# perdoch/hesaff

Hardware: AMD Instinct MI355X
Metric: keypoints/sec (descriptors written), 4K grayscale batch (higher is better)
Workload: dtype f32

## Files before the change

hesaff_amd/csrc/capi_impl.h:

```cpp
#pragma once

namespace {

int fail(hesaff_ctx *c, const HsError &e)
{
   if (c) c->err = e.msg; else g_create_error = e.msg;
   return e.code;
}

#define HS_API_BEGIN try {
#define HS_API_END(ctx)                                              \
   }                                                                 \
   catch (const HsError &e) { return fail(ctx, e); }                 \
   catch (const std::exception &e) { return fail(ctx, HsError(HESAFF_ERR_NOMEM, e.what())); } \
   return HESAFF_OK;

void bind_device(hesaff_ctx *c) { HIP_TRY(hipSetDevice(c->device)); }

void finish_stream(hesaff_ctx *c)
{
   HIP_TRY(hipStreamSynchronize(c->stream));
   HIP_TRY(hipGetLastError());
}

bool finite_f(float v) { return v == v && v - v == 0.0f; }

void validate_params(const hesaff_params &p)
{
   if (!finite_f(p.threshold) || !finite_f(p.edgeEigenValueRatio) || !finite_f(p.initialSigma) || !finite_f(p.convergenceThreshold) ||
       !finite_f(p.mrSize) || !finite_f(p.maxBinValue))
      throw HsError(HESAFF_ERR_ARG, "non-finite parameter");
   if (!(p.initialSigma > 0.0f)) throw HsError(HESAFF_ERR_ARG, "initialSigma must be positive");
   if (!(p.mrSize > 0.0f)) throw HsError(HESAFF_ERR_ARG, "mrSize must be positive");
   if (!(p.edgeEigenValueRatio > 0.0f)) throw HsError(HESAFF_ERR_ARG, "edgeEigenValueRatio must be positive");
   if (p.maxIterations < 1 || p.maxIterations > 1000) throw HsError(HESAFF_ERR_ARG, "maxIterations out of range (1..1000)");
   if (p.fast == 1)
      throw HsError(HESAFF_ERR_ARG, "hesaff_params.fast = 1 was withdrawn in ABI version 4 (it bought 1.02x); use 0 (parity mode) or 2");
   if (p.fast != 0 && p.fast != 2) throw HsError(HESAFF_ERR_ARG, "fast must be 0 (parity mode) or 2");
}

void begin_device_batch(hesaff_ctx *c, int n)
{
   bind_device(c);
   if (n > c->par.max_batch) throw HsError(HESAFF_ERR_ARG, "n exceeds hesaff_params.max_batch for the device-resident entry point");
}

template <class CHECK>
void detect_device(hesaff_ctx *c, int n, const SrcImages &src, int height, int width, int32_t *count_hessian, int32_t *count_desc,
                   const void **d_keys_out, int64_t *total_out, CHECK check_source)
{
   plan(c, c->par.max_batch, height, width);
   check_source();
   run_batch(c, src, n, height, width);
   const int32_t *hs = c->h_starts, *ds = c->h_starts + (n + 1);
   for (int b = 0; b < n; b++) {
      if (count_hessian) count_hessian[b] = hs[b + 1] - hs[b];
      if (count_desc) count_desc[b] = ds[b + 1] - ds[b];
   }
   if (d_keys_out) *d_keys_out = c->geo.b_out.p;
   if (total_out) *total_out = ds[n];
}

}

extern "C" {

const char *hesaff_version(void)
{
#ifdef HESAFF_TUNING
   return "hesaff_amd 0.3 (gfx950, tuning build)";
#else
   return "hesaff_amd 0.3 (gfx950)";
#endif
}

int hesaff_abi_version(void) { return HESAFF_ABI_VERSION; }
size_t hesaff_sizeof_params(void) { return sizeof(hesaff_params); }
size_t hesaff_sizeof_timings(void) { return sizeof(hesaff_timings); }
size_t hesaff_sizeof_region(void) { return sizeof(hesaff_region); }

int hesaff_device_count(void)
{
   int n = 0;
   if (hipGetDeviceCount(&n) != hipSuccess) { (void)hipGetLastError(); return 0; }
   return n;
}

int hesaff_shard_range(int n, int rank, int world, int *lo, int *hi)
{
   if (n < 0 || world < 1 || rank < 0 || rank >= world || !lo || !hi) return HESAFF_ERR_ARG;
   *lo = (int)(((long long)n * rank + world - 1) / world);
   *hi = (int)(((long long)n * (rank + 1) + world - 1) / world);
   return HESAFF_OK;
}

int hesaff_default_params(hesaff_params *p)
{
   if (!p) return HESAFF_ERR_ARG;
   p->threshold = 16.0f / 3.0f;
   p->edgeEigenValueRatio = 10.0f;
   p->initialSigma = 1.6f;
   p->maxIterations = 16;
   p->convergenceThreshold = 0.05f;
   p->mrSize = 3.0f * sqrtf(3.0f);
   p->maxBinValue = 0.2f;
   p->upscaleInputImage = 0;
   p->max_batch = 64;
   p->max_kpts_per_mpx = 40000;
   p->fast = 0;
   return HESAFF_OK;
}

int hesaff_create(hesaff_ctx **out, const hesaff_params *p, int device)
{
   if (!out) return HESAFF_ERR_ARG;
   *out = nullptr;
   hesaff_ctx *c = nullptr;
   try {
      int ndev = 0;
      if (hipGetDeviceCount(&ndev) != hipSuccess || ndev <= 0)
         throw HsError(HESAFF_ERR_DEVICE, "no HIP device visible: libhesaff_amd has no CPU fallback");
      if (device < 0 || device >= ndev) throw HsError(HESAFF_ERR_ARG, "device ordinal out of range");
      c = new hesaff_ctx();
      if (p) c->par = *p; else hesaff_default_params(&c->par);
      if (c->par.max_batch < 1) c->par.max_batch = 1;
      if (c->par.max_kpts_per_mpx < 1000) c->par.max_kpts_per_mpx = 1000;
      validate_params(c->par);
      c->device = device;
      c->fast_pyramid = c->par.fast == 2;
#ifdef HESAFF_TUNING
      if (const char *fm = getenv("HESAFF_FAST")) c->fast_pyramid = atoi(fm) == 2;
#endif
      bind_device(c);
      hipDeviceProp_t prop;
      HIP_TRY(hipGetDeviceProperties(&prop, device));
      if (strncmp(prop.gcnArchName, "gfx950", 6) != 0) {
         std::string m = std::string("device is ") + prop.gcnArchName + ", this library is built for gfx950 only";
         throw HsError(HESAFF_ERR_DEVICE, m);
      }
      {
         hipStream_t *slots[7] = {&c->stream, &c->side_streams[0], &c->side_streams[1], &c->side_streams[2], &c->side_streams[3], &c->sift_stream,
                                  &c->aff_stream};
         const int group[7] = {0, 1, 1, 2, 0, 3, 2};
         hipStream_t made[4] = {nullptr, nullptr, nullptr, nullptr};
         if (take_stream_set(device, c->sset))
            for (int g = 0; g < 4; g++) made[g] = c->sset.comp[g];
         for (int i = 0; i < 7; i++) {
            if (!made[group[i]]) HIP_TRY(hipStreamCreateWithFlags(&made[group[i]], hipStreamNonBlocking));
            *slots[i] = made[group[i]];
         }
         for (int g = 0; g < 4; g++) c->sset.comp[g] = made[g];
      }
      for (int i = 0; i < HS_NSIDE; i++) c->ev_join[i] = DevEvent(hipEventDisableTiming);
      c->ev_fork = DevEvent(hipEventDisableTiming);
      c->ev_detect_done = DevEvent(hipEventDisableTiming | hipEventBlockingSync);
      c->ev_batch_done = DevEvent(hipEventDisableTiming | hipEventBlockingSync);
      for (int i = 0; i < HS_NSLOT; i++) {
         c->ev_extract_done[i] = DevEvent(hipEventDisableTiming);
         c->ev_sift_done[i] = DevEvent(hipEventDisableTiming);
      }
      set_kernel_attrs(c);
      build_tables(c);
      refresh_tables_struct(c);
      memset(&c->tm, 0, sizeof c->tm);
#ifdef HESAFF_TUNING
      if (const char *ov = getenv("HESAFF_OVERLAP")) c->no_overlap = atoi(ov) == 0;
      c->debug = getenv("HESAFF_DEBUG") != nullptr;
#endif
   } catch (const HsError &e) {
      hesaff_destroy(c);
      return fail(nullptr, e);
   } catch (const std::exception &e) {
      hesaff_destroy(c);
      return fail(nullptr, HsError(HESAFF_ERR_NOMEM, e.what()));
   }
   *out = c;
   return HESAFF_OK;
}

void hesaff_destroy(hesaff_ctx *c)
{
   if (!c) return;
   const int device = c->device;
   (void)hipSetDevice(device);
   StreamSet set = c->sset;
   set.h2d = c->h2d_stream; set.d2h = c->d2h_stream;
   for (hipStream_t st : {c->stream, set.comp[0], set.comp[1], set.comp[2], set.comp[3], set.h2d, set.d2h})
      if (st) (void)hipStreamSynchronize(st);
   delete c;
   if (set.comp[0]) give_stream_set(device, set);
}

const char *hesaff_last_error(const hesaff_ctx *c) { return c ? c->err.c_str() : g_create_error.c_str(); }

int hesaff_set_profiling(hesaff_ctx *c, int level)
{
   if (!c) return HESAFF_ERR_ARG;
   c->profiling = level;
   return HESAFF_OK;
}

int hesaff_get_timings(const hesaff_ctx *c, hesaff_timings *t)
{
   if (!c || !t) return HESAFF_ERR_ARG;
   *t = c->tm;
   return HESAFF_OK;
}

int hesaff_detect_batch_device(hesaff_ctx *c, int n, const void *d_gray, int width, int height, int32_t *count_hessian,
                               int32_t *count_desc, const void **d_keys_out, int64_t *total_out)
{
   if (!c || n < 1 || !d_gray) return HESAFF_ERR_ARG;
   HS_API_BEGIN
   begin_device_batch(c, n);
   detect_device(c, n, SrcImages::u8(d_gray, 1, (long long)width * height, width), height, width, count_hessian, count_desc, d_keys_out, total_out, [] {});
   HS_API_END(c)
}

}

namespace {
using namespace hesaff_engine;

[[noreturn]] void throw_bad_f32(int index, const uint8_t *img, int H, int W, size_t stride)
{
   int row = 0, col = 0;
   float v = 0.0f;
   char msg[256];
   if (first_bad_f32(img, H, W, stride, &row, &col, &v))
      snprintf(msg, sizeof msg, "image %d: pixel (row %d, column %d) is %.9g; float input must be finite with |v| <= 2^20", index, row, col, (double)v);
   else
      snprintf(msg, sizeof msg, "image %d: a pixel is not finite or exceeds 2^20 in magnitude", index);
   throw HsError(HESAFF_ERR_ARG, msg);
}

const char *describe_bad_record(const hesaff_region &r, int from, int n_oct)
{
   const float lim = 1048576.0f;
   if (r.type < 0 || r.type > 2) return "type is not 0, 1 or 2";
   if (!finite_f(r.x) || !finite_f(r.y) || !finite_f(r.s) || !finite_f(r.response)) return "x, y, s or response is not finite";
   if (fabsf(r.x) > lim || fabsf(r.y) > lim) return "|x| or |y| exceeds 2^20";
   if (!(r.s > 0.0f && r.s <= lim)) return "s is not in (0, 2^20]";
   if (from == HESAFF_FROM_POINTS) {
      if (r.octave < 0 || r.octave >= n_oct) return "octave is outside this image's pyramid";
      if (r.level < 0 || r.level >= HS_NSCALES) return "level is not one the detector finds keypoints on (0..2)";
      return nullptr;
   }
   const float a[4] = {r.a11, r.a12, r.a21, r.a22};
   for (float v : a) {
      if (!finite_f(v)) return "a11..a22 is not finite";
      if (fabsf(v) > lim) return "|a_ij| exceeds 2^20";
   }
   if ((double)r.a11 * (double)r.a22 - (double)r.a12 * (double)r.a21 == 0.0) return "a11 * a22 - a12 * a21 is zero";
   if ((double)r.a11 * (double)r.a11 + (double)r.a12 * (double)r.a12 == 0.0) return "a11^2 + a12^2 is zero";
   return nullptr;
}

int pyramid_octaves(int H, int W, int up)
{
   int n = 0;
   for (int r = H << up, cc = W << up; r > 2 * HS_BORDER + 2 && cc > 2 * HS_BORDER + 2 && n < HS_MAX_OCTAVES; r /= 2, cc /= 2) n++;
   return n;
}

void ensure_copy_streams(hesaff_ctx *c)
{
   if (c->h2d_stream) return;
   int prio_least = 0, prio_greatest = 0;
   HIP_TRY(hipDeviceGetStreamPriorityRange(&prio_least, &prio_greatest));
   if (c->sset.h2d && c->sset.d2h) {
      c->h2d_stream = c->sset.h2d; c->d2h_stream = c->sset.d2h;
   } else {
      HIP_TRY(hipStreamCreateWithPriority(&c->h2d_stream, hipStreamNonBlocking, prio_greatest));
      HIP_TRY(hipStreamCreateWithPriority(&c->d2h_stream, hipStreamNonBlocking, prio_greatest));
   }
   for (int i = 0; i < 2; i++) {
      c->ev_h2d[i] = DevEvent(hipEventDisableTiming);
      c->ev_h2d_blk[i] = DevEvent(hipEventDisableTiming | hipEventBlockingSync);
      c->ev_in_free[i] = DevEvent(hipEventDisableTiming | hipEventBlockingSync);
      c->ev_out_ready[i] = DevEvent(hipEventDisableTiming);
      c->ev_d2h[i] = DevEvent(hipEventDisableTiming | hipEventBlockingSync);
      for (int q = 0; q < 4; q++) c->ev_exp[i][q] = DevEvent(hipEventDefault);
   }
}

void run_chunks(hesaff_ctx *c, ChunkIO &io, int ring)
{
   bind_device(c);
   ensure_copy_streams(c);
   struct State {
      HostChunk q;
      std::vector<int32_t> nh, nd;
      std::vector<size_t> off;
      std::vector<unsigned long long> toff;
      size_t text_at = 0, bin_at = 0;
      size_t regions_at = 0;
      int total = 0, block = -1, no = 0, largest = 0;
      uint32_t n_rec = 0;
      bool copied = false;
   };
   const int wants = io.wants();
   c->ring.reset(ring);
   if (ring > 0 && (int)c->pin_out.size() < ring) c->pin_out.resize((size_t)ring);
   std::vector<std::future<void>> presize((size_t)std::max(ring, 0));
   bool presized = false;
   struct JoinPresize {
      std::vector<std::future<void>> &f;
      ~JoinPresize() { for (auto &x : f) if (x.valid()) x.wait(); }
   } join_presize{presize};

   auto stage = [&](int k) -> std::unique_ptr<State> {
      (void)pthread_setname_np(pthread_self(), "hs-stage");
      HIP_TRY(hipSetDevice(c->device));
      std::unique_ptr<State> s(new State());
      if (!io.next(s->q)) return nullptr;
      const HostChunk &q = s->q;
      const int slot = k & 1;
      const size_t row_bytes = (size_t)q.W * q.bpp(), img_bytes = row_bytes * q.H;
      const size_t unit = q.blob_bytes ? q.blob_bytes : img_bytes, total = unit * q.data.size();
      hs_wait_event(c->ev_in_free[slot]);
      s->largest = std::max<int>((int)q.data.size(), std::min(io.largest_chunk((int)q.data.size()), c->par.max_batch));
      c->b_in2[slot].ensure(img_bytes * (size_t)s->largest);
      if (q.blob_bytes) c->b_jcoef[slot].ensure(unit * (size_t)s->largest);
      if (q.pinned) {
         uint8_t *dst = (uint8_t *)(q.blob_bytes ? c->b_jcoef[slot].p : c->b_in2[slot].p);
         for (size_t b = 0; b < q.data.size(); b++)
            HIP_TRY(hipMemcpyAsync(dst + unit * b, q.data[b], unit, hipMemcpyHostToDevice, c->h2d_stream));
         HIP_TRY(hipEventRecord(c->ev_h2d[slot], c->h2d_stream));
         HIP_TRY(hipEventRecord(c->ev_h2d_blk[slot], c->h2d_stream));
         hs_wait_event(c->ev_h2d_blk[slot]);
         io.staged(q);
         return s;
      }
      c->pin_in[slot].ensure(unit * (size_t)s->largest);
      const size_t nimg = q.data.size();
      std::vector<size_t> bad_img(nimg + 1, nimg);
      auto copy_images = [&](size_t b0, size_t b1) {
         for (size_t b = b0; b < b1; b++) {
            uint8_t *dst = (uint8_t *)c->pin_in[slot].p + unit * b;
            if (q.blob_bytes) { memcpy(dst, q.data[b], unit); continue; }
            const size_t stride = q.stride[b];
            if (q.f32) {
               for (int y = 0; y < q.H; y++)
                  if (!copy_row_f32(dst + row_bytes * y, q.data[b] + stride * y, q.W)) { bad_img[b0] = b; return; }
               continue;
            }
            if (stride == row_bytes) memcpy(dst, q.data[b], img_bytes);
            else for (int y = 0; y < q.H; y++) memcpy(dst + row_bytes * y, q.data[b] + stride * y, row_bytes);
         }
      };
      const size_t nthr = (total >= ((size_t)32 << 20) && nimg >= 4) ? (size_t)std::max(1, std::min(4, c->stage_threads)) : 1;
      {
         std::vector<std::thread> th;
         size_t t = 1;
         try {
            for (; t < nthr; t++) th.emplace_back(copy_images, nimg * t / nthr, nimg * (t + 1) / nthr);
         } catch (...) {
         }
         copy_images(0, nimg / nthr);
         if (t < nthr) copy_images(nimg * t / nthr, nimg);
         for (auto &x : th) x.join();
      }
      if (q.f32) {
         const size_t b = *std::min_element(bad_img.begin(), bad_img.end());
         if (b < nimg) throw_bad_f32(q.index[b], q.data[b], q.H, q.W, q.stride[b]);
      }
      if (q.from) {
         const int n_oct = pyramid_octaves(q.H, q.W, c->up);
         unsigned long long n_rec = 0;
         for (int cnt : q.region_count) n_rec += (unsigned long long)cnt;
         if (n_rec > 0x7fffffffull) throw HsError(HESAFF_ERR_CAPACITY, "more records in a chunk than 32-bit indices hold");
         const size_t rec_at = describe_records_offset((int)nimg), bytes = rec_at + (size_t)n_rec * sizeof(hesaff_region);
         c->pin_reg[slot].ensure_grow(bytes);
         c->b_reg[slot].ensure_grow(bytes);
         int32_t *starts = (int32_t *)c->pin_reg[slot].p;
         hesaff_region *dst = (hesaff_region *)((char *)c->pin_reg[slot].p + rec_at);
         size_t at = 0;
         for (size_t b = 0; b < nimg; b++) {
            starts[b] = (int32_t)at;
            const hesaff_region *src = q.regions[b];
            for (int i = 0; i < q.region_count[b]; i++) {
               if (const char *why = describe_bad_record(src[i], q.from, n_oct)) {
                  char msg[256];
                  snprintf(msg, sizeof msg, "image %d: record %d: %s", q.index[b], i, why);
                  throw HsError(HESAFF_ERR_ARG, msg);
               }
               dst[at + (size_t)i] = src[i];
            }
            at += (size_t)q.region_count[b];
         }
         starts[nimg] = (int32_t)at;
         s->n_rec = (uint32_t)at;
         HIP_TRY(hipMemcpyAsync(c->b_reg[slot].p, c->pin_reg[slot].p, bytes, hipMemcpyHostToDevice, c->h2d_stream));
      }
      HIP_TRY(hipMemcpyAsync(q.blob_bytes ? c->b_jcoef[slot].p : c->b_in2[slot].p, c->pin_in[slot].p, total, hipMemcpyHostToDevice, c->h2d_stream));
      HIP_TRY(hipEventRecord(c->ev_h2d[slot], c->h2d_stream));
      io.staged(q);
      return s;
   };
   auto deliver = [&](State &s) {
      if (s.copied) hs_wait_event(c->ev_d2h[s.no & 1]);
      if (s.total > 0 && c->profiling && (wants & (WANT_TEXT | WANT_BIN))) {
         float ms = 0.0f;
         float ms2 = 0.0f;
         if (hipEventElapsedTime(&ms, c->ev_exp[s.no & 1][0], c->ev_exp[s.no & 1][1]) == hipSuccess && hipEventElapsedTime(&ms2, c->ev_exp[s.no & 1][2], c->ev_exp[s.no & 1][3]) == hipSuccess) {
            ms += ms2; c->export_ms = ms; c->export_rows = s.total; c->tm.export_ms = ms; c->tm.export_rows = s.total; }
         else (void)hipGetLastError();
      }
      ChunkDone d;
      const char *blk = (const char *)c->pin_out[(size_t)s.block].p;
      d.chunk = &s.q; d.count_hessian = s.nh.data(); d.count_desc = s.nd.data(); d.key_off = s.off.data();
      d.keys = (wants & WANT_KEYS) ? (const hesaff_keypoint *)blk : nullptr; d.block = s.block;
      if (wants & WANT_TEXT) { d.text = blk + s.text_at; d.text_off = s.toff.data(); }
      if (wants & WANT_BIN) d.bin = blk + s.bin_at;
      if (wants & WANT_REGIONS) d.regions = (const hesaff_region *)(blk + s.regions_at);
      io.done(d);
   };

   std::future<std::unique_ptr<State>> staged = std::async(std::launch::async, stage, 0);
   std::unique_ptr<State> prev;
   try {
      for (int k = 0;; k++) {
         const auto dbg_t0 = std::chrono::steady_clock::now();
         const double dbg_c0 = c->debug ? thread_cpu_ms() : 0.0;
         std::unique_ptr<State> cur = staged.get();
         if (!cur) break;
         const auto dbg_t1 = std::chrono::steady_clock::now();
         const double dbg_c1 = c->debug ? thread_cpu_ms() : 0.0;
         cur->no = k;
         staged = std::async(std::launch::async, stage, k + 1);
         const HostChunk &q = cur->q;
         const int slot = k & 1, B = (int)q.data.size();
         const size_t row_bytes = (size_t)q.W * q.bpp(), img_bytes = row_bytes * q.H;
         HIP_TRY(hipStreamWaitEvent(c->stream, c->ev_h2d[slot], 0));
         try {
            plan(c, std::max(std::min<int>(c->par.max_batch, B), cur->largest), q.H, q.W);
            if (q.blob_bytes) jpeg_pixels(c, c->b_jcoef[slot].as<uint8_t>(), make_jpeg_geom(q.jpeg), B, (uint8_t *)c->b_in2[slot].p, img_bytes, c->stream);
            const SrcImages src = q.f32 ? SrcImages::f32(c->b_in2[slot].p, (long long)img_bytes, (int)row_bytes)
                                        : SrcImages::u8(c->b_in2[slot].p, q.ch, (long long)img_bytes, (int)row_bytes);
            if (q.from) run_describe(c, src, B, q.H, q.W, (const uint8_t *)c->b_reg[slot].p, cur->n_rec, q.from);
            else run_batch(c, src, B, q.H, q.W);
         } catch (const HsError &e) {
            if (e.code != HESAFF_ERR_ARG && e.code != HESAFF_ERR_CAPACITY) throw;
            HIP_TRY(hipEventRecord(c->ev_in_free[slot], c->stream));
            if (!io.failed(q, e.code)) throw;
            continue;
         }
         HIP_TRY(hipEventRecord(c->ev_in_free[slot], c->stream));
         const auto dbg_t2 = std::chrono::steady_clock::now();
         const double dbg_c2 = c->debug ? thread_cpu_ms() : 0.0;
         const int32_t *hs = c->h_starts, *ds = c->h_starts + (B + 1);
         cur->total = ds[B];
         cur->nh.resize((size_t)B); cur->nd.resize((size_t)B); cur->off.resize((size_t)B);
         for (int b = 0; b < B; b++) {
            cur->nh[(size_t)b] = hs[b + 1] - hs[b];
            cur->nd[(size_t)b] = ds[b + 1] - ds[b];
            cur->off[(size_t)b] = (size_t)ds[b];
         }
         const size_t n_rows = (size_t)cur->total, n_hess = (size_t)hs[B];
         const KeyRec *d_keys = c->geo.b_out.as<KeyRec>();
         size_t at = 0;
         auto place = [&at](size_t bytes) { const size_t o = at; at = (at + bytes + 255) & ~(size_t)255; return o; };
// ... 209 lines not shown
int hesaff_describe_regions(hesaff_ctx *c, int n, const uint8_t *const *images, const int *widths, const int *heights, const int *strides,
                            const int *channels, const hesaff_region *const *regions, const int *counts, int from, hesaff_region_result *results)
{
   if (!c || n < 0 || (n > 0 && (!images || !widths || !heights || !regions || !counts || !results))) return HESAFF_ERR_ARG;
   HS_API_BEGIN
   const DescribeInput di = describe_input(n, regions, counts, from);
   detect_images(c, n, images, false, widths, heights, strides, channels, 0, [&](ArrayIO &io) { io.region_results = results; }, di);
   HS_API_END(c)
}

int hesaff_describe_regions_f32(hesaff_ctx *c, int n, const float *const *images, const int *widths, const int *heights, const int *strides,
                                const hesaff_region *const *regions, const int *counts, int from, hesaff_region_result *results)
{
   if (!c || n < 0 || (n > 0 && (!images || !widths || !heights || !regions || !counts || !results))) return HESAFF_ERR_ARG;
   HS_API_BEGIN
   const DescribeInput di = describe_input(n, regions, counts, from);
   detect_images(c, n, images, true, widths, heights, strides, nullptr, 0, [&](ArrayIO &io) { io.region_results = results; }, di);
   HS_API_END(c)
}

int hesaff_detect_batch_device_f32(hesaff_ctx *c, int n, const void *d_planes, int width, int height, int row_stride, int64_t img_stride,
                                   int32_t *count_hessian, int32_t *count_desc, const void **d_keys_out, int64_t *total_out)
{
   if (!c || n < 1 || !d_planes || width < 1 || height < 1 || row_stride < 0 || img_stride < 0) return HESAFF_ERR_ARG;
   HS_API_BEGIN
   begin_device_batch(c, n);
   const long long rs = row_stride ? row_stride : 4LL * width;
   const long long is = img_stride ? (long long)img_stride : rs * height;
   if ((uintptr_t)d_planes % 4 != 0) throw HsError(HESAFF_ERR_ARG, "float planes not 4-byte aligned");
   if (rs < 4LL * width || rs % 4 != 0 || rs > 0x7fffffffLL)
      throw HsError(HESAFF_ERR_ARG, "row stride of a float plane must be at least 4 * width bytes and a multiple of 4");
   if (is % 4 != 0 || (n > 1 && is < rs * (height - 1) + 4LL * width))
      throw HsError(HESAFF_ERR_ARG, "image stride of the float planes must be a multiple of 4 and keep the images apart");
   detect_device(c, n, SrcImages::f32(d_planes, is, (int)rs), height, width, count_hessian, count_desc, d_keys_out, total_out,
                 [&] { check_device_f32(c, n, (const uint8_t *)d_planes, is, (int)rs, height, width); });
   HS_API_END(c)
}

int hesaff_set_output_format(hesaff_ctx *c, int format)
{
   if (!c || (format & ~(HESAFF_OUT_TEXT | HESAFF_OUT_BIN)) != 0 || format == 0) return HESAFF_ERR_ARG;
   c->out_format = format;
   return HESAFF_OK;
}

int hesaff_set_resume(hesaff_ctx *c, int on)
{
   if (!c || on < 0 || on > 2) return HESAFF_ERR_ARG;
   c->resume = on;
   return HESAFF_OK;
}

int hesaff_set_pinned_read_budget(hesaff_ctx *c, size_t max_bytes, size_t keep_bytes)
{
   if (!c) return HESAFF_ERR_ARG;
   {
      std::lock_guard<std::mutex> lk(c->pin_read.mu);
      c->pin_read.max_bytes = max_bytes;
      c->pin_read.keep_bytes = std::min(keep_bytes, max_bytes);
   }
   c->pin_read.trim(c->pin_read.keep_bytes);
   return HESAFF_OK;
}

int hesaff_set_pool_priority(hesaff_ctx *c, int mode)
{
   if (!c || mode < -1 || mode > 1) return HESAFF_ERR_ARG;
   c->pool_priority = mode;
   return HESAFF_OK;
}

int hesaff_process_files(hesaff_ctx *c, int n, const char *const *paths, const char *const *out_paths, int decode_threads,
                         int write_threads, hesaff_file_status *status)
{
   if (!c || n < 0 || (n > 0 && (!paths || !status))) return HESAFF_ERR_ARG;
   HS_API_BEGIN
   for (int i = 0; i < n; i++) { status[i].rc = HESAFF_ERR_IO; status[i].stage = HESAFF_FILE_PENDING; status[i].count_hessian = 0; status[i].count_desc = 0; }
   hesaff_host_plan hp;
   (void)hesaff_host_plan_for(1, &hp);
   const int dt = std::max(1, std::min(decode_threads > 0 ? decode_threads : hp.decode_threads, 64));
   const int wt = std::max(1, std::min(write_threads > 0 ? write_threads : hp.write_threads, 256));
   const bool device_jpeg = true;
   PinHooks pin;
   c->pin_read.device = c->device;
   pin.alloc = [](size_t bytes, void *user) -> void * { return ((hesaff_ctx *)user)->pin_read.take(bytes); };
   pin.release = [](void *p, size_t bytes, void *user) { ((hesaff_ctx *)user)->pin_read.give(p, bytes); };
   pin.user = c;
   const bool nice_pool = c->pool_priority == 1 || (c->pool_priority < 0 && hesaff_host_threads() <= dt + wt + 1);
   FileIO io(&c->ring, c->par.max_batch, c->par.mrSize, c->out_format, n, paths, out_paths, status, dt, wt, true, c->resume, device_jpeg, pin, nice_pool);
   c->stage_threads = hesaff_stage_threads_for_pool(dt + wt);
   try {
      run_chunks(c, io, 3);
      io.wait_writers();
   } catch (...) {
      io.shutdown();
      c->pin_read.trim(c->pin_read.keep_bytes);
      throw;
   }
   io.shutdown();
   c->pin_read.trim(c->pin_read.keep_bytes);
   HS_API_END(c)
}


int hesaff_stage_gaussian_blur(hesaff_ctx *c, const float *in, int rows, int cols, float sigma, float *out)
{
   if (!c || !in || !out || rows < 1 || cols < 1 || !(sigma > 0.0f)) return HESAFF_ERR_ARG;
   HS_API_BEGIN
   bind_device(c);
   const int K = hesaff::gauss_ksize(sigma);
   const int pitch = round_up(cols, 64);
   const size_t n = (size_t)rows * pitch;
   c->b_stage.ensure(n * 4 * 3 + (size_t)(K + 16) * 4);
   float *d_in = c->b_stage.as<float>(), *d_tmp = d_in + n, *d_out = d_tmp + n, *d_taps = d_out + n;
   std::vector<float> taps(K, 1.0f);
   if (K > 1) hesaff::gauss_taps(K, sigma, taps.data());
   HIP_TRY(hipMemcpy2DAsync(d_in, (size_t)pitch * 4, in, (size_t)cols * 4, (size_t)cols * 4, rows, hipMemcpyHostToDevice, c->stream));
   HIP_TRY(hipMemcpyAsync(d_taps, taps.data(), (size_t)K * 4, hipMemcpyHostToDevice, c->stream));
   DPlane pi = make_plane(d_in, rows, cols, pitch), pt = make_plane(d_tmp, rows, cols, pitch), po = make_plane(d_out, rows, cols, pitch);
   const DPlane none = make_plane(nullptr, 0, 0, 0);
   if (K == 1) {
      HIP_TRY(hipMemcpyAsync(d_out, d_in, n * 4, hipMemcpyDeviceToDevice, c->stream));
   } else if (K == 9 || K == 11 || K == 13 || K == 15) {
      launch_blur_hess<true, false, false>(c, pi, po, none, none, d_taps, K, 0.0f, 1);
   } else {
      const dim3 grid((cols + 255) / 256, rows, 1);
      hipLaunchKernelGGL(k_blur_rows_generic, grid, dim3(256), 0, c->stream, pi, pt, (const float *)d_taps, K);
      hipLaunchKernelGGL(k_blur_cols_generic, grid, dim3(256), 0, c->stream, pt, po, (const float *)d_taps, K);
   }
   HIP_TRY(hipMemcpy2DAsync(out, (size_t)cols * 4, d_out, (size_t)pitch * 4, (size_t)cols * 4, rows, hipMemcpyDeviceToHost, c->stream));
   finish_stream(c);
   HS_API_END(c)
}

int hesaff_stage_hessian_response(hesaff_ctx *c, const float *in, int rows, int cols, float norm, float *out)
{
   if (!c || !in || !out || rows < 1 || cols < 1) return HESAFF_ERR_ARG;
   HS_API_BEGIN
   bind_device(c);
   const int pitch = round_up(cols, 64);
   const size_t n = (size_t)rows * pitch;
   c->b_stage.ensure(n * 4 * 4 + 64);
   float *d_in = c->b_stage.as<float>(), *d_out = d_in + n, *d_l = d_out + n, *d_r = d_l + n, *d_taps = d_r + n;
   HIP_TRY(hipMemcpy2DAsync(d_in, (size_t)pitch * 4, in, (size_t)cols * 4, (size_t)cols * 4, rows, hipMemcpyHostToDevice, c->stream));
   DPlane pi = make_plane(d_in, rows, cols, pitch), po = make_plane(d_out, rows, cols, pitch);
   std::vector<float> taps(9);
   hesaff::gauss_taps(9, 1.2262737f, taps.data());
   HIP_TRY(hipMemcpyAsync(d_taps, taps.data(), 9 * 4, hipMemcpyHostToDevice, c->stream));
   launch_march<9, true, true, false, true>(c, pi, make_plane(d_l, rows, cols, pitch), make_plane(d_r, rows, cols, pitch), make_plane(nullptr, 0, 0, 0),
                                            d_taps, 1.0f, 1, po, norm * norm);
   HIP_TRY(hipMemcpy2DAsync(out, (size_t)cols * 4, d_out, (size_t)pitch * 4, (size_t)cols * 4, rows, hipMemcpyDeviceToHost, c->stream));
   finish_stream(c);
   HS_API_END(c)
}

int hesaff_stage_half_image(hesaff_ctx *c, const float *in, int rows, int cols, float *out)
{
   if (!c || !in || !out || rows < 2 || cols < 2) return HESAFF_ERR_ARG;
   HS_API_BEGIN
   bind_device(c);
   const size_t n = (size_t)rows * cols;
   const int r2 = rows / 2, c2 = cols / 2;
   c->b_stage.ensure(n * 4 * 2);
   float *d_in = c->b_stage.as<float>(), *d_out = d_in + n;
   HIP_TRY(hipMemcpyAsync(d_in, in, n * 4, hipMemcpyHostToDevice, c->stream));
   DPlane pi = make_plane(d_in, rows, cols, cols), po = make_plane(d_out, r2, c2, c2);
   hipLaunchKernelGGL(k_half, dim3((c2 + 255) / 256, r2, 1), dim3(256), 0, c->stream, pi, po);
   HIP_TRY(hipMemcpyAsync(out, d_out, (size_t)r2 * c2 * 4, hipMemcpyDeviceToHost, c->stream));
   finish_stream(c);
   HS_API_END(c)
}

static int stage_pyramid(hesaff_ctx *c, const void *image, bool f32, int rows, int cols, float *planes, int *n_octaves, size_t *n_floats)
{
   if (!c || rows < 1 || cols < 1) return HESAFF_ERR_ARG;
   HS_API_BEGIN
   bind_device(c);
   plan(c, 1, rows, cols);
   size_t nf = 0;
   for (const OctGeom &g : c->oct) nf += (size_t)10 * g.rows * g.cols;
   if (n_octaves) *n_octaves = (int)c->oct.size();
   if (n_floats) *n_floats = nf;
   if (planes) {
      if (!image) throw HsError(HESAFF_ERR_ARG, f32 ? "plane is NULL" : "gray is NULL");
      const size_t row_bytes = (size_t)cols * (f32 ? 4 : 1), bytes = row_bytes * rows;
      if (f32) {
         if ((uintptr_t)image % 4 != 0) throw HsError(HESAFF_ERR_ARG, "float plane not 4-byte aligned");
         int r = 0, col = 0;
         float v = 0.0f;
         if (first_bad_f32((const uint8_t *)image, rows, cols, row_bytes, &r, &col, &v))
            throw_bad_f32(0, (const uint8_t *)image, rows, cols, row_bytes);
      }
      c->b_input.ensure(bytes);
      c->b_stage.ensure((size_t)rows * round_up(cols, 64) * 4);
      HIP_TRY(hipMemcpyAsync(c->b_input.p, image, bytes, hipMemcpyHostToDevice, c->stream));
      c->ev_used = 0;
      StageTimer tm(c);
      Lists s = make_lists(c);
      const SrcImages src = f32 ? SrcImages::f32(c->b_input.p, (long long)bytes, (int)row_bytes) : SrcImages::u8(c->b_input.p, 1, (long long)bytes, (int)row_bytes);
      run_detection(c, src, 1, s, tm, true, planes);
      finish_stream(c);
   }
   HS_API_END(c)
}

int hesaff_stage_pyramid(hesaff_ctx *c, const uint8_t *gray, int rows, int cols, float *planes, int *n_octaves, size_t *n_floats)
{
   return stage_pyramid(c, gray, false, rows, cols, planes, n_octaves, n_floats);
}

int hesaff_stage_pyramid_f32(hesaff_ctx *c, const float *plane, int rows, int cols, float *planes, int *n_octaves, size_t *n_floats)
{
   return stage_pyramid(c, plane, true, rows, cols, planes, n_octaves, n_floats);
}

int hesaff_stage_hessian_keypoints(hesaff_ctx *c, const uint8_t *gray, int rows, int cols, int cap, float *f, int32_t *iv, int *count)
{
   if (!c || !gray || rows < 1 || cols < 1 || !count) return HESAFF_ERR_ARG;
   HS_API_BEGIN
   bind_device(c);
   plan(c, 1, rows, cols);
   c->b_input.ensure((size_t)rows * cols);
   HIP_TRY(hipMemcpyAsync(c->b_input.p, gray, (size_t)rows * cols, hipMemcpyHostToDevice, c->stream));
   c->ev_used = 0;
   StageTimer tm(c);
   Lists s = make_lists(c);
   run_detection(c, SrcImages::u8(c->b_input.p, 1, (long long)rows * cols, cols), 1, s, tm, false, nullptr);
   uint32_t cn[8];
   HIP_TRY(hipMemcpyAsync(cn, s.counters, sizeof cn, hipMemcpyDeviceToHost, c->stream));
   finish_stream(c);
   if (cn[2] != 0 || cn[1] > c->cap) throw HsError(HESAFF_ERR_CAPACITY, "keypoint capacity exceeded");
   const int n = (int)cn[3];
   *count = n;
   const int m = std::min(n, cap);
   if (m > 0 && f && iv) {
      std::vector<float> x(m), y(m), sc(m), resp(m);
      std::vector<int32_t> meta(m), key(m);
      HIP_TRY(hipMemcpy(x.data(), s.hl.x, (size_t)m * 4, hipMemcpyDeviceToHost));
      HIP_TRY(hipMemcpy(y.data(), s.hl.y, (size_t)m * 4, hipMemcpyDeviceToHost));
      HIP_TRY(hipMemcpy(sc.data(), s.hl.s, (size_t)m * 4, hipMemcpyDeviceToHost));
      HIP_TRY(hipMemcpy(resp.data(), s.hl.response, (size_t)m * 4, hipMemcpyDeviceToHost));
      HIP_TRY(hipMemcpy(meta.data(), s.hl.meta, (size_t)m * 4, hipMemcpyDeviceToHost));
      HIP_TRY(hipMemcpy(key.data(), s.hl.r0c0, (size_t)m * 4, hipMemcpyDeviceToHost));
      for (int i = 0; i < m; i++) {
         const int octave = (meta[i] >> 4) & 15, level = (meta[i] >> 2) & 3, type = meta[i] & 3;
         const OctGeom &g = c->oct[octave];
         const uint32_t pix = (uint32_t)key[i] % (uint32_t)(g.rows * g.cols);
         f[5 * i] = x[i]; f[5 * i + 1] = y[i]; f[5 * i + 2] = sc[i]; f[5 * i + 3] = c->consts.pd0 * (float)(1 << octave); f[5 * i + 4] = resp[i];
         iv[5 * i] = type; iv[5 * i + 1] = octave; iv[5 * i + 2] = level; iv[5 * i + 3] = (int32_t)(pix / g.cols); iv[5 * i + 4] = (int32_t)(pix % g.cols);
      }
   }
   HS_API_END(c)
}

int hesaff_stage_find_affine_shape(hesaff_ctx *c, const float *blur, int rows, int cols, int n, const float *kp, int32_t *converged,
                                   float *U, int32_t *iters)
{
   if (!c || !blur || !kp || rows < 2 || cols < 2 || n < 0) return HESAFF_ERR_ARG;
   HS_API_BEGIN
   bind_device(c);
   if (n == 0) return HESAFF_OK;
   const size_t np = (size_t)rows * cols;
   c->b_stage.ensure(np * 4 + (size_t)n * (4 + 6) * 4 + 64);
   float *d_plane = c->b_stage.as<float>();
   float *d_kp = d_plane + np;
   int32_t *d_conv = (int32_t *)(d_kp + (size_t)4 * n), *d_iters = d_conv + n;
   float *d_U = (float *)(d_iters + n);
   HIP_TRY(hipMemcpyAsync(d_plane, blur, np * 4, hipMemcpyHostToDevice, c->stream));
   HIP_TRY(hipMemcpyAsync(d_kp, kp, (size_t)n * 16, hipMemcpyHostToDevice, c->stream));
   AffineOut ao; ao.converged = d_conv; ao.iters = d_iters; ao.U = d_U;
   DPlane P = make_plane(d_plane, rows, cols, cols);
   hipLaunchKernelGGL(k_affine_stage, dim3(std::min((n + HS_AFFP_G - 1) / HS_AFFP_G, 256 * 6)), dim3(64), 0, c->stream, P, (const float *)d_kp, n, c->tables, c->consts, ao);
   if (converged) HIP_TRY(hipMemcpyAsync(converged, d_conv, (size_t)n * 4, hipMemcpyDeviceToHost, c->stream));
   if (iters) HIP_TRY(hipMemcpyAsync(iters, d_iters, (size_t)n * 4, hipMemcpyDeviceToHost, c->stream));
   if (U) HIP_TRY(hipMemcpyAsync(U, d_U, (size_t)n * 16, hipMemcpyDeviceToHost, c->stream));
   finish_stream(c);
   HS_API_END(c)
}

int hesaff_stage_rectify(hesaff_ctx *c, int n, float *A)
{
   if (!c || !A || n < 0) return HESAFF_ERR_ARG;
   HS_API_BEGIN
   bind_device(c);
   if (n == 0) return HESAFF_OK;
   c->b_stage.ensure((size_t)n * 16);
   HIP_TRY(hipMemcpyAsync(c->b_stage.p, A, (size_t)n * 16, hipMemcpyHostToDevice, c->stream));
   hipLaunchKernelGGL(k_rectify_stage, dim3((n + 255) / 256), dim3(256), 0, c->stream, n, c->b_stage.as<float>());
   HIP_TRY(hipMemcpyAsync(A, c->b_stage.p, (size_t)n * 16, hipMemcpyDeviceToHost, c->stream));
   finish_stream(c);
   HS_API_END(c)
}

int hesaff_stage_normalize_affine(hesaff_ctx *c, const float *img, int rows, int cols, int n, const float *kp, const float *A,
                                  int32_t *rejected, float *patches)
{
   if (!c || !img || !kp || !A || rows < 2 || cols < 2 || n < 0) return HESAFF_ERR_ARG;
   HS_API_BEGIN
   bind_device(c);
   if (n == 0) return HESAFF_OK;
   plan(c, 1, rows, cols);
   if ((uint32_t)n > c->cap) throw HsError(HESAFF_ERR_CAPACITY, "too many keypoints for this image size");
   Lists s = make_lists(c);
   hipStream_t st = c->stream;
   HIP_TRY(hipMemcpy2DAsync(c->gray.p, (size_t)c->gray.pitch * 4, img, (size_t)cols * 4, (size_t)cols * 4, rows, hipMemcpyHostToDevice, st));
   std::vector<float> x(n), y(n), sc(n);
   std::vector<int32_t> meta(n, 0), P0(n), alive(n);
   for (int i = 0; i < n; i++) { x[i] = kp[3 * i]; y[i] = kp[3 * i + 1]; sc[i] = kp[3 * i + 2]; }
   HIP_TRY(hipMemcpyAsync(s.hl.x, x.data(), (size_t)n * 4, hipMemcpyHostToDevice, st));
   HIP_TRY(hipMemcpyAsync(s.hl.y, y.data(), (size_t)n * 4, hipMemcpyHostToDevice, st));
   HIP_TRY(hipMemcpyAsync(s.hl.s, sc.data(), (size_t)n * 4, hipMemcpyHostToDevice, st));
   HIP_TRY(hipMemcpyAsync(s.hl.meta, meta.data(), (size_t)n * 4, hipMemcpyHostToDevice, st));
   HIP_TRY(hipMemcpyAsync(s.pw.A, A, (size_t)n * 16, hipMemcpyHostToDevice, st));
   HIP_TRY(hipMemsetAsync(s.counters, 0, 64 * 4, st));
   uint32_t nn = (uint32_t)n;
   HIP_TRY(hipMemcpyAsync(s.counters + 3, &nn, 4, hipMemcpyHostToDevice, st));
   hipLaunchKernelGGL(k_prepare_patch_given_A, dim3((n + 255) / 256), dim3(256), 0, st, s.hl, (const uint32_t *)(s.counters + 3), rows, cols,
                      c->consts, c->tables, s.pw);
   c->b_patches.ensure((size_t)n * HS_PATCH_PIX * 4);
   HIP_TRY(hipMemsetAsync(c->b_patches.p, 0, (size_t)n * HS_PATCH_PIX * 4, st));
   unsigned long long large_rows = 0;
   c->batch_max_p = 0;
   for (int i = 0; i < n; i++) {
      const float mrScale = ceilf(sc[i] * c->consts.mrSize);
      const long long P = (mrScale < 1.0e6f) ? 2 * (long long)mrScale + 3 : 0;
      if (P > HS_BIN3_PMAX && P <= c->max_p0 + 2) { large_rows += (unsigned long long)P; c->batch_max_p = std::max(c->batch_max_p, (int)P); }
   }
   if (large_rows > 0xffffffffull) throw HsError(HESAFF_ERR_NOMEM, "too many huge windows in one call");
   run_patch_stage(c, s, c->gray, c->b_patches.as<float>(), 0, (uint32_t)large_rows);
   uint32_t ovf = 0;
   HIP_TRY(hipMemcpyAsync(&ovf, s.counters + 6, 4, hipMemcpyDeviceToHost, st));
   HIP_TRY(hipMemcpyAsync(alive.data(), s.pw.alive, (size_t)n * 4, hipMemcpyDeviceToHost, st));
   if (patches) HIP_TRY(hipMemcpyAsync(patches, c->b_patches.p, (size_t)n * HS_PATCH_PIX * 4, hipMemcpyDeviceToHost, st));
   finish_stream(c);
   if (ovf) throw HsError(HESAFF_ERR_NOMEM, "large-window row buffer exceeded (internal bound violated)");
   if (rejected) for (int i = 0; i < n; i++) rejected[i] = alive[i] ? 0 : 1;
   HS_API_END(c)
}

int hesaff_stage_sift(hesaff_ctx *c, int n, const float *patches, uint8_t *desc)
{
   if (!c || !patches || !desc || n < 0) return HESAFF_ERR_ARG;
   HS_API_BEGIN
   bind_device(c);
   if (n == 0) return HESAFF_OK;
   const size_t N = (size_t)n;
   const size_t off_alive = N * HS_PATCH_PIX * 4, off_mv = off_alive + N * 4, off_vec = off_mv + N * 8, off_desc = off_vec + N * 128 * 4;
   const size_t off_vo = (off_desc + N * 128 + 63) & ~(size_t)63, total = off_vo + N * HS_VO_PITCH * 8 + 64;
   c->b_stage.ensure(total);
   char *base = (char *)c->b_stage.p;
   std::vector<int32_t> ones(N, 1);
   HIP_TRY(hipMemcpyAsync(base, patches, N * HS_PATCH_PIX * 4, hipMemcpyHostToDevice, c->stream));
   HIP_TRY(hipMemcpyAsync(base + off_alive, ones.data(), N * 4, hipMemcpyHostToDevice, c->stream));
   HIP_TRY(hipMemsetAsync(base + off_vo, 0, N * HS_VO_PITCH * 8 + 64, c->stream));
   SiftIO so;
   so.patches = (const float *)base; so.alive = (const int32_t *)(base + off_alive); so.meanvar = (float *)(base + off_mv);
   so.vec = (float *)(base + off_vec); so.desc = (uint8_t *)(base + off_desc); so.h_lo = 0; so.h_hi = (uint32_t)n;
   launch_sift(c, c->stream, so, (uint32_t)n, (float2 *)(base + off_vo));
   HIP_TRY(hipMemcpyAsync(desc, base + off_desc, N * 128, hipMemcpyDeviceToHost, c->stream));
   finish_stream(c);
   HS_API_END(c)
}

int hesaff_stage_export(hesaff_ctx *c, const hesaff_keypoint *keys, int n, float mrSize, int format, char **out, size_t *len)
{
   if (!c || n < 0 || (n > 0 && !keys) || !out || !len || (format != HESAFF_OUT_TEXT && format != HESAFF_OUT_BIN)) return HESAFF_ERR_ARG;
   HS_API_BEGIN
   bind_device(c);
   const float saved = c->par.mrSize;
   c->par.mrSize = mrSize;
   char *buf = nullptr;
   try {
      const size_t N = (size_t)n;
      c->b_stage.ensure(std::max<size_t>(N * sizeof(KeyRec), 16));
      if (n > 0) HIP_TRY(hipMemcpyAsync(c->b_stage.p, keys, N * sizeof(KeyRec), hipMemcpyHostToDevice, c->stream));
      const KeyRec *d_keys = c->b_stage.as<KeyRec>();
      char head[64];
      size_t hl, body;
      if (format == HESAFF_OUT_TEXT) {
         const int32_t starts[2] = {0, n};
         c->b_ex_starts.ensure(16);
         HIP_TRY(hipMemcpyAsync(c->b_ex_starts.p, starts, sizeof starts, hipMemcpyHostToDevice, c->stream));
         std::vector<unsigned long long> off;
         body = (size_t)export_text_prepare(c, d_keys, (uint32_t)n, c->b_ex_starts.as<int32_t>(), 1, off);
         hl = (size_t)snprintf(head, sizeof head, "%d\n%d\n", 128, n);
      } else {
         body = N * EX_BIN_ROW;
         memcpy(head, "HESAFFB1", 8);
         const uint32_t dim = 128, cnt = (uint32_t)n;
         memcpy(head + 8, &dim, 4); memcpy(head + 12, &cnt, 4);
         hl = 16;
      }
      buf = (char *)malloc(hl + body + 1);
      if (!buf) throw HsError(HESAFF_ERR_NOMEM, "malloc failed");
      memcpy(buf, head, hl);
      if (body > 0) {
         c->b_generic.ensure(body + 16);
         if (format == HESAFF_OUT_TEXT) export_text_write(c, d_keys, (uint32_t)n, (char *)c->b_generic.p);
         else export_bin_rows(c, d_keys, (uint32_t)n, (char *)c->b_generic.p);
         HIP_TRY(hipMemcpyAsync(buf + hl, c->b_generic.p, body, hipMemcpyDeviceToHost, c->stream));
      }
      finish_stream(c);
      *out = buf;
      *len = hl + body;
   } catch (...) {
      c->par.mrSize = saved;
      free(buf);
      throw;
   }
   c->par.mrSize = saved;
   HS_API_END(c)
}

int hesaff_stage_fmt_g(hesaff_ctx *c, int n, const float *v, char *text, int32_t *lens)
{
   if (!c || n < 0 || (n > 0 && (!v || !text || !lens))) return HESAFF_ERR_ARG;
   HS_API_BEGIN
   bind_device(c);
   if (n == 0) return HESAFF_OK;
   const size_t N = (size_t)n;
   c->b_stage.ensure(N * (4 + 16 + 4));
   float *d_v = c->b_stage.as<float>();
   int32_t *d_len = (int32_t *)(d_v + N);
   char *d_text = (char *)(d_len + N);
   HIP_TRY(hipMemcpyAsync(d_v, v, N * 4, hipMemcpyHostToDevice, c->stream));
   HIP_TRY(hipMemsetAsync(d_text, 0, N * 16, c->stream));
   hipLaunchKernelGGL(k_fmt_g_test, dim3((n + 255) / 256), dim3(256), 0, c->stream, n, (const float *)d_v, d_text, d_len);
   HIP_TRY(hipMemcpyAsync(text, d_text, N * 16, hipMemcpyDeviceToHost, c->stream));
   HIP_TRY(hipMemcpyAsync(lens, d_len, N * 4, hipMemcpyDeviceToHost, c->stream));
   finish_stream(c);
   HS_API_END(c)
}

int hesaff_stage_jpeg_pixels(hesaff_ctx *c, const hesaff_jpeg_layout *layout, int n, const uint8_t *blobs, size_t blob_bytes, uint8_t *pixels)
{
   if (!c || !layout || n < 0 || (n > 0 && (!blobs || !pixels))) return HESAFF_ERR_ARG;
   HS_API_BEGIN
   bind_device(c);
   if (n == 0) return HESAFF_OK;
   const JpegGeom g = make_jpeg_geom(*layout);
   if ((size_t)g.blob_bytes != blob_bytes) throw HsError(HESAFF_ERR_ARG, "blob size does not match the layout");
   const size_t img = (size_t)g.W * g.H * g.nc;
   c->b_jcoef[0].ensure(blob_bytes * (size_t)n);
   c->b_stage.ensure(img * (size_t)n);
   HIP_TRY(hipMemcpyAsync(c->b_jcoef[0].p, blobs, blob_bytes * (size_t)n, hipMemcpyHostToDevice, c->stream));
   jpeg_pixels(c, c->b_jcoef[0].as<uint8_t>(), g, n, c->b_stage.as<uint8_t>(), img, c->stream);
   HIP_TRY(hipMemcpyAsync(pixels, c->b_stage.p, img * (size_t)n, hipMemcpyDeviceToHost, c->stream));
   finish_stream(c);
   HS_API_END(c)
}

int hesaff_stage_math(hesaff_ctx *c, int n, const float *a, const float *b, float *atan2_out, float *pow2_out)
{
   if (!c || !a || !b || n < 0) return HESAFF_ERR_ARG;
   HS_API_BEGIN
   bind_device(c);
   if (n == 0) return HESAFF_OK;
   c->b_stage.ensure((size_t)n * 16);
   float *d_a = c->b_stage.as<float>(), *d_b = d_a + n, *d_at = d_b + n, *d_pw = d_at + n;
   HIP_TRY(hipMemcpyAsync(d_a, a, (size_t)n * 4, hipMemcpyHostToDevice, c->stream));
   HIP_TRY(hipMemcpyAsync(d_b, b, (size_t)n * 4, hipMemcpyHostToDevice, c->stream));
   hipLaunchKernelGGL(k_math, dim3((n + 255) / 256), dim3(256), 0, c->stream, n, (const float *)d_a, (const float *)d_b, d_at, d_pw);
   if (atan2_out) HIP_TRY(hipMemcpyAsync(atan2_out, d_at, (size_t)n * 4, hipMemcpyDeviceToHost, c->stream));
   if (pow2_out) HIP_TRY(hipMemcpyAsync(pow2_out, d_pw, (size_t)n * 4, hipMemcpyDeviceToHost, c->stream));
   finish_stream(c);
   HS_API_END(c)
}

int hesaff_stage_math_sift(hesaff_ctx *c, int n, const float *gy, const float *gx, float *ori_general, float *ori_nd, float *grad_general,
                           float *grad_nd)
{
   if (!c || !gy || !gx || !ori_general || !ori_nd || !grad_general || !grad_nd || n < 0) return HESAFF_ERR_ARG;
   HS_API_BEGIN
   bind_device(c);
   if (n == 0) return HESAFF_OK;
   c->b_stage.ensure((size_t)n * 24);
   float *d = c->b_stage.as<float>();
   HIP_TRY(hipMemcpyAsync(d, gy, (size_t)n * 4, hipMemcpyHostToDevice, c->stream));
   HIP_TRY(hipMemcpyAsync(d + n, gx, (size_t)n * 4, hipMemcpyHostToDevice, c->stream));
   hipLaunchKernelGGL(k_math_sift, dim3(std::min(4096, (n + 255) / 256)), dim3(256), 0, c->stream, n, (const float *)d, (const float *)(d + n),
                      d + 2 * (size_t)n, d + 3 * (size_t)n, d + 4 * (size_t)n, d + 5 * (size_t)n);
   float *outs[4] = {ori_general, ori_nd, grad_general, grad_nd};
   for (int q = 0; q < 4; q++) HIP_TRY(hipMemcpyAsync(outs[q], d + (2 + q) * (size_t)n, (size_t)n * 4, hipMemcpyDeviceToHost, c->stream));
   finish_stream(c);
   HS_API_END(c)
}


int hesaff_table_gauss_mask(int size, float *mask)
{
   if (size < 1 || !(size & 1) || !mask) return HESAFF_ERR_ARG;
   hesaff::gauss_mask(size, mask);
   return HESAFF_OK;
}
int hesaff_table_circ_gauss_mask(int size, float *mask)
{
   if (size < 1 || !(size & 1) || !mask) return HESAFF_ERR_ARG;
   hesaff::circ_gauss_mask(size, mask);
   return HESAFF_OK;
}
int hesaff_table_sift_bins(int32_t *bin0, int32_t *bin1, float *w0, float *w1)
{
   if (!bin0 || !bin1 || !w0 || !w1) return HESAFF_ERR_ARG;
   hesaff::sift_bins(bin0, bin1, w0, w1);
   return HESAFF_OK;
}
int hesaff_table_gauss_kernel(float sigma, int cap, float *taps, int *ksize)
{
   if (!ksize) return HESAFF_ERR_ARG;
   const int K = hesaff::gauss_ksize(sigma);
   *ksize = K;
   if (taps) {
      if (cap < K) return HESAFF_ERR_ARG;
      if (K == 1) taps[0] = 1.0f; else hesaff::gauss_taps(K, sigma, taps);
   }
   return HESAFF_OK;
}

}
```

hesaff_amd/csrc/hmath.h:

```cpp
#pragma once
#include <stdint.h>

#if defined(__HIPCC__)
#define HM_HD __host__ __device__ __forceinline__
#else
#define HM_HD inline
#endif

HM_HD uint32_t hm_f2u(float f) { union { float f; uint32_t u; } v; v.f = f; return v.u; }
HM_HD float    hm_u2f(uint32_t u) { union { float f; uint32_t u; } v; v.u = u; return v.f; }
HM_HD uint64_t hm_d2u(double f) { union { double f; uint64_t u; } v; v.f = f; return v.u; }
HM_HD double   hm_u2d(uint64_t u) { union { double f; uint64_t u; } v; v.u = u; return v.f; }

HM_HD float hm_fabsf(float x) { return hm_u2f(hm_f2u(x) & 0x7fffffffu); }

HM_HD float hm_atanf(float x)
{
   const float atanhi0 = hm_u2f(0x3eed6338u), atanhi1 = hm_u2f(0x3f490fdau),
               atanhi2 = hm_u2f(0x3f7b985eu), atanhi3 = hm_u2f(0x3fc90fdau);
   const float atanlo0 = hm_u2f(0x31ac3769u), atanlo1 = hm_u2f(0x33222168u),
               atanlo2 = hm_u2f(0x33140fb4u), atanlo3 = hm_u2f(0x33a22168u);
   const float aT0 = hm_u2f(0x3eaaaaabu), aT1 = hm_u2f(0xbe4ccccdu), aT2 = hm_u2f(0x3e124925u),
               aT3 = hm_u2f(0xbde38e38u), aT4 = hm_u2f(0x3dba2e6eu), aT5 = hm_u2f(0xbd9d8795u),
               aT6 = hm_u2f(0x3d886b35u), aT7 = hm_u2f(0xbd6ef16bu), aT8 = hm_u2f(0x3d4bda59u),
               aT9 = hm_u2f(0xbd15a221u), aT10 = hm_u2f(0x3c8569d7u);
   const int32_t hx = (int32_t)hm_f2u(x);
   const int32_t ix = hx & 0x7fffffff;
   int id;
   float hi = 0.0f, lo = 0.0f;
   if (ix >= 0x4c000000) {
      if (ix > 0x7f800000) return x + x;
      return (hx > 0) ? (atanhi3 + atanlo3) : (-atanhi3 - atanlo3);
   }
   if (ix < 0x3ee00000) {
      if (ix < 0x31000000) return x;
      id = -1;
   } else {
      x = hm_fabsf(x);
      float num, den;
      if (ix < 0x3f980000) {
         if (ix < 0x3f300000) { id = 0; hi = atanhi0; lo = atanlo0; num = 2.0f * x - 1.0f; den = 2.0f + x; }
         else                 { id = 1; hi = atanhi1; lo = atanlo1; num = x - 1.0f; den = x + 1.0f; }
      } else {
         if (ix < 0x401c0000) { id = 2; hi = atanhi2; lo = atanlo2; num = x - 1.5f; den = 1.0f + 1.5f * x; }
         else                 { id = 3; hi = atanhi3; lo = atanlo3; num = -1.0f; den = x; }
      }
      x = num / den;
   }
   const float z = x * x;
   const float w = z * z;
   const float s1 = z * (aT0 + w * (aT2 + w * (aT4 + w * (aT6 + w * (aT8 + w * aT10)))));
   const float s2 = w * (aT1 + w * (aT3 + w * (aT5 + w * (aT7 + w * aT9))));
   if (id < 0) return x - x * (s1 + s2);
   const float r = hi - ((x * (s1 + s2) - lo) - x);
   return (hx < 0) ? -r : r;
}

HM_HD float hm_atan2f(float y, float x)
{
   const float tiny = 1.0e-30f;
   const float pi_o_4 = hm_u2f(0x3f490fdbu), pi_o_2 = hm_u2f(0x3fc90fdbu),
               pi = hm_u2f(0x40490fdbu), pi_lo = hm_u2f(0xb3bbbd2eu);
   const int32_t hx = (int32_t)hm_f2u(x), hy = (int32_t)hm_f2u(y);
   const int32_t ix = hx & 0x7fffffff, iy = hy & 0x7fffffff;
   if (ix > 0x7f800000 || iy > 0x7f800000) return x + y;
   if (hx == 0x3f800000) return hm_atanf(y);
   const int m = (int)(((uint32_t)hy >> 31) & 1u) | (int)(((uint32_t)hx >> 30) & 2u);
   if (iy == 0) {
      switch (m) {
         case 0: case 1: return y;
         case 2: return pi + tiny;
         default: return -pi - tiny;
      }
   }
   if (ix == 0) return (hy < 0) ? (-pi_o_2 - tiny) : (pi_o_2 + tiny);
   if (ix == 0x7f800000) {
      if (iy == 0x7f800000) {
         switch (m) {
            case 0: return pi_o_4 + tiny;
            case 1: return -pi_o_4 - tiny;
            case 2: return 3.0f * pi_o_4 + tiny;
            default: return -3.0f * pi_o_4 - tiny;
         }
      } else {
         switch (m) {
            case 0: return 0.0f;
            case 1: return -0.0f;
            case 2: return pi + tiny;
            default: return -pi - tiny;
         }
      }
   }
   if (iy == 0x7f800000) return (hy < 0) ? (-pi_o_2 - tiny) : (pi_o_2 + tiny);
   const int32_t k = (iy - ix) >> 23;
   float z;
   if (k > 60) z = pi_o_2 + 0.5f * pi_lo;
   else if (hx < 0 && k < -60) z = 0.0f;
   else z = hm_atanf(hm_fabsf(y / x));
   switch (m) {
      case 0: return z;
      case 1: return hm_u2f(hm_f2u(z) ^ 0x80000000u);
      case 2: return pi - (z - pi_lo);
      default: return (z - pi_lo) - pi;
   }
}

HM_HD float hm_atan2f_sel(float y, float x)
{
   const float pi_o_2 = hm_u2f(0x3fc90fdbu), pi = hm_u2f(0x40490fdbu), pi_lo = hm_u2f(0xb3bbbd2eu);
   const int32_t hx = (int32_t)hm_f2u(x), hy = (int32_t)hm_f2u(y);
   const int32_t ix = hx & 0x7fffffff, iy = hy & 0x7fffffff;
   const int32_t k = (iy - ix) >> 23;
   if ((ix >= 0x7f800000) | (iy >= 0x7f800000) | ((iy != 0) & (ix != 0) & ((k > 60) | (k < -60)))) return hm_atan2f(y, x);
   const float q = hm_fabsf(y / x);
   const int32_t iq = (int32_t)hm_f2u(q);
   const bool i0 = iq < 0x3f300000, i1 = iq < 0x3f980000, i2 = iq < 0x401c0000, im = iq < 0x3ee00000;
   float num = i1 ? (i0 ? 2.0f * q - 1.0f : q - 1.0f) : (i2 ? q - 1.5f : -1.0f);
   float den = i1 ? (i0 ? 2.0f + q : q + 1.0f) : (i2 ? 1.0f + 1.5f * q : q);
   float hi = i1 ? (i0 ? hm_u2f(0x3eed6338u) : hm_u2f(0x3f490fdau)) : (i2 ? hm_u2f(0x3f7b985eu) : hm_u2f(0x3fc90fdau));
   float lo = i1 ? (i0 ? hm_u2f(0x31ac3769u) : hm_u2f(0x33222168u)) : (i2 ? hm_u2f(0x33140fb4u) : hm_u2f(0x33a22168u));
   num = im ? q : num;
   den = im ? 1.0f : den;
   hi = im ? 0.0f : hi;
   lo = im ? 0.0f : lo;
   const float xr = num / den;
   const float z = xr * xr;
   const float w = z * z;
   const float aT0 = hm_u2f(0x3eaaaaabu), aT1 = hm_u2f(0xbe4ccccdu), aT2 = hm_u2f(0x3e124925u),
               aT3 = hm_u2f(0xbde38e38u), aT4 = hm_u2f(0x3dba2e6eu), aT5 = hm_u2f(0xbd9d8795u),
               aT6 = hm_u2f(0x3d886b35u), aT7 = hm_u2f(0xbd6ef16bu), aT8 = hm_u2f(0x3d4bda59u),
               aT9 = hm_u2f(0xbd15a221u), aT10 = hm_u2f(0x3c8569d7u);
   const float s1 = z * (aT0 + w * (aT2 + w * (aT4 + w * (aT6 + w * (aT8 + w * aT10)))));
   const float s2 = w * (aT1 + w * (aT3 + w * (aT5 + w * (aT7 + w * aT9))));
   float za = hi - ((xr * (s1 + s2) - lo) - xr);
   za = (iq >= 0x4c000000) ? hm_u2f(0x3fc90fdau) + hm_u2f(0x33a22168u) : za;
   float r = (hx < 0) ? pi - (za - pi_lo) : za;
   r = (ix == 0) ? ((iy == 0) ? ((hx < 0) ? pi : 0.0f) : pi_o_2) : r;
   return hm_u2f(hm_f2u(r) ^ ((uint32_t)hy & 0x80000000u));
}


#define HM_ATAN_TAB_FLOATS 40
#define HM_ATAN_TAB_INIT                                                                                           \
   {1.0f, 0.0f, 0.0f, 1.0f, 0.0f, 0.0f, 0.0f, 0.0f,                                                               \
    2.0f, 1.0f, -1.0f, 2.0f, 0x1.dac67p-2f , 0x1.586ed2p-28f , 0.0f, 0.0f,                  \
    1.0f, 1.0f, -1.0f, 1.0f, 0x1.921fb4p-1f , 0x1.4442dp-25f , 0.0f, 0.0f,                  \
    1.0f, 1.5f, -1.5f, 1.0f, 0x1.f730bcp-1f , 0x1.281f68p-25f , 0.0f, 0.0f,                 \
    0.0f, 1.0f, -1.0f, 0.0f, 0x1.921fb4p+0f , 0x1.4442dp-24f , 0.0f, 0.0f}

#if defined(__HIPCC__)
__host__ __device__ __attribute__((noinline)) inline float hm_atan2f_rare(float y, float x) { return hm_atan2f(y, x); }
#else
inline float hm_atan2f_rare(float y, float x) { return hm_atan2f(y, x); }
#endif

HM_HD float hm_div_normal(float a, float b)
{
#if defined(__HIP_DEVICE_COMPILE__)
   const float r0 = __builtin_amdgcn_rcpf(b);
   const float e0 = __builtin_fmaf(-b, r0, 1.0f);
   const float r1 = __builtin_fmaf(e0, r0, r0);
   const float q0 = a * r1;
   const float e1 = __builtin_fmaf(-b, q0, a);
   const float q1 = __builtin_fmaf(e1, r1, q0);
   const float e2 = __builtin_fmaf(-b, q1, a);
   return __builtin_fmaf(e2, r1, q1);
#else
   return a / b;
#endif
}
HM_HD float hm_sqrt_normal(float x)
{
#if defined(__HIP_DEVICE_COMPILE__)
   float s = __builtin_amdgcn_sqrtf(x);
   const float sd = hm_u2f(hm_f2u(s) - 1u), su = hm_u2f(hm_f2u(s) + 1u);
   const float vp = __builtin_fmaf(-sd, s, x), vs = __builtin_fmaf(-su, s, x);
   s = (vp <= 0.0f) ? sd : s;
   s = (vs > 0.0f) ? su : s;
   return s;
#else
   return __builtin_sqrtf(x);
#endif
}

template <bool ND>
HM_HD float hm_atan2f_tab_t(float y, float x, const float *tab)
{
   const float pi_o_2 = hm_u2f(0x3fc90fdbu), pi = hm_u2f(0x40490fdbu), pi_lo = hm_u2f(0xb3bbbd2eu);
   const int32_t hx = (int32_t)hm_f2u(x), hy = (int32_t)hm_f2u(y);
   const int32_t ix = hx & 0x7fffffff, iy = hy & 0x7fffffff;
   const int32_t k = (iy - ix) >> 23;
   if ((ix >= 0x7f800000) | (iy >= 0x7f800000) | ((iy != 0) & (ix != 0) & ((k > 60) | (k < -60)))) return hm_atan2f_rare(y, x);
   const float q = hm_fabsf(ND ? hm_div_normal(y, x) : y / x);
   const int32_t iq = (int32_t)hm_f2u(q);
   const int id = (int)(iq >= 0x3ee00000) + (int)(iq >= 0x3f300000) + (int)(iq >= 0x3f980000) + (int)(iq >= 0x401c0000);
   const float *row = tab + 8 * id;
   const float num = row[0] * q + row[2];
   const float den = row[1] * q + row[3];
   const float hi = row[4], lo = row[5];
   const float xr = ND ? hm_div_normal(num, den) : num / den;
   const float z = xr * xr;
   const float w = z * z;
   const float aT0 = hm_u2f(0x3eaaaaabu), aT1 = hm_u2f(0xbe4ccccdu), aT2 = hm_u2f(0x3e124925u),
               aT3 = hm_u2f(0xbde38e38u), aT4 = hm_u2f(0x3dba2e6eu), aT5 = hm_u2f(0xbd9d8795u),
               aT6 = hm_u2f(0x3d886b35u), aT7 = hm_u2f(0xbd6ef16bu), aT8 = hm_u2f(0x3d4bda59u),
               aT9 = hm_u2f(0xbd15a221u), aT10 = hm_u2f(0x3c8569d7u);
   const float s1 = z * (aT0 + w * (aT2 + w * (aT4 + w * (aT6 + w * (aT8 + w * aT10)))));
   const float s2 = w * (aT1 + w * (aT3 + w * (aT5 + w * (aT7 + w * aT9))));
   float za = hi - ((xr * (s1 + s2) - lo) - xr);
   za = (iq >= 0x4c000000) ? hm_u2f(0x3fc90fdau) + hm_u2f(0x33a22168u) : za;
   float r = (hx < 0) ? pi - (za - pi_lo) : za;
   r = (ix == 0) ? ((iy == 0) ? ((hx < 0) ? pi : 0.0f) : pi_o_2) : r;
   return hm_u2f(hm_f2u(r) ^ ((uint32_t)hy & 0x80000000u));
}
HM_HD float hm_atan2f_tab(float y, float x, const float *tab) { return hm_atan2f_tab_t<false>(y, x, tab); }
HM_HD float hm_atan2f_tab_nd(float y, float x, const float *tab) { return hm_atan2f_tab_t<true>(y, x, tab); }

HM_HD float hm_pow2f(float y)
{
   const uint64_t T[32] = {
      0x3ff0000000000000ull, 0x3fefd9b0d3158574ull, 0x3fefb5586cf9890full, 0x3fef9301d0125b51ull,
      0x3fef72b83c7d517bull, 0x3fef54873168b9aaull, 0x3fef387a6e756238ull, 0x3fef1e9df51fdee1ull,
      0x3fef06fe0a31b715ull, 0x3feef1a7373aa9cbull, 0x3feedea64c123422ull, 0x3feece086061892dull,
      0x3feebfdad5362a27ull, 0x3feeb42b569d4f82ull, 0x3feeab07dd485429ull, 0x3feea47eb03a5585ull,
      0x3feea09e667f3bcdull, 0x3fee9f75e8ec5f74ull, 0x3feea11473eb0187ull, 0x3feea589994cce13ull,
      0x3feeace5422aa0dbull, 0x3feeb737b0cdc5e5ull, 0x3feec49182a3f090ull, 0x3feed503b23e255dull,
      0x3feee89f995ad3adull, 0x3feeff76f2fb5e47ull, 0x3fef199bdd85529cull, 0x3fef3720dcef9069ull,
      0x3fef5818dcfba487ull, 0x3fef7c97337b9b5full, 0x3fefa4afa2a490daull, 0x3fefd0765b6e4540ull };
   const double C0 = hm_u2d(0x3fac6af84b912394ull);
   const double C1 = hm_u2d(0x3fcebfce50fac4f3ull);
   const double C2 = hm_u2d(0x3fe62e42ff0c52d6ull);
   const double SHIFT = hm_u2d(0x42e8000000000000ull);
   const double xd = (double)y;
   double kd = xd + SHIFT;
   const uint64_t ki = hm_d2u(kd);
   kd -= SHIFT;
   const double r = xd - kd;
   uint64_t t = T[ki & 31];
   t += ki << (52 - 5);
   const double s = hm_u2d(t);
#ifdef HM_POW2F_FMA
   const double z = __builtin_fma(C0, r, C1);
   const double r2 = r * r;
   double p = __builtin_fma(C2, r, 1.0);
   p = __builtin_fma(z, r2, p);
#else
   const double z = C0 * r + C1;
   const double r2 = r * r;
   double p = C2 * r + 1.0;
   p = z * r2 + p;
#endif
   p = p * s;
   return (float)p;
}

HM_HD float hm_sift_orient_coord(float ori)
{
   const double twopi = hm_u2d(0x401921fb54442d18ull);
   const double inv_twopi = hm_u2d(0x3fc45f306dc9c883ull);
   const double a = 8.0 * ((double)ori + twopi);
   const double q = a * inv_twopi;
   const double r = __builtin_fma(-q, twopi, a);
   const double q2 = __builtin_fma(r, inv_twopi, q);
   return (float)q2;
}
```

hesaff_amd/csrc/kernels_keypoint.h:

```cpp
#pragma once
#include <type_traits>
#include "device_common.h"
#include "kernels_pyramid.h"

struct PlaneTab {
   DPlane L[HS_MAX_OCTAVES][HS_NSCALES];
};

struct KpTables {
   const float *smm_mask;
   const float *sift_mask;
   const int32_t *mask_idx;
   int n_masked;
   const int4 *sgrad_nb;
   const int2 *sgrad_om;
   const int4 *vo_rows;
   const uint16_t *vo_src;
   const int32_t *bin0, *bin1;
   const float *w0, *w1;
   const float *patch_taps;
   const int32_t *patch_tap_off;
   const int32_t *patch_tap_k;
   int max_p0;
};

struct AffineOut {
   int32_t *converged;
   float *U;
   int32_t *iters;
};

#define HS_AFF_G 4
__device__ inline bool hs_window_outside(int imRows, int imCols, float ofsx, float ofsy, float a11, float a12, float a21, float a22, int half)
{
   const float width = (float)(imCols - 1), height = (float)(imRows - 1);
   bool outside = false;
#pragma unroll
   for (int q = 0; q < 4; q++) {
      const int j = (q & 1) ? half : -half, i = (q & 2) ? half : -half;
      const float rx = ofsx + (float)j * a12, ry = ofsy + (float)j * a22;
      const float fx = floorf(rx + (float)i * a11), fy = floorf(ry + (float)i * a21);
      outside = outside || !(fx >= 0.0f && fy >= 0.0f && fx < width && fy < height);
   }
   return outside;
}

#define HS_AFF_NT 23
#define HS_AFFP_G 4
#define HS_AFFP_L (64 / HS_AFFP_G)
#define HS_AFFP_SH 4
#define HS_AFFP_NT ((HS_SMM_PIX + HS_AFFP_L - 1) / HS_AFFP_L)
#define HS_AFF_BATCHES 2
#define HS_AFF_ARR 364

struct AffKp { const float *blur; int rows, cols, pitch; float x, y, s, pd; };

template <class Fetch>
__device__ __forceinline__ void hs_affine_groups(uint32_t first, uint32_t n, const float *__restrict__ mask_g, const DConsts &k, AffineOut out,
                                                 Fetch fetch)
{
   __shared__ __attribute__((aligned(16))) float s_arr[HS_AFFP_G][3][HS_AFF_ARR];
   __shared__ float s_mask[HS_AFF_ARR];
   __shared__ float s_bc[HS_AFFP_G][8];
   const int lane = threadIdx.x, grp = lane >> HS_AFFP_SH, li = lane & (HS_AFFP_L - 1);
   for (int i = lane; i < HS_SMM_PIX; i += 64) s_mask[i] = mask_g[i];
   float *s_img = s_arr[grp][0], *s_pa = s_arr[grp][0], *s_pb = s_arr[grp][1], *s_pc = s_arr[grp][2];
   uint32_t hstep = gridDim.x * HS_AFFP_G, h_end = n;
   uint32_t h = first + blockIdx.x * HS_AFFP_G + grp;
   if ((gridDim.x & 7u) == 0u && n > first) {
      const uint32_t n_items = (n - first + HS_AFFP_G - 1) / HS_AFFP_G;
      const uint32_t xcd = blockIdx.x & 7u, rank = blockIdx.x >> 3, per_xcd = gridDim.x >> 3;
      const uint32_t it_lo = (uint32_t)(((unsigned long long)n_items * xcd) >> 3), it_hi = (uint32_t)(((unsigned long long)n_items * (xcd + 1)) >> 3);
      hstep = per_xcd * HS_AFFP_G;
      h_end = min(first + it_hi * HS_AFFP_G, n);
      h = first + (it_lo + rank) * HS_AFFP_G + grp;
   }
#define HS_AFF_END h_end
   if (k.maxIterations <= 0) {
      for (; h < HS_AFF_END; h += hstep)
         if (li == 0) {
            out.converged[h] = 0; out.iters[h] = 0;
            out.U[4 * h + 0] = 1.0f; out.U[4 * h + 1] = 0.0f; out.U[4 * h + 2] = 0.0f; out.U[4 * h + 3] = 1.0f;
         }
      return;
   }
   const float *blur = nullptr;
   int pitch = 0, width = 0, height = 0, l = 0;
   float lx = 0, ly = 0, ratio = 0, u11 = 1.0f, u12 = 0.0f, u21 = 0.0f, u22 = 1.0f;
   float eigen_ratio_act = 0.0f, eigen_ratio_bef = 0.0f;
   bool active = h < HS_AFF_END;
   auto load_kp = [&]() {
      if (active) {
         const AffKp q = fetch(h);
         blur = q.blur; pitch = q.pitch; width = q.cols - 1; height = q.rows - 1;
         lx = q.x / q.pd; ly = q.y / q.pd;
         ratio = q.s / (k.affInitialSigma * q.pd);
         u11 = 1.0f; u12 = 0.0f; u21 = 0.0f; u22 = 1.0f;
         eigen_ratio_act = 0.0f; eigen_ratio_bef = 0.0f;
         l = 0;
      }
   };
   load_kp();
   HS_WAVE_LDS_SYNC();
   while (__ballot(active) != 0ull) {
      bool win_in = true;
      if (active) {
         const float a11 = u11 * ratio, a12 = u12 * ratio, a21 = u21 * ratio, a22 = u22 * ratio;
         win_in = !hs_window_outside(height + 1, width + 1, lx, ly, a11, a12, a21, a22, HS_SMM >> 1);
      }
      const bool all_in = __ballot(active && !win_in) == 0ull;
      auto sample = [&](auto inside_c) {
         constexpr bool INSIDE = decltype(inside_c)::value;
         const float a11 = u11 * ratio, a12 = u12 * ratio, a21 = u21 * ratio, a22 = u22 * ratio;
#pragma unroll
         for (int half = 0; half < HS_AFF_BATCHES; half++) {
            constexpr int NB = (HS_AFFP_NT + HS_AFF_BATCHES - 1) / HS_AFF_BATCHES;
            float sv[NB];
#pragma unroll
            for (int t = 0; t < NB; t++) {
               const int idx = min(li + HS_AFFP_L * (half * NB + t), HS_SMM_PIX - 1);
               const int jj = idx / HS_SMM, ii = idx - jj * HS_SMM;
               const int j = jj - (HS_SMM >> 1), i = ii - (HS_SMM >> 1);
               const float rx = lx + (float)j * a12;
               const float ry = ly + (float)j * a22;
               const float wx = rx + (float)i * a11;
               const float wy = ry + (float)i * a21;
               if (INSIDE) {
                  sv[t] = hs_tap_inside_ptr(blur, pitch, wx, wy);
               } else {
                  bool outside = false;
                  sv[t] = hs_bilinear(blur, pitch, width, height, wx, wy, outside);
               }
            }
#pragma unroll
            for (int t = 0; t < NB; t++) HS_KEEP(sv[t]);
#pragma unroll
            for (int t = 0; t < NB; t++) {
               const int idx = li + HS_AFFP_L * (half * NB + t);
               if (idx < HS_SMM_PIX) s_img[idx] = sv[t];
            }
         }
      };
      if (active) {
         if (all_in) sample(std::true_type{});
         else sample(std::false_type{});
      }
      HS_WAVE_LDS_SYNC();
      if (active) {
         float pa[HS_AFFP_NT];
#pragma unroll
         for (int t = 0; t < HS_AFFP_NT; t++) {
            const int idx = min(li + HS_AFFP_L * t, HS_SMM_PIX - 1);
            const int r = idx / HS_SMM, c = idx - r * HS_SMM;
            const float gxx = s_img[idx + (c < HS_SMM - 1 ? 1 : 0)] - s_img[idx - (c > 0 ? 1 : 0)];
            const float gyy = s_img[idx + (r < HS_SMM - 1 ? HS_SMM : 0)] - s_img[idx - (r > 0 ? HS_SMM : 0)];
            const float v = s_mask[idx];
            const float gxy = gxx * gyy;
            pa[t] = gxx * gxx * v;
            if (li + HS_AFFP_L * t < HS_SMM_PIX) {
               s_pb[idx] = gxy * v;
               s_pc[idx] = gyy * gyy * v;
            }
         }
         HS_WAVE_LDS_SYNC();
#pragma unroll
         for (int t = 0; t < HS_AFFP_NT; t++) {
            const int idx = li + HS_AFFP_L * t;
            if (idx < HS_SMM_PIX) s_pa[idx] = pa[t];
         }
      }
      HS_WAVE_LDS_SYNC();
      if (active && li < 3) {
         const float *pp = s_arr[grp][li];
         const float4 *p4 = reinterpret_cast<const float4 *>(pp);
         float acc = 0.0f;
         for (int i0 = 0; i0 < HS_SMM_PIX / 4; i0 += 10) {
            float4 q[10];
#pragma unroll
            for (int u = 0; u < 10; u++) q[u] = p4[i0 + u];
#pragma unroll
            for (int u = 0; u < 10; u++) { acc += q[u].x; acc += q[u].y; acc += q[u].z; acc += q[u].w; }
         }
         acc += pp[HS_SMM_PIX - 1];
         s_bc[grp][li] = acc / (float)HS_SMM_PIX;
      }
      HS_WAVE_LDS_SYNC();
      if (active && li == 0) {
         float a = s_bc[grp][0], b = s_bc[grp][1], c = s_bc[grp][2];
         float l1, l2;
         hs_inv_sqrt(a, b, c, l1, l2);
         eigen_ratio_bef = eigen_ratio_act;
         eigen_ratio_act = 1 - l2 / l1;
         const float u11t = u11, u12t = u12;
         const float n11 = a * u11t + b * u21, n12 = a * u12t + b * u22;
         const float n21 = b * u11t + c * u21, n22 = b * u12t + c * u22;
         int state = 0;
         if (!hs_eigenvalues(n11, n12, n21, n22, l1, l2)) state = 1;
         else if ((l1 / l2 > 6) || (l2 / l1 > 6)) state = 1;
         else if (eigen_ratio_act < k.convergenceThreshold && eigen_ratio_bef < k.convergenceThreshold) state = 2;
         s_bc[grp][3] = n11; s_bc[grp][4] = n12; s_bc[grp][5] = n21; s_bc[grp][6] = n22;
         s_bc[grp][7] = __int_as_float(state);
      }
      HS_WAVE_LDS_SYNC();
      if (active) {
         u11 = s_bc[grp][3]; u12 = s_bc[grp][4]; u21 = s_bc[grp][5]; u22 = s_bc[grp][6];
         const int state = __float_as_int(s_bc[grp][7]);
         if (state != 0 || l + 1 >= k.maxIterations) {
            if (li == 0) {
               out.converged[h] = (state == 2) ? 1 : 0;
               out.iters[h] = (state == 2) ? l : 0;
               out.U[4 * h + 0] = u11; out.U[4 * h + 1] = u12; out.U[4 * h + 2] = u21; out.U[4 * h + 3] = u22;
            }
            h += hstep;
            active = h < HS_AFF_END;
            load_kp();
         } else {
            l++;
         }
      }
      HS_WAVE_LDS_SYNC();
   }
}


__global__ __launch_bounds__(64) void k_affine(PlaneTab pt, HessList hl, uint32_t h_lo, uint32_t h_hi, const uint32_t *__restrict__ n_ptr,
                                               KpTables tb, DConsts k, AffineOut out)
{
   const uint32_t n = min(min(*n_ptr, hl.cap), h_hi);
   hs_affine_groups(
      h_lo, n, tb.smm_mask, k, out, [&](uint32_t h) {
      const int meta = hl.meta[h];
      const int b = meta >> 8, octave = (meta >> 4) & 15, level = (meta >> 2) & 3;
      const DPlane &P = pt.L[octave][level];
      AffKp q;
      q.blur = P.img(b); q.rows = P.rows; q.cols = P.cols; q.pitch = P.pitch;
      q.x = hl.x[h]; q.y = hl.y[h]; q.s = hl.s[h]; q.pd = k.pd0 * (float)(1 << octave);
      return q;
   });
}

__global__ __launch_bounds__(64) void k_affine_stage(DPlane P, const float *__restrict__ kp , int n, KpTables tb, DConsts k,
                                                     AffineOut out)
{
   hs_affine_groups(0u, (uint32_t)n, tb.smm_mask, k, out, [&](uint32_t h) {
      AffKp q;
      q.blur = P.img(0); q.rows = P.rows; q.cols = P.cols; q.pitch = P.pitch;
      q.x = kp[4 * h]; q.y = kp[4 * h + 1]; q.s = kp[4 * h + 2]; q.pd = kp[4 * h + 3];
      return q;
   });
}

#define HS_NBINS 5
#define HS_BIN3_PMAX 512
__host__ __device__ inline int hs_patch_bin(int P) { return P <= 41 ? 0 : (P <= 64 ? 1 : (P <= 128 ? 2 : (P <= HS_BIN3_PMAX ? 3 : 4))); }

struct PatchWork {
   float *A;
   int32_t *P0;
   int32_t *alive;
   uint32_t *bin_count;
   uint32_t *bin_work;
   uint32_t *bin_items;
   uint32_t cap;
};

__device__ __forceinline__ int hs_window_p0(float s, float mrSize)
{
   const float mrScale = ceilf(s * mrSize);
   const int m = (mrScale < 1.0e6f) ? (int)mrScale : 1000000;
   return 2 * m + 1;
}

__global__ __launch_bounds__(256) void k_image_large_rows(HessList hl, const uint32_t *__restrict__ n_ptr, float mrSize, uint32_t *__restrict__ rows, int nimg,
                                                          int max_p0);

template <bool RECTIFY>
__device__ __forceinline__ void hs_prepare_patch_body(const HessList &hl, uint32_t h_lo, uint32_t n, const AffineOut &aff, int imRows, int imCols,
                                                      const DConsts &k, const KpTables &tb, const PatchWork &pw)
{
   for (uint32_t h0 = h_lo + blockIdx.x * blockDim.x; h0 < n; h0 += gridDim.x * blockDim.x) {
      const uint32_t h = h0 + threadIdx.x;
      const bool valid = h < n;
      int alive = 0, P0 = 0;
      if (valid && (!RECTIFY || aff.converged[h])) {
         float a11, a12, a21, a22;
         if (RECTIFY) {
            a11 = aff.U[4 * h]; a12 = aff.U[4 * h + 1]; a21 = aff.U[4 * h + 2]; a22 = aff.U[4 * h + 3];
            hs_rectify(a11, a12, a21, a22);
            pw.A[4 * h] = a11; pw.A[4 * h + 1] = a12; pw.A[4 * h + 2] = a21; pw.A[4 * h + 3] = a22;
         } else {
            a11 = pw.A[4 * h]; a12 = pw.A[4 * h + 1]; a21 = pw.A[4 * h + 2]; a22 = pw.A[4 * h + 3];
         }
         P0 = hs_window_p0(hl.s[h], k.mrSize);
         const float scale = (float)P0 / (float)HS_PATCH;
         bool rej = hs_check_borders(imRows, imCols, hl.x[h], hl.y[h], a11 * scale, a12 * scale, a21 * scale, a22 * scale);
         if (!rej && (double)scale > 0.4) rej = hs_window_outside(imRows, imCols, hl.x[h], hl.y[h], a11, a12, a21, a22, (P0 + 2) >> 1);
         alive = (!rej && P0 <= tb.max_p0) ? 1 : 0;
      }
      if (valid) {
         pw.alive[h] = alive;
         pw.P0[h] = alive ? P0 : 0;
      }
      int bin = -1;
      if (alive) {
         const float scale = (float)P0 / (float)HS_PATCH;
         const int P = ((double)scale > 0.4) ? P0 + 2 : 0;
         bin = hs_patch_bin(P);
      }
      const int lane = threadIdx.x & 63;
#pragma unroll
      for (int bq = 0; bq < HS_NBINS; bq++) {
         const unsigned long long m = __ballot(bin == bq);
         if (m == 0ull) continue;
         const int leader = __ffsll((long long)m) - 1;
         uint32_t base = 0;
         if (lane == leader) base = atomicAdd(pw.bin_count + bq, (uint32_t)__popcll(m));
         base = __shfl(base, leader, 64);
         if (bin == bq) pw.bin_items[(size_t)bq * pw.cap + base + (uint32_t)__popcll(m & ((1ull << lane) - 1ull))] = h;
      }
   }
}

__global__ __launch_bounds__(256) void k_image_large_rows(HessList hl, const uint32_t *__restrict__ n_ptr, float mrSize, uint32_t *__restrict__ rows, int nimg,
                                                          int max_p0)
{
   const uint32_t n = min(*n_ptr, hl.cap);
   for (uint32_t h = blockIdx.x * blockDim.x + threadIdx.x; h < n; h += gridDim.x * blockDim.x) {
      const int P0 = hs_window_p0(hl.s[h], mrSize);
      const float scale = (float)P0 / (float)HS_PATCH;
      const int P = ((double)scale > 0.4) ? P0 + 2 : 0;
      if (hs_patch_bin(P) == HS_NBINS - 1 && P0 < (1 << 20) && P0 <= max_p0) {
         atomicAdd(rows + (hl.meta[h] >> 8), (uint32_t)P);
         atomicMax(rows + nimg + 1, (uint32_t)P);
      }
   }
}

__global__ __launch_bounds__(256) void k_prepare_patch(HessList hl, uint32_t h_lo, uint32_t h_hi, const uint32_t *__restrict__ n_ptr, AffineOut aff,
                                                       int imRows, int imCols, DConsts k, KpTables tb, PatchWork pw)
{
   hs_prepare_patch_body<true>(hl, h_lo, min(min(*n_ptr, hl.cap), h_hi), aff, imRows, imCols, k, tb, pw);
}

__global__ __launch_bounds__(256) void k_prepare_patch_given_A(HessList hl, const uint32_t *__restrict__ n_ptr, int imRows, int imCols,
                                                               DConsts k, KpTables tb, PatchWork pw)
{
   AffineOut none;
   none.converged = nullptr; none.U = nullptr; none.iters = nullptr;
   hs_prepare_patch_body<false>(hl, 0u, min(*n_ptr, hl.cap), none, imRows, imCols, k, tb, pw);
}

struct KeyRec {
   float x, y, s, a11, a12, a21, a22, response;
   int32_t type;
   uint8_t desc[128];
};

#define HS_PACK_KP 64
#define HS_PACK_DW 41
__global__ __launch_bounds__(256) void k_pack(HessList hl, const uint32_t *__restrict__ n_ptr, PatchWork pw,
                                              const uint32_t *__restrict__ rank, const uint8_t *__restrict__ desc, KeyRec *__restrict__ out)
{
   static_assert(sizeof(KeyRec) == 4 * HS_PACK_DW, "record layout");
   __shared__ uint32_t s_rec[HS_PACK_KP * HS_PACK_DW];
   __shared__ int s_lr[HS_PACK_KP];
   const uint32_t n = min(*n_ptr, hl.cap);
   const int tid = threadIdx.x;
   const uint32_t *desc32 = reinterpret_cast<const uint32_t *>(desc);
   uint32_t *out32 = reinterpret_cast<uint32_t *>(out);
   for (uint32_t h0 = blockIdx.x * HS_PACK_KP; h0 < n; h0 += gridDim.x * HS_PACK_KP) {
      const uint32_t base = rank[h0];
      if (tid < HS_PACK_KP) {
         const uint32_t h = h0 + tid;
         const bool live = h < n && pw.alive[h];
         const int lr = live ? (int)(rank[h] - base) : -1;
         s_lr[tid] = lr;
         if (live) {
            uint32_t *r = s_rec + lr * HS_PACK_DW;
            const float4 A = *reinterpret_cast<const float4 *>(pw.A + 4 * (size_t)h);
            r[0] = __float_as_uint(hl.x[h]); r[1] = __float_as_uint(hl.y[h]); r[2] = __float_as_uint(hl.s[h]);
            r[3] = __float_as_uint(A.x); r[4] = __float_as_uint(A.y); r[5] = __float_as_uint(A.z); r[6] = __float_as_uint(A.w);
            r[7] = __float_as_uint(hl.response[h]);
            r[8] = (uint32_t)(hl.meta[h] & 3);
         }
      }
      __syncthreads();
      int n_live = 0;
#pragma unroll
      for (int q = 0; q < HS_PACK_KP * 32 / 256; q++) {
         const int idx = tid + 256 * q, j = idx >> 5, d = idx & 31;
         const int lr = s_lr[j];
         if (lr >= 0) s_rec[lr * HS_PACK_DW + 9 + d] = desc32[(size_t)(h0 + j) * 32 + d];
      }
      for (int j = HS_PACK_KP - 1; j >= 0; j--)
         if (s_lr[j] >= 0) { n_live = s_lr[j] + 1; break; }
      __syncthreads();
      const uint32_t total = (uint32_t)n_live * HS_PACK_DW;
      uint32_t *o = out32 + (size_t)base * HS_PACK_DW;
      for (uint32_t i = tid; i < total; i += 256) o[i] = s_rec[i];
      __syncthreads();
   }
}

struct RegionTab { float pd[HS_MAX_OCTAVES]; };
#define HS_REGION_DW 16
__global__ __launch_bounds__(256) void k_pack_regions(HessList hl, uint32_t n, AffineOut aff, PatchWork pw, const uint32_t *__restrict__ rank,
                                                      const int32_t *__restrict__ desc_starts, RegionTab tab, uint4 *__restrict__ out)
{
   for (uint32_t h = blockIdx.x * blockDim.x + threadIdx.x; h < n; h += gridDim.x * blockDim.x) {
      const int meta = hl.meta[h];
      const int b = meta >> 8, octave = (meta >> 4) & 15, level = (meta >> 2) & 3, type = meta & 3;
      const bool converged = aff.converged[h] != 0;
      const bool described = converged && pw.alive[h] != 0;
      uint4 U = make_uint4(0u, 0u, 0u, 0u);
      uint32_t iters = 0u;
      if (converged) {
         U = *reinterpret_cast<const uint4 *>(aff.U + 4 * (size_t)h);
         iters = (uint32_t)aff.iters[h];
      }
      const uint32_t outcome = converged ? (described ? 2u : 1u) : 0u;
      const uint32_t key = described ? rank[h] - (uint32_t)desc_starts[b] : 0xffffffffu;
      uint4 *o = out + 4 * (size_t)h;
      o[0] = make_uint4(__float_as_uint(hl.x[h]), __float_as_uint(hl.y[h]), __float_as_uint(hl.s[h]), __float_as_uint(tab.pd[octave]));
      o[1] = make_uint4(__float_as_uint(hl.response[h]), (uint32_t)type, (uint32_t)octave, (uint32_t)level);
      o[2] = U;
      o[3] = make_uint4(iters, outcome, key, 0u);
   }
}

__global__ __launch_bounds__(256) void k_ingest_regions(const uint4 *__restrict__ recs, uint32_t n, const int32_t *__restrict__ starts, int nimg,
                                                        int shapes, HessList hl, AffineOut aff, uint32_t *__restrict__ n_hess,
                                                        int32_t *__restrict__ hess_starts)
{
   const uint32_t t0 = blockIdx.x * blockDim.x + threadIdx.x;
   if (t0 <= (uint32_t)nimg) hess_starts[t0] = starts[t0];
   if (t0 == 0) *n_hess = n;
   for (uint32_t h = t0; h < n; h += gridDim.x * blockDim.x) {
      const uint4 *r = recs + 4 * (size_t)h;
      const uint4 q0 = r[0], q1 = r[1];
      int lo = 0, hi = nimg;
      while (hi - lo > 1) {
         const int mid = (lo + hi) >> 1;
         if ((uint32_t)starts[mid] <= h) lo = mid; else hi = mid;
      }
      const uint32_t octave = q1.z < (uint32_t)HS_MAX_OCTAVES ? q1.z : 0u, level = q1.w < 4u ? q1.w : 0u, type = q1.y & 3u;
      hl.x[h] = __uint_as_float(q0.x); hl.y[h] = __uint_as_float(q0.y); hl.s[h] = __uint_as_float(q0.z);
      hl.response[h] = __uint_as_float(q1.x);
      hl.meta[h] = (int32_t)(((uint32_t)lo << 8) | (octave << 4) | (level << 2) | type);
      hl.r0c0[h] = 0;
      if (shapes) {
         const uint4 q2 = r[2], q3 = r[3];
         *reinterpret_cast<uint4 *>(aff.U + 4 * (size_t)h) = q2;
         aff.converged[h] = 1;
         aff.iters[h] = (int32_t)q3.x;
      }
   }
}

__global__ void k_math(int n, const float *__restrict__ a, const float *__restrict__ b, float *__restrict__ at, float *__restrict__ pw)
{
   const int i = blockIdx.x * blockDim.x + threadIdx.x;
   if (i >= n) return;
   at[i] = hm_atan2f(a[i], b[i]);
   pw[i] = hm_pow2f(a[i]);
}

__global__ void k_rectify_stage(int n, float *A)
{
   const int i = blockIdx.x * blockDim.x + threadIdx.x;
   if (i >= n) return;
   hs_rectify(A[4 * i], A[4 * i + 1], A[4 * i + 2], A[4 * i + 3]);
}
```

hesaff_amd/csrc/kernels_sift.h:

```cpp
#pragma once
#include "kernels_patch.h"

struct SiftIO {
   const float *patches;
   const int32_t *alive;
   float *meanvar;
   float *vec;
   uint8_t *desc;
   uint32_t h_lo, h_hi;
};

#define HS_VO_DIM 40
#define HS_VO_TILE (HS_VO_DIM * HS_VO_DIM)
#define HS_VO_ITEMS 648
#define HS_VO_ZERO 642
#define HS_VO_PITCH (2 * HS_VO_ITEMS)
#define HS_SIFT_MSK_IT 5
#define SM_TILE 64

#define SM_KP 16
#define SM_PX (64 * 64 / SM_KP)
#define SM_UNROLL 8
#define SM_ROW (SM_PX + 1)
__global__ __launch_bounds__(64) void k_sift_meanvar(SiftIO io, KpTables tb)
{
   __shared__ float s_tile[SM_KP * SM_ROW];
   const int lane = threadIdx.x;
   const uint32_t n = io.h_hi - io.h_lo;
   const uint32_t k0 = blockIdx.x * SM_KP;
   const int nm = tb.n_masked;
   const float gsum = (float)nm;
   const uint32_t kmine = min(k0 + (uint32_t)min(lane, SM_KP - 1), n - 1);
   float sum = 0.0f, mean = 0.0f;
   for (int pass = 0; pass < 2; pass++) {
      float acc = 0.0f;
      for (int c0 = 0; c0 < nm; c0 += SM_PX) {
         const int cnt = min(SM_PX, nm - c0);
         int pix[SM_PX / 64];
#pragma unroll
         for (int u = 0; u < SM_PX / 64; u++) pix[u] = (lane + 64 * u < cnt) ? tb.mask_idx[c0 + lane + 64 * u] : 0;
#pragma unroll SM_UNROLL
         for (int k = 0; k < SM_KP; k++) {
            const uint32_t kp = min(k0 + k, n - 1);
            const float *pp = io.patches + (size_t)kp * HS_PATCH_PIX;
#pragma unroll
            for (int u = 0; u < SM_PX / 64; u++) {
               const float *q = pp + pix[u];
               s_tile[k * SM_ROW + lane + 64 * u] = *q;
            }
         }
         __syncthreads();
         if (lane < SM_KP) {
            const float *row = s_tile + lane * SM_ROW;
            if (pass == 0) {
               for (int l = 0; l < cnt; l++) acc += row[l];
            } else {
               for (int l = 0; l < cnt; l++) { const float d = mean - row[l]; acc += d * d; }
            }
         }
         __syncthreads();
      }
      if (pass == 0) { sum = acc; mean = sum / gsum; }
      else {
         const float var = sqrtf(acc / gsum);
         if (lane < SM_KP && k0 + lane < n) { io.meanvar[2 * (size_t)kmine] = mean; io.meanvar[2 * (size_t)kmine + 1] = var; }
      }
   }
}

__global__ __launch_bounds__(256) void k_sift_grad(SiftIO io, KpTables tb, float2 *__restrict__ vo)
{
   __shared__ float s_p[HS_PATCH_PIX];
   __shared__ float s_at[HM_ATAN_TAB_FLOATS];
   __shared__ __attribute__((aligned(16))) float2 s_vo[HS_VO_TILE];
   const int tid = threadIdx.x;
   const uint32_t n = io.h_hi - io.h_lo;
   for (int i = tid; i < HS_VO_TILE; i += 256) s_vo[i] = make_float2(0.0f, 0.0f);
   constexpr int VO_NI = (HS_VO_ITEMS + 255) / 256;
   int vsrc[VO_NI];
#pragma unroll
   for (int i = 0; i < VO_NI; i++) vsrc[i] = tb.vo_src[min(tid + 256 * i, HS_VO_ITEMS - 1)];
   {
      const float at_init[HM_ATAN_TAB_FLOATS] = HM_ATAN_TAB_INIT;
      if (tid < HM_ATAN_TAB_FLOATS) s_at[tid] = at_init[tid];
   }
   int4 nbq[HS_SIFT_MSK_IT];
   int2 omq[HS_SIFT_MSK_IT];
#pragma unroll
   for (int q = 0; q < HS_SIFT_MSK_IT; q++) { nbq[q] = tb.sgrad_nb[tid + 256 * q]; omq[q] = tb.sgrad_om[tid + 256 * q]; }
   uint32_t k = blockIdx.x;
   if (k >= n) return;
   float pv[HS_PATCH_PIX_IT];
   int alive = io.alive[io.h_lo + k];
   float mean = io.meanvar[2 * (size_t)k], var = io.meanvar[2 * (size_t)k + 1];
   {
      const float *gp = io.patches + (size_t)k * HS_PATCH_PIX;
#pragma unroll
      for (int q = 0; q < HS_PATCH_PIX_IT; q++) pv[q] = gp[min(tid + 256 * q, HS_PATCH_PIX - 1)];
   }
   for (; k < n; k += gridDim.x) {
      const bool cur_alive = alive != 0;
      const bool cur_norm = !((double)var < 0.0001);
      if (cur_alive) {
         const bool norm = cur_norm;
         const float fac = 50.0f / var;
#pragma unroll
         for (int q = 0; q < HS_PATCH_PIX_IT; q++) {
            const int i = tid + 256 * q;
            if (i < HS_PATCH_PIX) {
               float v = pv[q];
               if (norm) { v = 128 + fac * (v - mean); v = v > 255 ? 255.0f : v; v = v < 0 ? 0.0f : v; }
               s_p[i] = v;
            }
         }
      }
      const uint32_t kn = k + gridDim.x;
      if (kn < n) {
         alive = io.alive[io.h_lo + kn];
         mean = io.meanvar[2 * (size_t)kn]; var = io.meanvar[2 * (size_t)kn + 1];
         const float *gp = io.patches + (size_t)kn * HS_PATCH_PIX;
#pragma unroll
         for (int q = 0; q < HS_PATCH_PIX_IT; q++) pv[q] = gp[min(tid + 256 * q, HS_PATCH_PIX - 1)];
      }
      __syncthreads();
      if (cur_alive) {
         auto pixels = [&](auto nd_c) {
            constexpr bool ND = decltype(nd_c)::value;
#pragma unroll
            for (int q = 0; q < HS_SIFT_MSK_IT; q++) {
               if (omq[q].x >= 0) {
                  const char *sp = reinterpret_cast<const char *>(s_p);
                  const float gx = *reinterpret_cast<const float *>(sp + nbq[q].y) - *reinterpret_cast<const float *>(sp + nbq[q].x);
                  const float gy = *reinterpret_cast<const float *>(sp + nbq[q].w) - *reinterpret_cast<const float *>(sp + nbq[q].z);
                  const float grad = ND ? hm_sqrt_normal(gx * gx + gy * gy) : sqrtf(gx * gx + gy * gy);
                  const float ori = ND ? hm_atan2f_tab_nd(gy, gx, s_at) : hm_atan2f_tab(gy, gx, s_at);
                  const float o = hm_sift_orient_coord(ori);
                  s_vo[omq[q].x] = make_float2(__int_as_float(omq[q].y) * grad, o);
               }
               __builtin_amdgcn_sched_barrier(0);
            }
         };
         if (cur_norm) pixels(std::true_type{});
         else pixels(std::false_type{});
      }
      __syncthreads();
      if (cur_alive) {
         float4 *o4 = reinterpret_cast<float4 *>(vo + (size_t)k * HS_VO_PITCH);
         const float4 *t4 = reinterpret_cast<const float4 *>(s_vo);
#pragma unroll
         for (int i = 0; i < VO_NI; i++) {
            const int e = tid + 256 * i;
            if (e < HS_VO_ITEMS) {
               const float4 v = t4[vsrc[i]];
               hs_store_nt4(reinterpret_cast<float *>(o4 + e), v.x, v.y, v.z, v.w);
            }
         }
      }
      __syncthreads();
   }
}


__global__ void k_math_sift(int n, const float *__restrict__ gy, const float *__restrict__ gx, float *__restrict__ ori_g,
                            float *__restrict__ ori_nd, float *__restrict__ grad_g, float *__restrict__ grad_nd)
{
   __shared__ float s_at[HM_ATAN_TAB_FLOATS];
   {
      const float at_init[HM_ATAN_TAB_FLOATS] = HM_ATAN_TAB_INIT;
      if (threadIdx.x < HM_ATAN_TAB_FLOATS) s_at[threadIdx.x] = at_init[threadIdx.x];
   }
   __syncthreads();
   for (int i = blockIdx.x * blockDim.x + threadIdx.x; i < n; i += gridDim.x * blockDim.x) {
      const float y = gy[i], x = gx[i];
      ori_g[i] = hm_atan2f(y, x);
      ori_nd[i] = hm_atan2f_tab_nd(y, x, s_at);
      grad_g[i] = sqrtf(x * x + y * y);
      grad_nd[i] = hm_sqrt_normal(x * x + y * y);
   }
}

#define HS_HIST_AHEAD 1
__global__ __launch_bounds__(64) void k_sift_hist(SiftIO io, KpTables tb, const float2 *__restrict__ vo)
{
   __shared__ __attribute__((aligned(2048))) float s_acc[8 * 64];
   __shared__ float s_cw[64];
   const int tid = threadIdx.x;
   const int kq = tid >> 4, cell = tid & 15, cb_r = cell >> 2, cb_c = cell & 3;
   {
      const int b = tid >> 4, i = tid & 15, r = 8 * b + i;
      float w = 0.0f;
      if (r < HS_PATCH) {
         if (tb.bin0[r] == 8 * b && tb.w0[r] != 0.0f) w = tb.w0[r];
         else if (tb.bin1[r] == 8 * b) w = tb.w1[r];
      }
      s_cw[tid] = w;
      __syncthreads();
   }
   float cwc[16];
#pragma unroll
   for (int j = 0; j < 16; j++) cwc[j] = s_cw[cb_c * 16 + j];
   const uint32_t n = io.h_hi - io.h_lo;
   float *acc = s_acc + tid;
   typedef __attribute__((address_space(3))) float lds_float;
   const uint32_t acc_base = (uint32_t)(uintptr_t)(lds_float *)acc;
   __shared__ __attribute__((aligned(16))) float4 s_rows[16 * (HS_VO_DIM / 2)];
   __shared__ uint16_t s_vtab[HS_VO_DIM * (HS_VO_DIM / 2)];
   for (int q = tid; q < HS_VO_DIM * (HS_VO_DIM / 2); q += 64) {
      const int r = q / (HS_VO_DIM / 2), f = q - r * (HS_VO_DIM / 2);
      const int4 rw = tb.vo_rows[r];
      s_vtab[q] = (uint16_t)((f >= rw.y && f <= rw.z) ? rw.x + f : HS_VO_ZERO);
   }
   __syncthreads();
   int st_kq[5];
   const uint16_t *st_tab[5];
#pragma unroll
   for (int u = 0; u < 5; u++) {
      const int e = tid + 64 * u, row16 = e / (HS_VO_DIM / 2);
      st_kq[u] = row16 >> 2;
      st_tab[u] = s_vtab + 8 * (row16 & 3) * (HS_VO_DIM / 2) + (e - row16 * (HS_VO_DIM / 2));
   }
   const float4 *my_rows = s_rows + (4 * kq + cb_r) * (HS_VO_DIM / 2) + 4 * cb_c;
   for (uint32_t g = blockIdx.x; 4 * g < n; g += gridDim.x) {
      const uint32_t k = 4 * g + kq;
      const bool valid = k < n && io.alive[io.h_lo + min(k, n - 1)];
#pragma unroll
      for (int b = 0; b < 8; b++) acc[64 * b] = 0.0f;
      const float4 *g4 = reinterpret_cast<const float4 *>(vo + (size_t)(4 * g) * HS_VO_PITCH);
      const int kmax = (int)min(3u, n - 1 - 4 * g);
      int st_src[5];
#pragma unroll
      for (int u = 0; u < 5; u++) st_src[u] = min(st_kq[u], kmax) * HS_VO_ITEMS;
      auto item_at = [&](int u, int i) { return st_src[u] + (int)st_tab[u][i * (HS_VO_DIM / 2)]; };
      float4 st0 = g4[item_at(0, 0)], st1 = g4[item_at(1, 0)], st2 = g4[item_at(2, 0)], st3 = g4[item_at(3, 0)],
             st4 = g4[item_at(4, 0)];
      auto step = [&](int i, float4 &a0, float4 &a1, float4 &a2, float4 &a3, float4 &a4) {
         HS_WAVE_LDS_SYNC();
         s_rows[tid] = a0; s_rows[tid + 64] = a1; s_rows[tid + 128] = a2; s_rows[tid + 192] = a3; s_rows[tid + 256] = a4;
         HS_WAVE_LDS_SYNC();
         {
            const int in = min(i + HS_HIST_AHEAD, 15);
            a0 = g4[item_at(0, in)]; a1 = g4[item_at(1, in)]; a2 = g4[item_at(2, in)]; a3 = g4[item_at(3, in)];
            a4 = g4[item_at(4, in)];
         }
         if (valid) {
            float4 cur[8];
#pragma unroll
            for (int m = 0; m < 8; m++) cur[m] = my_rows[m];
            const float wr = s_cw[cb_r * 16 + i];
#pragma unroll
            for (int j = 0; j < 16; j++) {
               const float qx = (j & 1) ? cur[j >> 1].z : cur[j >> 1].x;
               const float qy = (j & 1) ? cur[j >> 1].w : cur[j >> 1].y;
               const float wc = cwc[j] * qx;
               const float v = wr * wc;
               const float wo1 = __builtin_amdgcn_fractf(qy);
               const float wo0 = 1.0f - wo1;
               const uint32_t x8 = (uint32_t)(int)qy << 8;
               lds_float *p0 = (lds_float *)(uintptr_t)((x8 & 0x700u) | acc_base);
               lds_float *p1 = (lds_float *)(uintptr_t)(((x8 + 0x100u) & 0x700u) | acc_base);
               const float t0 = v * wo0, t1 = v * wo1;
               const float a0 = *p0, a1 = *p1;
               *p0 = a0 + t0;
               *p1 = a1 + t1;
            }
         }
      };
#pragma unroll 1
      for (int i = 0; i < 16; i++) step(i, st0, st1, st2, st3, st4);
      if (k < n) {
         float4 *dst = reinterpret_cast<float4 *>(io.vec + (size_t)k * 128 + cell * 8);
         dst[0] = make_float4(acc[0], acc[64], acc[128], acc[192]);
         dst[1] = make_float4(acc[256], acc[320], acc[384], acc[448]);
      }
   }
}

__global__ __launch_bounds__(64) void k_sift_quantize(SiftIO io, DConsts kc)
{
   __shared__ float s_t[SM_TILE * 129];
   const int lane = threadIdx.x;
   const uint32_t n = io.h_hi - io.h_lo;
   const uint32_t k0 = blockIdx.x * SM_TILE;
   for (int k = 0; k < SM_TILE; k++) {
      const uint32_t kp = min(k0 + k, n - 1);
      s_t[k * 129 + lane] = io.vec[(size_t)kp * 128 + lane];
      s_t[k * 129 + 64 + lane] = io.vec[(size_t)kp * 128 + 64 + lane];
   }
   __syncthreads();
   float *v = s_t + lane * 129;
   {
      float vectlen = 0.0f;
      for (int i = 0; i < 128; i++) { const float x = v[i]; vectlen += x * x; }
      vectlen = sqrtf(vectlen);
      const float fac = 1.0f / vectlen;
      bool changed = false;
      for (int i = 0; i < 128; i++) {
         float x = v[i] * fac;
         if (x > kc.maxBinValue) { x = kc.maxBinValue; changed = true; }
         v[i] = x;
      }
      if (changed) {
         float l2 = 0.0f;
         for (int i = 0; i < 128; i++) { const float x = v[i]; l2 += x * x; }
         l2 = sqrtf(l2);
         const float f2 = 1.0f / l2;
         for (int i = 0; i < 128; i++) v[i] *= f2;
      }
      for (int i = 0; i < 128; i++) {
         const float q = 512.0f * v[i];
         int bq = (q == q) ? (int)q : 0;
         v[i] = (float)min(bq, 255);
      }
   }
   __syncthreads();
   for (int k = 0; k < SM_TILE; k++) {
      const uint32_t kp = k0 + k;
      if (kp >= n) break;
      const uint32_t h = io.h_lo + kp;
      if (!io.alive[h]) continue;
      if (lane < 32) {
         const float *r = s_t + k * 129 + 4 * lane;
         const uint32_t w = (uint32_t)r[0] | ((uint32_t)r[1] << 8) | ((uint32_t)r[2] << 16) | ((uint32_t)r[3] << 24);
         *reinterpret_cast<uint32_t *>(io.desc + (size_t)h * 128 + 4 * lane) = w;
      }
   }
}
```

hesaff_amd/csrc/pipeline.hip:

```cpp
#include <hip/hip_runtime.h>
#include <algorithm>
#include <atomic>
#include <chrono>
#include <cmath>
#include <cstdio>
#include <cstdlib>
#include <cstring>
#include <string>
#include <vector>
#include <condition_variable>
#include <deque>
#include <future>
#include <map>
#include <memory>
#include <mutex>
#include <thread>

#include "../../include/hesaff_amd.h"
#include "host_tables.h"
#include "kernels_keypoint.h"
#include "kernels_patch.h"
#include "kernels_sift.h"
#include "kernels_pyramid.h"
#include "kernels_export.h"
// ... 44 lines not shown
   HsError(int c, const std::string &m) : code(c), msg(m) {}
};

static void hs_wait_event(hipEvent_t ev)
{
   timespec t0;
   clock_gettime(CLOCK_MONOTONIC, &t0);
   for (int tries = 0;; tries++) {
      const hipError_t e = hipEventQuery(ev);
      if (e == hipSuccess) return;
      if (e != hipErrorNotReady) throw HsError(HESAFF_ERR_DEVICE, std::string("hipEventQuery: ") + hipGetErrorString(e));
      (void)hipGetLastError();
      if (tries < 16) continue;
      timespec now;
      clock_gettime(CLOCK_MONOTONIC, &now);
      const long long waited = (long long)(now.tv_sec - t0.tv_sec) * 1000000000ll + (now.tv_nsec - t0.tv_nsec);
      const timespec nap = {0, (long)std::min<long long>(std::max<long long>(waited / 8, 20000), 200000)};
      nanosleep(&nap, nullptr);
   }
}

static double thread_cpu_ms()
{
   timespec ts;
   clock_gettime(CLOCK_THREAD_CPUTIME_ID, &ts);
   return (double)ts.tv_sec * 1e3 + (double)ts.tv_nsec * 1e-6;
}

struct DevBuf {
   void *p = nullptr;
   size_t bytes = 0;
   DevBuf() = default;
   DevBuf(const DevBuf &) = delete;
   DevBuf &operator=(const DevBuf &) = delete;
   DevBuf(DevBuf &&o) noexcept : p(o.p), bytes(o.bytes) { o.p = nullptr; o.bytes = 0; }
   DevBuf &operator=(DevBuf &&o) noexcept
   {
      if (this != &o) { release(); p = o.p; bytes = o.bytes; o.p = nullptr; o.bytes = 0; }
      return *this;
   }
   ~DevBuf() { release(); }
   void ensure(size_t need)
   {
      if (need <= bytes) return;
      void *q = nullptr;
      hipError_t e = hipMalloc(&q, need);
      if (e != hipSuccess && p) {
         (void)hipGetLastError();
         (void)hipFree(p);
         p = nullptr; bytes = 0;
         e = hipMalloc(&q, need);
      }
      if (e != hipSuccess) {
         (void)hipGetLastError();
         if (p) (void)hipFree(p);
         p = nullptr; bytes = 0;
         char buf[256];
         snprintf(buf, sizeof buf, "hipMalloc(%zu bytes) failed: %s", need, hipGetErrorString(e));
         throw HsError(HESAFF_ERR_NOMEM, buf);
      }
      if (p) (void)hipFree(p);
      p = q;
      bytes = need;
   }
   void ensure_grow(size_t need)
   {
      if (need <= bytes) return;
      try { ensure(need + need / 8); }
      catch (const HsError &) { ensure(need); }
   }
   void release()
   {
      if (p) (void)hipFree(p);
      p = nullptr;
      bytes = 0;
   }
   template <class T> T *as() const { return (T *)p; }
};

struct PinBuf {
   void *p = nullptr;
   size_t bytes = 0;
   PinBuf() = default;
   PinBuf(const PinBuf &) = delete;
   PinBuf &operator=(const PinBuf &) = delete;
   PinBuf(PinBuf &&o) noexcept : p(o.p), bytes(o.bytes) { o.p = nullptr; o.bytes = 0; }
   PinBuf &operator=(PinBuf &&o) noexcept
   {
      if (this != &o) { release(); p = o.p; bytes = o.bytes; o.p = nullptr; o.bytes = 0; }
      return *this;
   }
   ~PinBuf() { release(); }
   void release() { if (p) (void)hipHostFree(p); p = nullptr; bytes = 0; }
   hipError_t replace(size_t cap)
   {
      release();
      const hipError_t e = hipHostMalloc(&p, cap, hipHostMallocDefault);
      if (e != hipSuccess) p = nullptr; else bytes = cap;
      return e;
   }
   void ensure(size_t need)
   {
      if (need <= bytes) return;
      const hipError_t e = replace(need);
      if (e != hipSuccess) throw HsError(HESAFF_ERR_NOMEM, std::string("hipHostMalloc failed: ") + hipGetErrorString(e));
   }
   void ensure_grow(size_t need)
   {
      if (need <= bytes) return;
      ensure((need + need / 4 + ((size_t)2 << 20) - 1) & ~(((size_t)2 << 20) - 1));
   }
   void *ensure_small(size_t need)
   {
      if (need > bytes && replace(std::max<size_t>(need * 2, 4096)) != hipSuccess)
         throw HsError(HESAFF_ERR_NOMEM, "hipHostMalloc failed (small result block)");
      return p;
   }
};

struct DevEvent {
   hipEvent_t e = nullptr;
   DevEvent() = default;
   explicit DevEvent(unsigned flags) { HIP_TRY(hipEventCreateWithFlags(&e, flags)); }
   DevEvent(const DevEvent &) = delete;
   DevEvent &operator=(const DevEvent &) = delete;
   DevEvent(DevEvent &&o) noexcept : e(o.e) { o.e = nullptr; }
   DevEvent &operator=(DevEvent &&o) noexcept
   {
      if (this != &o) { reset(); e = o.e; o.e = nullptr; }
      return *this;
   }
   ~DevEvent() { reset(); }
   void reset() { if (e) (void)hipEventDestroy(e); e = nullptr; }
   operator hipEvent_t() const { return e; }
};

struct OctGeom {
   int rows, cols, pitch;
   long long word_base;
   int words_per_row;
};

static inline int round_up(int v, int m) { return (v + m - 1) / m * m; }

#define HS_NSIDE 4
#define HS_LARGE_NW 2
#define HS_LARGE_SPLIT 1280
#define HS_AFF_BLOCKS_PER_CU 8
#define HS_GRID_LOC 1024
#define HS_GRID_DED 512
#define HS_GRID_SCAT 1024
#define HS_GRID_PACK 3584
#define HS_MID_CAP 6
#define HS_BIG_CAP 4
#define HS_OVERSUB 128u
#define HS_NSLOT 3
struct StreamSet { hipStream_t comp[4] = {nullptr, nullptr, nullptr, nullptr}; hipStream_t h2d = nullptr, d2h = nullptr; };
static std::mutex g_sets_mu;
static std::map<int, std::vector<StreamSet>> g_idle_sets;
static bool take_stream_set(int device, StreamSet &out)
{
   std::lock_guard<std::mutex> lk(g_sets_mu);
   std::vector<StreamSet> &v = g_idle_sets[device];
   if (v.empty()) return false;
   out = v.back();
   v.pop_back();
   return true;
}
static void give_stream_set(int device, const StreamSet &s)
{
   std::lock_guard<std::mutex> lk(g_sets_mu);
   g_idle_sets[device].push_back(s);
}

struct hesaff_ctx {
   hesaff_params par;
   int device = 0;
   StreamSet sset;
   hipStream_t stream = nullptr;
   std::string err;
   hesaff::OctaveSchedule sched;
   DConsts consts;

   DevBuf t_smm, t_sift, t_bin0, t_bin1, t_w0, t_w1, t_pyr_taps, t_patch_taps, t_patch_off, t_patch_k;
   int pyr_K[5];
   int pyr_tap_off[5];
   bool pyr_march = false;
   int max_p0 = 0;
   int batch_max_p = 0;
   int n_masked = 0;
   KpTables tables;

   int up = 0;
   int B = 0, H = 0, W = 0;
   std::vector<OctGeom> oct;
   long long words_per_image = 0;
   uint32_t cap = 0;
   uint32_t cand_cap = 0;
   bool map_clean = false;
   int map_kbits = 32;
   uint32_t map_epoch = 0;

   struct GeomBufs {
      DevBuf b_gray, b_up, b_L, b_L3, b_R, b_map, b_bitmask, b_prefix, b_blocksums;
      DevBuf b_cand, b_rec_f, b_rec_i, b_rec_w, b_hess_f, b_hess_i, b_aff, b_pw, b_bins, b_rank, b_desc, b_out, b_starts;
   } geo;
   DevBuf b_generic;
   std::vector<DPlane> L;
   DPlane gray, upimg, L3, R[5];
   DevBuf b_counters;
   DevBuf b_patches, b_stage;
   DevBuf b_input;
   DevBuf b_in2[2], b_outstage[2];
   PinBuf pin_in[2];
   PinBuf pin_reg[2];
   DevBuf b_reg[2];
   struct PinReadCache {
      static constexpr size_t kLargest = (size_t)64 << 20;
      size_t max_bytes = (size_t)4 << 30;
      size_t keep_bytes = (size_t)1 << 30;
      std::mutex mu;
      std::vector<std::pair<void *, size_t>> parked;
      size_t bytes_total = 0;
      int device = 0;
      void *take(size_t bytes)
      {
         if (bytes == 0 || bytes > kLargest) return nullptr;
         std::vector<std::pair<void *, size_t>> evicted;
         bool room = false;
         {
            std::lock_guard<std::mutex> lk(mu);
            for (size_t k = 0; k < parked.size(); k++)
               if (parked[k].second == bytes) { void *q = parked[k].first; parked[k] = parked.back(); parked.pop_back(); return q; }
            while (bytes_total + bytes > max_bytes && !parked.empty()) {
               evicted.push_back(parked.back());
               bytes_total -= parked.back().second;
               parked.pop_back();
            }
            room = bytes_total + bytes <= max_bytes;
            if (room) bytes_total += bytes;
         }
         for (auto &b : evicted) (void)hipHostFree(b.first);
         if (!room) return nullptr;
         void *q = nullptr;
         if (hipSetDevice(device) != hipSuccess || hipHostMalloc(&q, bytes, hipHostMallocDefault) != hipSuccess) {
            (void)hipGetLastError();
            std::lock_guard<std::mutex> lk(mu);
            bytes_total -= bytes;
            return nullptr;
         }
         return q;
      }
      void give(void *q, size_t bytes)
      {
         std::lock_guard<std::mutex> lk(mu);
         parked.emplace_back(q, bytes);
      }
      void trim(size_t keep)
      {
         std::vector<std::pair<void *, size_t>> out;
         {
            std::lock_guard<std::mutex> lk(mu);
            size_t held = 0;
            for (auto &b : parked) held += b.second;
            while (held > keep && !parked.empty()) {
               out.push_back(parked.back());
               held -= parked.back().second; bytes_total -= parked.back().second;
               parked.pop_back();
            }
         }
         for (auto &b : out) (void)hipHostFree(b.first);
      }
      ~PinReadCache() { trim(0); }
   } pin_read;
   DevEvent ev_h2d_blk[2];
   std::vector<PinBuf> pin_out;
   hesaff_engine::BlockRing ring;
   hipStream_t h2d_stream = nullptr, d2h_stream = nullptr;
   DevEvent ev_exp[2][4];
   float export_ms = 0.0f; int32_t export_rows = 0;
   DevEvent ev_h2d[2], ev_in_free[2], ev_out_ready[2], ev_d2h[2];
   PinBuf h_small_end, h_small_mid, h_small_exp;
   int32_t *h_starts = nullptr;
   DevBuf t_mask_idx, t_sgrad_nb, t_sgrad_om, t_vo_rows, t_vo_src, b_rowprefix, b_trows, b_trows2, b_trows3;
   DevBuf b_jcoef[2], b_jplane;
   DevBuf b_ex_len, b_ex_sums, b_ex_off, b_ex_imgoff, b_ex_starts;
   size_t rows_lds_set = 0;
   int n_cu = 256;
   uint32_t g_small0 = 256 * 6, g_small1 = 256 * 4, g_mid = HS_MID_BLOCKS, g_big = HS_BIG_BLOCKS, g_lfin = 256 * 4, g_shist = 256 * 32;
   uint32_t sgrad_grid = 256 * 32;
   uint32_t trows_rows = 4u << 20;

   hesaff_timings tm;
   int profiling = 0;
   int out_format = HESAFF_OUT_TEXT;
   int resume = 0;
   int pool_priority = -1;
   int stage_threads = 4;
   hipStream_t side_streams[HS_NSIDE] = {nullptr, nullptr, nullptr, nullptr};
   hipStream_t sift_stream = nullptr;
   hipStream_t aff_stream = nullptr;
   DevEvent ev_detect_done, ev_batch_done;
   std::vector<DevEvent> ev_aff;
   DevEvent ev_extract_done[HS_NSLOT], ev_sift_done[HS_NSLOT];
   DevBuf b_patches2[HS_NSLOT];
   DevBuf b_siftvec2, b_meanvar2, b_siftvo2;
   DevEvent ev_fork, ev_join[HS_NSIDE];
   bool fast_pyramid = false;
   bool no_overlap = false;
   bool debug = false;

   std::vector<DevEvent> ev_pool;
   size_t ev_used = 0;
};

namespace {

struct EvPair { hipEvent_t a, b; int kind; double bytes; };

hipEvent_t get_event(hesaff_ctx *c)
{
   if (c->ev_used == c->ev_pool.size()) c->ev_pool.emplace_back(hipEventDefault);
   return c->ev_pool[c->ev_used++];
}

template <class T> void upload(DevBuf &b, const std::vector<T> &v)
{
   b.ensure(std::max<size_t>(v.size() * sizeof(T), 16));
   HIP_TRY(hipMemcpy(b.p, v.data(), v.size() * sizeof(T), hipMemcpyHostToDevice));
}

void build_tables(hesaff_ctx *c)
{
   std::vector<float> smm(HS_SMM_PIX), sm(HS_PATCH_PIX), w0(HS_PATCH), w1(HS_PATCH);
   std::vector<int32_t> b0(HS_PATCH), b1(HS_PATCH);
   hesaff::gauss_mask(HS_SMM, smm.data());
   hesaff::circ_gauss_mask(HS_PATCH, sm.data());
   hesaff::sift_bins(b0.data(), b1.data(), w0.data(), w1.data());
   {
      std::vector<int32_t> midx;
      for (int i = 0; i < HS_PATCH_PIX; i++)
         if (sm[i] > 0) midx.push_back(i);
      c->n_masked = (int)midx.size();
      upload(c->t_mask_idx, midx);
      std::vector<int32_t> nb(4 * 1280, 0), om(2 * 1280, 0);
      for (size_t s = 0; s < 1280; s++) {
         const bool used = s < midx.size();
         const int i = used ? midx[s] : 0, r = i / HS_PATCH, cc = i - r * HS_PATCH;
         const bool valid = used && r < HS_PATCH - 1 && cc < HS_PATCH - 1;
         if (valid) {
            nb[4 * s + 0] = 4 * (cc == 0 ? i : i - 1);
            nb[4 * s + 1] = 4 * (i + 1);
            nb[4 * s + 2] = 4 * (r == 0 ? i : i - HS_PATCH);
            nb[4 * s + 3] = 4 * (i + HS_PATCH);
         }
         om[2 * s + 0] = valid ? r * (HS_PATCH - 1) + cc : -1;
         memcpy(&om[2 * s + 1], &sm[i], 4);
      }
      upload(c->t_sgrad_nb, nb); upload(c->t_sgrad_om, om);
      std::vector<int32_t> vrow(4 * HS_VO_DIM, 0);
      std::vector<uint16_t> vsrc(HS_VO_ITEMS, 0);
      int at = 0;
      for (int r = 0; r < HS_VO_DIM; r++) {
         int flo = 1, fhi = 0;
         for (int cc = 0; cc < HS_VO_DIM; cc++)
            if (sm[r * HS_PATCH + cc] > 0) { if (fhi < flo) flo = cc / 2; fhi = cc / 2; }
         vrow[4 * r + 0] = at - flo; vrow[4 * r + 1] = flo; vrow[4 * r + 2] = fhi;
         for (int f = flo; f <= fhi; f++, at++)
            if (at < HS_VO_ITEMS) vsrc[(size_t)at] = (uint16_t)(r * (HS_VO_DIM / 2) + f);
      }
      if (at != HS_VO_ZERO || sm[0] > 0) throw HsError(HESAFF_ERR_ARG, "internal: gradient-pair layout does not match the circular mask");
      upload(c->t_vo_rows, vrow); upload(c->t_vo_src, vsrc);
   }
   upload(c->t_smm, smm); upload(c->t_sift, sm); upload(c->t_bin0, b0); upload(c->t_bin1, b1); upload(c->t_w0, w0); upload(c->t_w1, w1);
   c->up = c->par.upscaleInputImage > 0 ? 1 : 0;
   c->sched = hesaff::make_schedule(c->par.initialSigma, c->up != 0);
   std::vector<float> taps;
   for (int i = 0; i < 5; i++) {
      const float sigma = i == 0 ? c->sched.init_sigma : c->sched.blur_sigma[i];
      c->pyr_tap_off[i] = (int)taps.size();
      taps.resize(taps.size() + 256, 0.0f);
      if (i == 0 && !(c->sched.init_sigma > 0.0f)) { c->pyr_K[0] = 0; continue; }
      const int K = hesaff::gauss_ksize(sigma);
      if (K > 255) throw HsError(HESAFF_ERR_ARG, "initialSigma too large (a pyramid blur would need more than 255 taps)");
      c->pyr_K[i] = K;
      if (K == 1) taps[c->pyr_tap_off[i]] = 1.0f;
      else hesaff::gauss_taps(K, sigma, taps.data() + c->pyr_tap_off[i]);
   }
   c->pyr_march = c->pyr_K[1] == 9 && c->pyr_K[2] == 11 && c->pyr_K[3] == 13 && c->pyr_K[4] == 15;
   upload(c->t_pyr_taps, taps);
   const hesaff_params &p = c->par;
   DConsts &k = c->consts;
   k.edgeScoreThreshold = (p.edgeEigenValueRatio + 1.0f) * (p.edgeEigenValueRatio + 1.0f) / p.edgeEigenValueRatio;
   k.finalThreshold = p.threshold * p.threshold;
   k.positiveThreshold = (float)(0.8 * k.finalThreshold);
   k.negativeThreshold = -k.positiveThreshold;
   k.convergenceThreshold = p.convergenceThreshold;
   k.affInitialSigma = 1.6f;
   k.mrSize = p.mrSize;
   k.maxBinValue = p.maxBinValue;
   k.maxIterations = p.maxIterations;
   k.pd0 = c->up ? 0.5f : 1.0f;
}

void ensure_patch_taps(hesaff_ctx *c, int max_p0)
{
   if (max_p0 <= c->max_p0) return;
   if ((max_p0 & 1) == 0) max_p0++;
   std::vector<float> taps;
   std::vector<int32_t> off((max_p0 + 1) / 2), kk((max_p0 + 1) / 2);
   for (int P0 = 1; P0 <= max_p0; P0 += 2) {
      const float scale = (float)P0 / (float)HS_PATCH;
      const float sigma = 1.5f * scale;
      const int K = hesaff::gauss_ksize(sigma);
      off[(P0 - 1) / 2] = (int32_t)taps.size();
      kk[(P0 - 1) / 2] = K;
      taps.resize(taps.size() + K);
      if (K == 1) taps[taps.size() - 1] = 1.0f;
      else hesaff::gauss_taps(K, sigma, taps.data() + off[(P0 - 1) / 2]);
   }
   upload(c->t_patch_taps, taps); upload(c->t_patch_off, off); upload(c->t_patch_k, kk);
   c->max_p0 = max_p0;
}

void refresh_tables_struct(hesaff_ctx *c)
{
   KpTables &t = c->tables;
   t.smm_mask = c->t_smm.as<float>(); t.sift_mask = c->t_sift.as<float>();
   t.bin0 = c->t_bin0.as<int32_t>(); t.bin1 = c->t_bin1.as<int32_t>();
   t.w0 = c->t_w0.as<float>(); t.w1 = c->t_w1.as<float>();
   t.patch_taps = c->t_patch_taps.as<float>(); t.patch_tap_off = c->t_patch_off.as<int32_t>(); t.patch_tap_k = c->t_patch_k.as<int32_t>();
   t.max_p0 = c->max_p0;
   t.mask_idx = c->t_mask_idx.as<int32_t>();
   t.sgrad_nb = c->t_sgrad_nb.as<int4>(); t.sgrad_om = c->t_sgrad_om.as<int2>();
   t.vo_rows = c->t_vo_rows.as<int4>(); t.vo_src = c->t_vo_src.as<uint16_t>();
   t.n_masked = c->n_masked;
}

DPlane make_plane(float *p, int rows, int cols, int pitch)
{
   DPlane d;
   d.p = p; d.rows = rows; d.cols = cols; d.pitch = pitch; d.img_stride = (long long)rows * pitch;
   return d;
}

template <class KERNEL> void set_dyn_lds(KERNEL kern, size_t lds)
{
   HIP_TRY(hipFuncSetAttribute((const void *)kern, hipFuncAttributeMaxDynamicSharedMemorySize, (int)lds));
}

size_t small_extract_lds_bytes(int bin) { return (size_t)(bin == 0 ? SmallGeom<0>::FLOATS : SmallGeom<1>::FLOATS) * 4; }
size_t mid_lds_bytes() { return (size_t)MidGeom<HS_MID_PMAX>::FLOATS * 4; }
size_t big_lds_bytes() { return (size_t)MidGeom<HS_BIN3_PMAX>::FLOATS * 4; }

constexpr size_t HS_LDS_PER_CU = 160 * 1024;
struct LargeGeom { int srow_stride, tap_stride; size_t lds; };
LargeGeom large_geom(int pmax)
{
   LargeGeom g;
   g.srow_stride = round_up((int)(pmax * 1.23) + 16, 64);
   g.tap_stride = round_up((int)(pmax * 0.22) + 8, 64);
   g.lds = (size_t)4 * (g.srow_stride + g.tap_stride) * 4;
   return g;
}

template <class KERNEL> uint32_t resident_grid(hesaff_ctx *c, KERNEL kern, int threads, size_t dyn_lds, uint32_t fallback_per_cu)
{
   int nb = 0;
   if (hipOccupancyMaxActiveBlocksPerMultiprocessor(&nb, (const void *)kern, threads, dyn_lds) != hipSuccess || nb < 1) {
      (void)hipGetLastError();
      nb = (int)fallback_per_cu;
   }
   return (uint32_t)c->n_cu * (uint32_t)nb;
}

void set_kernel_attrs(hesaff_ctx *c)
{
   set_dyn_lds(k_patch_extract_small<0>, small_extract_lds_bytes(0));
   set_dyn_lds(k_patch_extract_small<1>, small_extract_lds_bytes(1));
   set_dyn_lds(k_patch_mid<HS_MID_PMAX>, mid_lds_bytes());
   set_dyn_lds(k_patch_mid<HS_BIN3_PMAX>, big_lds_bytes());
   hipDeviceProp_t prop;
   HIP_TRY(hipGetDeviceProperties(&prop, c->device));
   c->n_cu = std::max(1, prop.multiProcessorCount);
   c->g_small0 = resident_grid(c, k_patch_extract_small<0>, 256, small_extract_lds_bytes(0), 6);
   c->g_small1 = resident_grid(c, k_patch_extract_small<1>, 256, small_extract_lds_bytes(1), 4);
   c->g_mid = std::min<uint32_t>(resident_grid(c, k_patch_mid<HS_MID_PMAX>, 256, mid_lds_bytes(), HS_MID_CAP), HS_MID_BLOCKS);
   c->g_big = std::min<uint32_t>(resident_grid(c, k_patch_mid<HS_BIN3_PMAX>, 256, big_lds_bytes(), HS_BIG_CAP), HS_BIG_BLOCKS);
   c->g_lfin = resident_grid(c, k_patch_large_finish, 256, 0, 4);
   c->g_shist = resident_grid(c, k_sift_hist, 64, 0, 32);
   c->sgrad_grid = (uint32_t)c->n_cu * 32u;
   c->g_small0 *= HS_OVERSUB; c->g_small1 *= HS_OVERSUB; c->g_shist *= HS_OVERSUB;
}

void plan_buffers(hesaff_ctx *c, int B, int H, int W);
void plan(hesaff_ctx *c, int B, int H, int W)
{
   try {
      plan_buffers(c, B, H, W);
   } catch (const HsError &e) {
      if (e.code == HESAFF_ERR_NOMEM) {
         (void)hipStreamSynchronize(c->stream);
         c->geo = hesaff_ctx::GeomBufs();
         c->map_clean = false;
      }
      throw;
   }
}

void plan_buffers(hesaff_ctx *c, int B, int H, int W)
{
   if (B <= c->B && H == c->H && W == c->W) return;
   if (H < 1 || W < 1 || (H << c->up) > 65535 || (W << c->up) > 65535) throw HsError(HESAFF_ERR_ARG, "image size out of range (1..65535 at the first pyramid level)");
   const int PH = H << c->up, PW = W << c->up;
   c->B = c->H = c->W = 0;
   c->oct.clear();
   c->L.clear();
   long long words = 0;
   size_t L_floats = 0;
   {
      int r = PH, cc = PW;
      const int minSize = 2 * HS_BORDER + 2;
      while (r > minSize && cc > minSize) {
         OctGeom g;
         g.rows = r; g.cols = cc; g.pitch = round_up(cc, 64);
         g.words_per_row = (cc + 63) / 64;
         g.word_base = words;
         words += (long long)HS_NSCALES * r * g.words_per_row;
         L_floats += (size_t)3 * B * r * g.pitch;
         c->oct.push_back(g);
         r /= 2; cc /= 2;
         if ((int)c->oct.size() >= HS_MAX_OCTAVES) break;
      }
   }
   c->words_per_image = words;
   const int pitch0 = round_up(W, 64);
   const size_t plane0 = (size_t)B * H * pitch0;
   c->geo.b_gray.ensure(plane0 * 4);
   c->gray = make_plane(c->geo.b_gray.as<float>(), H, W, pitch0);
   c->geo.b_L.ensure(std::max<size_t>(L_floats * 4, 16));
   {
      float *p = c->geo.b_L.as<float>();
      for (const OctGeom &g : c->oct)
         for (int l = 0; l < 3; l++) {
            c->L.push_back(make_plane(p, g.rows, g.cols, g.pitch));
            p += (size_t)B * g.rows * g.pitch;
         }
   }
   const int ppitch0 = round_up(PW, 64);
   const size_t pplane0 = (size_t)B * PH * ppitch0;
   if (c->up) {
      c->geo.b_up.ensure(pplane0 * 4);
      c->upimg = make_plane(c->geo.b_up.as<float>(), PH, PW, ppitch0);
   }
   c->geo.b_L3.ensure(pplane0 * 4);
   c->geo.b_R.ensure(pplane0 * 4 * 5);
   {
      const void *before = c->geo.b_map.p;
      const size_t before_bytes = c->geo.b_map.bytes;
      c->geo.b_map.ensure(std::max<size_t>((size_t)B * PH * PW * 4, 16));
      if (c->geo.b_map.p != before || c->geo.b_map.bytes != before_bytes) c->map_clean = false;
      int kb = 1;
      while (kb < 32 && (3ull * (unsigned long long)PH * PW) > (1ull << kb)) kb++;
      if (kb != c->map_kbits) { c->map_kbits = kb; c->map_clean = false; }
   }
   const long long total_words = (long long)B * words;
   c->geo.b_bitmask.ensure(std::max<size_t>((size_t)total_words * 8, 16));
   c->geo.b_prefix.ensure(std::max<size_t>((size_t)(total_words + 1) * 4, 16));
   double mpx = (double)B * PH * PW / 1.0e6;
   double capd = mpx * (double)c->par.max_kpts_per_mpx;
   if (capd < 4096) capd = 4096;
   if (capd > 2.0e9) throw HsError(HESAFF_ERR_ARG, "batch too large for 32-bit keypoint indices");
   c->cap = ((uint32_t)capd + 63u) & ~63u;
   const size_t cap = c->cap;
   const long long scan_items = std::max<long long>(total_words, (long long)cap);
   c->geo.b_blocksums.ensure((size_t)((scan_items + SCAN_BLOCK - 1) / SCAN_BLOCK + 1) * 4);
   c->b_counters.ensure(64 * 4);
   {
      const unsigned long long waves0 = (unsigned long long)((PW + EXM_STRIP - 1) / EXM_STRIP) * (unsigned long long)(PH / 32 + 1) * (unsigned long long)B;
      const unsigned long long cc = (unsigned long long)cap + (unsigned long long)cap / 8 + HS_CAND_BLOCK * waves0;
      if (cc > 0xfffffff0ull) throw HsError(HESAFF_ERR_ARG, "batch too large for 32-bit candidate indices");
      c->cand_cap = (uint32_t)cc;
      c->geo.b_cand.ensure((size_t)cc * sizeof(CandRec));
   }
   c->geo.b_rec_f.ensure(cap * 4 * 4);
   c->geo.b_rec_i.ensure(cap * 4 * 4);
   c->geo.b_rec_w.ensure(cap * 8);
   c->geo.b_hess_f.ensure(cap * 4 * 4);
   c->geo.b_hess_i.ensure(cap * 2 * 4);
   c->geo.b_aff.ensure(cap * 6 * 4);
   c->geo.b_pw.ensure(cap * 6 * 4);
   c->geo.b_bins.ensure(cap * HS_NBINS * 4);
   c->geo.b_rank.ensure((cap + 1) * 4);
   c->geo.b_desc.ensure(cap * 128);
   c->geo.b_out.ensure(cap * sizeof(KeyRec));
   c->geo.b_starts.ensure(((size_t)(B + 1) * 3 + 2) * 4);
   const int max_p0 = (int)std::floor(std::sqrt((double)W * (double)H)) + 3;
   ensure_patch_taps(c, max_p0);
   refresh_tables_struct(c);
   c->b_trows2.ensure((size_t)HS_MID_BLOCKS * (HS_MID_PMAX + 2 * HS_MID_RPAD) * HS_NEED * 4);
   c->b_trows3.ensure((size_t)HS_BIG_BLOCKS * (HS_BIN3_PMAX + 2 * HS_BIG_RPAD) * HS_NEED * 4);
   {
      const LargeGeom lg = large_geom(c->max_p0 + 2);
      if (lg.lds / 4 > HS_LDS_PER_CU) throw HsError(HESAFF_ERR_ARG, "image too large for the large-window row kernel (sqrt(width x height) above about 27900)");
      const size_t want = std::min<size_t>(lg.lds + (size_t)8 * lg.srow_stride * 4, HS_LDS_PER_CU);
      if (want > c->rows_lds_set) {
         set_dyn_lds(k_patch_large_rows, want);
         c->rows_lds_set = want;
      }
   }
   c->B = B; c->H = H; c->W = W;
}

template <class LOAD> void exclusive_scan(hesaff_ctx *c, LOAD load, long long n, uint32_t *out, uint32_t *total)
{
   if (n <= 0) { HIP_TRY(hipMemsetAsync(total, 0, 4, c->stream)); return; }
   const int nb = (int)((n + SCAN_BLOCK - 1) / SCAN_BLOCK);
   uint32_t *bs = c->geo.b_blocksums.as<uint32_t>();
   hipLaunchKernelGGL(k_scan_reduce<LOAD>, dim3(nb), dim3(256), 0, c->stream, load, n, bs);
   hipLaunchKernelGGL(k_scan_sums, dim3(1), dim3(256), 0, c->stream, bs, nb, total);
   hipLaunchKernelGGL(k_scan_down<LOAD>, dim3(nb), dim3(256), 0, c->stream, load, n, bs, out);
}

struct StageTimer {
   hesaff_ctx *c;
   std::vector<EvPair> pairs;
   std::vector<hipStream_t> streams;
   explicit StageTimer(hesaff_ctx *ctx) : c(ctx) {}
   int begin(int kind, double bytes = 0, hipStream_t st = nullptr)
   {
      if (!c->profiling) return -1;
      if (kind >= 100 && c->profiling < 2) return -1;
      if (!st) st = c->stream;
      EvPair p; p.a = get_event(c); p.b = get_event(c); p.kind = kind; p.bytes = bytes;
      (void)hipEventRecord(p.a, st);
      pairs.push_back(p);
      streams.push_back(st);
      return (int)pairs.size() - 1;
   }
   void end(int id) { if (id >= 0) (void)hipEventRecord(pairs[id].b, streams[id]); }
};

enum { T_PYR = 0, T_DET = 1, T_AFF = 2, T_PATCH = 3, T_SIFT = 4, T_TOTAL = 5, T_PACK = 6, T_BLURHESS = 100, T_EXTREMA = 101 };

template <int K, bool WL, bool WR, bool WH, bool WR0 = false, int SRC = SRC_PLANE>
void launch_march(hesaff_ctx *c, const DPlane &in, const DPlane &outL, const DPlane &outR, const DPlane &outHalf, const float *taps,
                  float norm2, int B, const DPlane &outR0 = DPlane(), float norm2_in = 0.0f, const GraySrc &gs = GraySrc(), const DPlane &outGray = DPlane())
{
   const int strips = (in.cols + BM_STRIP - 1) / BM_STRIP;
   const long long blocks_per_band = (long long)((strips + 3) / 4) * B;
   int best_nb = 16 * (int)std::max<long long>(1, std::min<long long>(4, 64 / std::max<long long>(1, blocks_per_band)));
   best_nb = std::max(1, std::min(best_nb, std::max(1, in.rows / 8)));
   const int band = (in.rows + best_nb - 1) / best_nb;
   if (c->debug) fprintf(stderr, "[hesaff] march K=%d %dx%d B=%d bands=%d band=%d blocks=%lld\n", K, in.cols, in.rows, B, best_nb, band, blocks_per_band * best_nb);
   const dim3 grid((strips + 3) / 4, (in.rows + band - 1) / band, B);
   hipLaunchKernelGGL((k_blur_hess_march<K, WL, WR, WH, WR0, SRC>), grid, dim3(256), 0, c->stream, in, outL, outR, outHalf, taps, norm2, band, outR0, norm2_in, gs, outGray);
}

template <bool WL, bool WR, bool WH>
void launch_blur_hess(hesaff_ctx *c, const DPlane &in, const DPlane &outL, const DPlane &outR, const DPlane &outHalf, const float *taps, int K,
                      float norm2, int B)
{
   switch (K) {
      case 9: launch_march<9, WL, WR, WH>(c, in, outL, outR, outHalf, taps, norm2, B); return;
      case 11: launch_march<11, WL, WR, WH>(c, in, outL, outR, outHalf, taps, norm2, B); return;
      case 13: launch_march<13, WL, WR, WH>(c, in, outL, outR, outHalf, taps, norm2, B); return;
      case 15: launch_march<15, WL, WR, WH>(c, in, outL, outR, outHalf, taps, norm2, B); return;
      default: break;
   }
   if (K <= 2 * BH_RMAX + 1) {
      const dim3 grid((in.cols + BH_TW - 1) / BH_TW, (in.rows + BH_TH - 1) / BH_TH, B);
      hipLaunchKernelGGL((k_blur_hess_tile<WL, WR, WH>), grid, dim3(256), 0, c->stream, in, outL, outR, outHalf, taps, K, norm2);
      return;
   }
   const size_t planeF = (size_t)B * in.rows * in.pitch;
   c->b_generic.ensure(planeF * 4 * 2);
   const DPlane tmp = make_plane(c->b_generic.as<float>(), in.rows, in.cols, in.pitch);
   const DPlane blurred = WL ? outL : make_plane(c->b_generic.as<float>() + planeF, in.rows, in.cols, in.pitch);
   const dim3 grid((in.cols + 255) / 256, in.rows, B);
   hipLaunchKernelGGL(k_blur_rows_generic, grid, dim3(256), 0, c->stream, in, tmp, taps, K);
   hipLaunchKernelGGL(k_blur_cols_generic, grid, dim3(256), 0, c->stream, tmp, blurred, taps, K);
   if (WR) hipLaunchKernelGGL(k_hess, grid, dim3(256), 0, c->stream, blurred, outR, norm2);
   if (WH) hipLaunchKernelGGL(k_half, dim3((outHalf.cols + 255) / 256, outHalf.rows, B), dim3(256), 0, c->stream, blurred, outHalf);
}

enum SrcFormat { HS_SRC_U8C1 = 0, HS_SRC_U8C3 = 1, HS_SRC_F32 = 2 };
struct SrcImages {
   const uint8_t *p;
   int format;
   long long img_stride;
   int row_stride;
   int channels() const { return format == HS_SRC_U8C3 ? 3 : 1; }
   static SrcImages u8(const void *p, int channels, long long img_stride, int row_stride)
   {
      return SrcImages{(const uint8_t *)p, channels == 3 ? HS_SRC_U8C3 : HS_SRC_U8C1, img_stride, row_stride};
   }
   static SrcImages f32(const void *p, long long img_stride, int row_stride) { return SrcImages{(const uint8_t *)p, HS_SRC_F32, img_stride, row_stride}; }
};

struct Lists {
   CandList cl;
   RecList rl;
   HessList hl;
   AffineOut ao;
   PatchWork pw;
   uint32_t *counters;
};

Lists make_lists(hesaff_ctx *c)
{
   Lists s;
   uint32_t *cnt = c->b_counters.as<uint32_t>();
   const size_t cap = c->cap;
   s.counters = cnt;
   s.cl.count = cnt + 0; s.cl.items = c->geo.b_cand.as<CandRec>(); s.cl.cap = c->cand_cap; s.cl.overflow = cnt + 2;
   s.rl.count = cnt + 1; s.rl.cap = c->cap;
   float *rf = c->geo.b_rec_f.as<float>();
   s.rl.x = rf; s.rl.y = rf + cap; s.rl.s = rf + 2 * cap; s.rl.response = rf + 3 * cap;
   uint32_t *ri = c->geo.b_rec_i.as<uint32_t>();
   s.rl.meta = (int32_t *)ri; s.rl.cell = ri + cap; s.rl.key = ri + 2 * cap; s.rl.bit = ri + 3 * cap;
   s.rl.word = c->geo.b_rec_w.as<long long>();
   float *hf = c->geo.b_hess_f.as<float>();
   s.hl.x = hf; s.hl.y = hf + cap; s.hl.s = hf + 2 * cap; s.hl.response = hf + 3 * cap;
   int32_t *hi = c->geo.b_hess_i.as<int32_t>();
   s.hl.meta = hi; s.hl.r0c0 = hi + cap; s.hl.cap = c->cap;
   int32_t *ai = c->geo.b_aff.as<int32_t>();
   s.ao.converged = ai; s.ao.iters = ai + cap; s.ao.U = (float *)(ai + 2 * cap);
   int32_t *pi = c->geo.b_pw.as<int32_t>();
   s.pw.P0 = pi; s.pw.alive = pi + cap; s.pw.A = (float *)(pi + 2 * cap);
   s.pw.bin_count = cnt + 8; s.pw.bin_work = cnt + 24; s.pw.bin_items = c->geo.b_bins.as<uint32_t>(); s.pw.cap = c->cap;
   return s;
}

void run_patch_stage(hesaff_ctx *c, const Lists &s, const DPlane &image, float *patches_out, uint32_t h_base, uint32_t large_rows_bound,
                     const PlaneTab *pt = nullptr)
{
   hipStream_t st = c->stream;
   PatchIO io;
   memset(&io, 0, sizeof io);
   io.image = image;
   io.patches = patches_out;
   io.h_base = h_base;
   if (c->fast_pyramid && pt) {
      hipStream_t s0 = st;
      const bool forked = c->side_streams[0] && !c->no_overlap;
      if (forked) {
         HIP_TRY(hipEventRecord(c->ev_fork, st));
         HIP_TRY(hipStreamWaitEvent(c->side_streams[0], c->ev_fork, 0));
         s0 = c->side_streams[0];
      }
      hipLaunchKernelGGL(k_patch_extract_small<0>, dim3(c->g_small0), dim3(256), small_extract_lds_bytes(0), s0, s.hl, s.pw, io, c->tables);
      if (forked) HIP_TRY(hipEventRecord(c->ev_join[0], s0));
      hipLaunchKernelGGL(k_patch_pyramid, dim3((uint32_t)c->n_cu * 32u), dim3(256), 0, st, s.hl, s.pw, io, *pt, (int)c->oct.size(), c->consts.pd0, 1);
      if (forked) HIP_TRY(hipStreamWaitEvent(st, c->ev_join[0], 0));
      return;
   }
   hipStream_t s0 = st, s1 = st, s2 = st, s3 = st;
   const bool forked = c->side_streams[0] && !c->no_overlap;
   if (forked) {
      HIP_TRY(hipEventRecord(c->ev_fork, st));
      for (int i = 0; i < HS_NSIDE; i++) HIP_TRY(hipStreamWaitEvent(c->side_streams[i], c->ev_fork, 0));
      s0 = c->side_streams[0]; s1 = c->side_streams[1]; s2 = c->side_streams[2]; s3 = c->side_streams[3];
   }
   {
      PatchIO io2 = io;
      io2.trows = c->b_trows2.as<float>();
      PatchIO io3 = io;
      io3.trows = c->b_trows3.as<float>();
      hipLaunchKernelGGL(k_patch_extract_small<0>, dim3(c->g_small0), dim3(256), small_extract_lds_bytes(0), s0, s.hl, s.pw, io, c->tables);
      hipLaunchKernelGGL(k_patch_extract_small<1>, dim3(c->g_small1), dim3(256), small_extract_lds_bytes(1), s1, s.hl, s.pw, io, c->tables);
      hipLaunchKernelGGL(k_patch_mid<HS_MID_PMAX>, dim3(c->g_mid), dim3(256), mid_lds_bytes(), s2, s.hl, s.pw, io2, c->tables);
      hipLaunchKernelGGL(k_patch_mid<HS_BIN3_PMAX>, dim3(c->g_big), dim3(256), big_lds_bytes(), s3, s.hl, s.pw, io3, c->tables);
   }
   if (large_rows_bound > 0) {
      const uint32_t rows_cap = std::max(large_rows_bound, c->trows_rows);
      c->b_trows.ensure((size_t)rows_cap * HS_NEED * 4);
      c->b_rowprefix.ensure(((size_t)c->cap + 1) * 4);
      const int pmax = std::min(c->max_p0 + 2, std::max(HS_BIN3_PMAX + 1, (c->batch_max_p > 0 ? c->batch_max_p : c->max_p0 + 2)));
      io.trows = c->b_trows.as<float>();
      io.row_prefix = c->b_rowprefix.as<uint32_t>();
      io.trows_cap = rows_cap;
      io.overflow = s.counters + 6;
      hipLaunchKernelGGL(k_large_prefix, dim3(1), dim3(256), 0, st, s.pw, c->b_rowprefix.as<uint32_t>());
      auto launch_rows = [&](int p_lo, int p_hi) {
         const LargeGeom lg = large_geom(std::min(c->max_p0 + 2, (p_hi + 255) / 256 * 256));
         const size_t wave1 = lg.lds / 4;
         const size_t wave3 = wave1 + (size_t)2 * lg.srow_stride * 4;
         const int nrow = wave3 * 6 <= HS_LDS_PER_CU ? 3 : 1;
         const size_t per_wave = nrow == 3 ? wave3 : wave1;
         uint32_t nw = 4;
         while (nw > 1 && per_wave * nw > HS_LDS_PER_CU) nw >>= 1;
         if (nw == 4 && (HS_LDS_PER_CU / (per_wave * 2)) * 2 > (HS_LDS_PER_CU / (per_wave * 4)) * 4) nw = 2;
         if (nrow == 3) nw = std::min<uint32_t>(nw, HS_LARGE_NW);
         const uint32_t gblocks = std::min<uint32_t>((large_rows_bound + nw * HS_LARGE_CHUNK - 1) / (nw * HS_LARGE_CHUNK), 256 * 16 * (4 / nw));
         hipLaunchKernelGGL(k_patch_large_rows, dim3(gblocks), dim3(64 * nw), per_wave * nw, st, s.hl, s.pw, io, c->tables, lg.srow_stride, lg.tap_stride, nrow,
                            p_lo, std::min(p_hi, 0x7ffffff0));
      };
      if (pmax > HS_LARGE_SPLIT) { launch_rows(0, HS_LARGE_SPLIT); launch_rows(HS_LARGE_SPLIT, pmax); }
      else launch_rows(0, pmax);
      hipLaunchKernelGGL(k_patch_large_finish, dim3(c->g_lfin), dim3(256), 0, st, s.pw, io, c->tables);
   }
   if (forked) {
      for (int i = 0; i < HS_NSIDE; i++) HIP_TRY(hipEventRecord(c->ev_join[i], c->side_streams[i]));
      for (int i = 0; i < HS_NSIDE; i++) HIP_TRY(hipStreamWaitEvent(st, c->ev_join[i], 0));
   }
}

void run_detection(hesaff_ctx *c, const SrcImages &src, int B, const Lists &s, StageTimer &tm, bool keep_all_planes, float *planes_out,
                   bool detect = true)
{
   const hesaff::OctaveSchedule &sc = c->sched;
   hipStream_t st = c->stream;
   uint32_t *cnt = s.counters;
   const float *ptaps = c->t_pyr_taps.as<float>();
   if (detect) {
      HIP_TRY(hipMemsetAsync(cnt, 0, 64 * 4, st));
      HIP_TRY(hipMemsetAsync(c->geo.b_bitmask.p, 0, std::max<size_t>((size_t)B * c->words_per_image * 8, 8), st));
      if (!c->map_clean) { HIP_TRY(hipMemsetAsync(c->geo.b_map.p, 0xFF, c->geo.b_map.bytes, st)); c->map_epoch = c->map_kbits < 32 ? (0xffffffffu >> c->map_kbits) : 0u; c->map_clean = true; }
   }

   int t = tm.begin(T_PYR);
   DPlane none = make_plane(nullptr, 0, 0, 0);
   const bool fused_gray = !c->oct.empty() && c->pyr_K[0] == 11 && !c->up;
   if (fused_gray) {
      GraySrc gs;
      gs.p = src.p; gs.channels = src.channels(); gs.img_stride = src.img_stride; gs.row_stride = src.row_stride;
      const int tb = tm.begin(T_BLURHESS, 0);
      if (src.format == HS_SRC_F32)
         launch_march<11, true, false, false, false, SRC_F32>(c, c->gray, c->L[0], none, none, ptaps + c->pyr_tap_off[0], 0.0f, B, DPlane(), 0.0f, gs, c->gray);
      else
         launch_march<11, true, false, false, false, SRC_U8>(c, c->gray, c->L[0], none, none, ptaps + c->pyr_tap_off[0], 0.0f, B, DPlane(), 0.0f, gs, c->gray);
      tm.end(tb);
   } else {
      const bool direct = c->pyr_K[0] == 0 && !c->oct.empty();
      if (src.format == HS_SRC_F32) {
         const size_t wb = (size_t)c->W * 4, dpitch = (size_t)c->gray.pitch * 4;
         if (src.img_stride == (long long)src.row_stride * c->H)
            HIP_TRY(hipMemcpy2DAsync(c->gray.p, dpitch, src.p, (size_t)src.row_stride, wb, (size_t)c->H * B, hipMemcpyDeviceToDevice, st));
         else
            for (int b = 0; b < B; b++)
               HIP_TRY(hipMemcpy2DAsync(c->gray.img(b), dpitch, src.p + (long long)b * src.img_stride, (size_t)src.row_stride, wb, (size_t)c->H,
                                        hipMemcpyDeviceToDevice, st));
      } else {
         const dim3 grid((c->W + 255) / 256, c->H, B);
         hipLaunchKernelGGL(k_gray, grid, dim3(256), 0, st, src.p, src.channels(), src.img_stride, src.row_stride, c->gray);
      }
      if (c->up) {
         const dim3 g2((c->upimg.cols + 255) / 256, c->upimg.rows, B);
         hipLaunchKernelGGL(k_double, g2, dim3(256), 0, st, c->gray, c->upimg);
      }
      const DPlane &first = c->up ? c->upimg : c->gray;
      if (direct) HIP_TRY(hipMemcpyAsync(c->L[0].p, first.p, (size_t)B * first.img_stride * 4, hipMemcpyDeviceToDevice, st));
      if (!c->oct.empty() && c->pyr_K[0] > 0) {
         const int tb = tm.begin(T_BLURHESS, 0);
         launch_blur_hess<true, false, false>(c, first, c->L[0], none, none, ptaps + c->pyr_tap_off[0], c->pyr_K[0], 0.0f, B);
         tm.end(tb);
      }
   }
   tm.end(t);
   float *pout = planes_out;
   for (size_t o = 0; o < c->oct.size(); o++) {
      const OctGeom &g = c->oct[o];
      const size_t planeF = (size_t)B * g.rows * g.pitch;
      DPlane Lo[5], Ro[5];
      for (int l = 0; l < 3; l++) Lo[l] = c->L[o * 3 + l];
      Lo[3] = make_plane(c->geo.b_L3.as<float>(), g.rows, g.cols, g.pitch);
      Lo[4] = none;
      if (keep_all_planes) Lo[4] = make_plane(c->b_stage.as<float>(), g.rows, g.cols, g.pitch);
      for (int l = 0; l < 5; l++) Ro[l] = make_plane(c->geo.b_R.as<float>() + l * planeF, g.rows, g.cols, g.pitch);
      t = tm.begin(T_PYR);
      const bool fuse_r0 = c->pyr_march;
      if (!fuse_r0 && detect) {
         const dim3 grid((g.cols + 255) / 256, g.rows, B);
         hipLaunchKernelGGL(k_hess, grid, dim3(256), 0, st, Lo[0], Ro[0], sc.norm2[0]);
      }
      const bool has_next = o + 1 < c->oct.size();
      for (int i = 1; i <= 4 && !detect; i++) {
         if (i == 4 || (i == 3 && !has_next)) break;
         const float *taps = ptaps + c->pyr_tap_off[i];
         const int tb = tm.begin(T_BLURHESS, (i == 3 ? 5.0 : 8.0) * (double)B * g.rows * g.cols);
         if (i < 3) launch_blur_hess<true, false, false>(c, Lo[i - 1], Lo[i], none, none, taps, c->pyr_K[i], 0.0f, B);
         else launch_blur_hess<false, false, true>(c, Lo[2], none, none, c->L[(o + 1) * 3], taps, c->pyr_K[i], 0.0f, B);
         tm.end(tb);
      }
      for (int i = 1; i <= 4 && detect; i++) {
         double bytes = 12.0 * (double)B * g.rows * g.cols;
         if (i == 1 && fuse_r0) bytes += 8.0 * (double)B * g.rows * g.cols;
         if (i == 3 && has_next) bytes += 2.0 * (double)B * g.rows * g.cols;
         const float *taps = ptaps + c->pyr_tap_off[i];
         const int K = c->pyr_K[i];
         const int tb = tm.begin(T_BLURHESS, bytes);
         if (i == 1 && fuse_r0) launch_march<9, true, true, false, true>(c, Lo[0], Lo[1], Ro[1], none, taps, sc.norm2[1], B, Ro[0], sc.norm2[0]);
         else if (i < 3) launch_blur_hess<true, true, false>(c, Lo[i - 1], Lo[i], Ro[i], none, taps, K, sc.norm2[i], B);
         else if (i == 3) {
            if (has_next) launch_blur_hess<true, true, true>(c, Lo[2], Lo[3], Ro[3], c->L[(o + 1) * 3], taps, K, sc.norm2[3], B);
            else launch_blur_hess<true, true, false>(c, Lo[2], Lo[3], Ro[3], none, taps, K, sc.norm2[3], B);
         } else {
            if (keep_all_planes) launch_blur_hess<true, true, false>(c, Lo[3], Lo[4], Ro[4], none, taps, K, sc.norm2[4], B);
            else launch_blur_hess<false, true, false>(c, Lo[3], none, Ro[4], none, taps, K, sc.norm2[4], B);
         }
         tm.end(tb);
      }
      tm.end(t);
      if (planes_out) {
         for (int l = 0; l < 5; l++) {
            HIP_TRY(hipMemcpy2DAsync(pout, (size_t)g.cols * 4, Lo[l].p, (size_t)g.pitch * 4, (size_t)g.cols * 4, g.rows, hipMemcpyDeviceToHost, st));
            pout += (size_t)g.rows * g.cols;
         }
         for (int l = 0; l < 5; l++) {
            HIP_TRY(hipMemcpy2DAsync(pout, (size_t)g.cols * 4, Ro[l].p, (size_t)g.pitch * 4, (size_t)g.cols * 4, g.rows, hipMemcpyDeviceToHost, st));
            pout += (size_t)g.rows * g.cols;
         }
      }
      if (!detect) continue;
      t = tm.begin(T_DET);
      HIP_TRY(hipMemsetAsync(cnt + 0, 0, 4, st));
      HIP_TRY(hipMemcpyAsync(cnt + 32 + o, cnt + 1, 4, hipMemcpyDeviceToDevice, st));
      OctaveCtx oc;
      for (int l = 0; l < 5; l++) { oc.R[l] = Ro[l]; oc.L[l] = Lo[l]; oc.sigma[l] = sc.level_sigma[l]; }
      oc.pixelDistance = c->consts.pd0 * (float)(1 << o);
      oc.octave = (int)o;
      oc.map = c->geo.b_map.as<uint32_t>();
      if (c->map_epoch == 0) { HIP_TRY(hipMemsetAsync(c->geo.b_map.p, 0xFF, c->geo.b_map.bytes, st)); c->map_epoch = c->map_kbits < 32 ? (0xffffffffu >> c->map_kbits) : 0u; }
      if (c->map_epoch > 0) c->map_epoch--;
      oc.map_epoch = c->map_kbits < 32 ? (c->map_epoch << c->map_kbits) : 0u;
      oc.word_base = g.word_base;
      oc.words_per_image = c->words_per_image;
      oc.words_per_row = g.words_per_row;
      if (g.rows > 2 * HS_BORDER && g.cols > 2 * HS_BORDER) {
         FivePlanes fp;
         for (int l = 0; l < 5; l++) fp.R[l] = Ro[l];
         const int strips = (g.cols + EXM_STRIP - 1) / EXM_STRIP;
         auto waves_at = [&](int rows_per_band) { return (long long)strips * ((g.rows + rows_per_band - 1) / rows_per_band) * B; };
         const int band = waves_at(128) >= 4096 ? 128 : (waves_at(64) >= 4096 ? 64 : 32);
         const dim3 grid(strips, (g.rows + band - 1) / band, B);
         const int te = tm.begin(T_EXTREMA, 20.0 * (double)B * g.rows * g.cols);
         hipLaunchKernelGGL(k_extrema_march, grid, dim3(64), 0, st, fp, c->consts.positiveThreshold, c->consts.negativeThreshold, s.cl, band);
         tm.end(te);
         hipLaunchKernelGGL(k_localize, dim3(HS_GRID_LOC), dim3(256), 0, st, oc, s.cl, s.rl, c->consts);
         hipLaunchKernelGGL(k_dedupe, dim3(HS_GRID_DED), dim3(256), 0, st, oc, s.rl, (const uint32_t *)(cnt + 32 + o),
                            c->geo.b_bitmask.as<unsigned long long>());
      }
      tm.end(t);
   }
   if (!detect) return;
   t = tm.begin(T_DET);
   const long long total_words = (long long)B * c->words_per_image;
   LoadPopc lp; lp.p = c->geo.b_bitmask.as<unsigned long long>();
   exclusive_scan(c, lp, total_words, c->geo.b_prefix.as<uint32_t>(), cnt + 3);
   HessItem *items = reinterpret_cast<HessItem *>(c->geo.b_cand.p);
   static_assert(sizeof(HessItem) == 32 && sizeof(CandRec) >= sizeof(HessItem), "the items fit the candidate slots (cand_cap >= cap)");
   hipLaunchKernelGGL(k_scatter_ordered, dim3(HS_GRID_SCAT), dim3(256), 0, st, s.rl, (const unsigned long long *)c->geo.b_bitmask.p,
                      (const uint32_t *)c->geo.b_prefix.p, items, s.hl.cap);
   hipLaunchKernelGGL(k_hess_deal, dim3(HS_GRID_SCAT), dim3(256), 0, st, (const HessItem *)items, (const uint32_t *)(cnt + 3), s.hl);
   hipLaunchKernelGGL(k_image_counts, dim3((B + 1 + 63) / 64), dim3(64), 0, st, (const uint32_t *)c->geo.b_prefix.p,
                      c->words_per_image, B, (const uint32_t *)(cnt + 3), c->geo.b_starts.as<int32_t>());
   HIP_TRY(hipMemsetAsync(c->geo.b_starts.as<int32_t>() + 2 * (B + 1), 0, (size_t)(B + 2) * 4, st));
   hipLaunchKernelGGL(k_image_large_rows, dim3(512), dim3(256), 0, st, s.hl, (const uint32_t *)(cnt + 3), c->consts.mrSize,
                      c->geo.b_starts.as<uint32_t>() + 2 * (B + 1), B, c->max_p0);
   tm.end(t);
}

__global__ void k_desc_starts(const int32_t *__restrict__ hess_starts, int nimg, const uint32_t *__restrict__ rank,
                              const uint32_t *__restrict__ n_hess, const uint32_t *__restrict__ total_desc, int32_t *__restrict__ out)
{
   const int b = blockIdx.x * blockDim.x + threadIdx.x;
   if (b > nimg) return;
   const uint32_t hs = (uint32_t)hess_starts[b];
   out[b] = (b == nimg || hs >= *n_hess) ? (int32_t)*total_desc : (int32_t)rank[hs];
}

void collect_timings(hesaff_ctx *c, StageTimer &tm, int B)
{
   hesaff_timings &t = c->tm;
   memset(&t, 0, sizeof t);
   for (const EvPair &p : tm.pairs) {
      float ms = 0;
      (void)hipEventElapsedTime(&ms, p.a, p.b);
      switch (p.kind) {
         case T_PYR: t.pyramid_ms += ms; break;
         case T_DET: t.detect_ms += ms; break;
         case T_AFF: t.affine_ms += ms; break;
         case T_PATCH: t.patch_ms += ms; break;
         case T_SIFT: t.sift_ms += ms; break;
         case T_PACK: t.pack_ms += ms; break;
         case T_TOTAL: t.total_ms += ms; break;
         case T_BLURHESS:
            if (p.bytes > 0) { t.blur_hess_ms += ms; t.blur_hess_launches++; t.blur_hess_bytes += p.bytes; }
            break;
         case T_EXTREMA: t.extrema_ms += ms; t.extrema_launches++; t.extrema_bytes += p.bytes; break;
      }
   }
   double sumN = 0;
   for (const OctGeom &g : c->oct) sumN += (double)g.rows * g.cols;
   t.pyramid_bytes = (double)B * (5.0 * c->H * c->W + 58.0 * sumN);
   t.export_ms = c->export_ms; t.export_rows = c->export_rows;
}

void launch_sift(hesaff_ctx *c, hipStream_t ss, const SiftIO &so, uint32_t n, float2 *vo)
{
   const uint32_t nb64 = (n + 63) / 64;
   hipLaunchKernelGGL(k_sift_meanvar, dim3((n + SM_KP - 1) / SM_KP), dim3(64), 0, ss, so, c->tables);
   hipLaunchKernelGGL(k_sift_grad, dim3(std::min(n, c->sgrad_grid)), dim3(256), 0, ss, so, c->tables, vo);
   hipLaunchKernelGGL(k_sift_hist, dim3(std::min<uint32_t>((n + 3) / 4, c->g_shist)), dim3(64), 0, ss, so, c->tables, (const float2 *)vo);
   hipLaunchKernelGGL(k_sift_quantize, dim3(nb64), dim3(64), 0, ss, so, c->consts);
}

void ensure_group_buffers(hesaff_ctx *c, uint32_t n)
{
   for (int slot = 0; slot < HS_NSLOT; slot++) c->b_patches2[slot].ensure_grow((size_t)n * HS_PATCH_PIX * 4);
   c->b_siftvec2.ensure_grow((size_t)n * 128 * 4);
   c->b_meanvar2.ensure_grow((size_t)n * 2 * 4);
   const void *before = c->b_siftvo2.p;
   const size_t bytes_before = c->b_siftvo2.bytes;
   c->b_siftvo2.ensure_grow((size_t)n * HS_VO_PITCH * 8 + 64);
   if (c->b_siftvo2.p != before || c->b_siftvo2.bytes != bytes_before) HIP_TRY(hipMemsetAsync(c->b_siftvo2.p, 0, c->b_siftvo2.bytes, c->stream));
}

const int32_t *fetch_hessian_starts(hesaff_ctx *c, int B)
{
   hipStream_t st = c->stream;
   int32_t *hs = (int32_t *)c->h_small_mid.ensure_small(((size_t)3 * (B + 1) + 1) * 4);
   HIP_TRY(hipMemcpyAsync(hs, c->geo.b_starts.p, ((size_t)3 * (B + 1) + 1) * 4, hipMemcpyDeviceToHost, st));
   HIP_TRY(hipEventRecord(c->ev_detect_done, st));
   const double dbg_ca = c->debug ? thread_cpu_ms() : 0.0;
   hs_wait_event(c->ev_detect_done);
   if (c->debug) fprintf(stderr, "[hesaff] run_batch: caller's CPU inside the wait for the detection stage %.2f ms\n", thread_cpu_ms() - dbg_ca);
   return hs;
}

void run_keypoint_stages(hesaff_ctx *c, const Lists &s, StageTimer &tm, int tt, int B, int H, int W, const int32_t *hs, bool with_affine)
{
   hipStream_t st = c->stream;
   uint32_t *cnt = s.counters;
   int t;
   PlaneTab pt;
   memset(&pt, 0, sizeof pt);
   uint32_t n_hess_host = 0;
   for (size_t o = 0; o < c->oct.size(); o++)
      for (int l = 0; l < 3; l++) pt.L[o][l] = c->L[o * 3 + l];
   {
      if ((uint32_t)hs[B] > c->cap) throw HsError(HESAFF_ERR_CAPACITY, "keypoint capacity exceeded; raise hesaff_params.max_kpts_per_mpx");
      n_hess_host = (uint32_t)hs[B];
      const uint32_t *lrows = (const uint32_t *)hs + 2 * (B + 1);
      c->batch_max_p = (int)lrows[B + 1];
      const uint32_t group_kpts = std::min<uint32_t>(std::max<uint32_t>((uint32_t)hs[B] / 16u, 300000u), 1200000u);
      struct Group { uint32_t lo, hi, large_rows; };
      std::vector<Group> groups;
      uint32_t max_n = 0;
      for (int g0 = 0; g0 < B;) {
         int g1 = g0 + 1;
         unsigned long long rows = lrows[g0];
         while (g1 < B && (uint32_t)(hs[g1 + 1] - hs[g0]) <= group_kpts && rows + lrows[g1] <= c->trows_rows) { rows += lrows[g1]; g1++; }
         if (rows > 0xffffffffull) throw HsError(HESAFF_ERR_NOMEM, "window rows of one image exceed 32 bits");
         if (hs[g1] > hs[g0]) {
            groups.push_back({(uint32_t)hs[g0], (uint32_t)hs[g1], (uint32_t)rows});
            max_n = std::max(max_n, (uint32_t)(hs[g1] - hs[g0]));
         }
         g0 = g1;
      }
      while (c->ev_aff.size() < groups.size()) c->ev_aff.emplace_back(hipEventDisableTiming);
      if (max_n) ensure_group_buffers(c, max_n);
      hipStream_t as = c->no_overlap ? st : c->aff_stream;
      if (as != st && with_affine) HIP_TRY(hipStreamWaitEvent(as, c->ev_detect_done, 0));
      auto launch_affine = [&](size_t gi) {
         if (!with_affine) return;
         const int ta = tm.begin(T_AFF, 0, as);
         const uint32_t agrid = std::min<uint32_t>((groups[gi].hi - groups[gi].lo + HS_AFFP_G - 1) / HS_AFFP_G, (uint32_t)c->n_cu * HS_AFF_BLOCKS_PER_CU);
         hipLaunchKernelGGL(k_affine, dim3(agrid), dim3(64), 0, as, pt, s.hl, groups[gi].lo, groups[gi].hi, (const uint32_t *)(cnt + 3), c->tables, c->consts, s.ao);
         tm.end(ta);
         if (as != st) HIP_TRY(hipEventRecord(c->ev_aff[gi], as));
      };
      if (!groups.empty()) launch_affine(0);
      bool slot_used[HS_NSLOT] = {};
      for (size_t gi = 0; gi < groups.size(); gi++) {
         const uint32_t h_lo = groups[gi].lo, h_hi = groups[gi].hi, n = h_hi - h_lo;
         if (gi + 1 < groups.size()) launch_affine(gi + 1);
         if (as != st && with_affine) HIP_TRY(hipStreamWaitEvent(st, c->ev_aff[gi], 0));
         const int slot = (int)(gi % HS_NSLOT);
         if (slot_used[slot]) HIP_TRY(hipStreamWaitEvent(st, c->ev_sift_done[slot], 0));
         t = tm.begin(T_PATCH);
         HIP_TRY(hipMemsetAsync(cnt + 8, 0, 24 * 4, st));
         hipLaunchKernelGGL(k_prepare_patch, dim3(1024), dim3(256), 0, st, s.hl, h_lo, h_hi, (const uint32_t *)(cnt + 3), s.ao, H, W, c->consts,
                            c->tables, s.pw);
         run_patch_stage(c, s, c->gray, c->b_patches2[slot].as<float>(), h_lo, groups[gi].large_rows, &pt);
         tm.end(t);
         HIP_TRY(hipEventRecord(c->ev_extract_done[slot], st));
         hipStream_t ss = c->no_overlap ? st : c->sift_stream;
         if (ss != st) HIP_TRY(hipStreamWaitEvent(ss, c->ev_extract_done[slot], 0));
         SiftIO so;
         so.patches = c->b_patches2[slot].as<float>(); so.alive = s.pw.alive; so.meanvar = c->b_meanvar2.as<float>();
         so.vec = c->b_siftvec2.as<float>(); so.desc = c->geo.b_desc.as<uint8_t>(); so.h_lo = h_lo; so.h_hi = h_hi;
         const int ts = tm.begin(T_SIFT, 0, ss);
         launch_sift(c, ss, so, n, c->b_siftvo2.as<float2>());
         tm.end(ts);
         HIP_TRY(hipEventRecord(c->ev_sift_done[slot], ss));
         slot_used[slot] = true;
      }
      for (int sl = 0; sl < HS_NSLOT; sl++)
         if (slot_used[sl]) HIP_TRY(hipStreamWaitEvent(st, c->ev_sift_done[sl], 0));
   }
   t = tm.begin(T_PACK);
   LoadFlagI32 lf; lf.p = s.pw.alive;
   exclusive_scan(c, lf, (long long)n_hess_host, c->geo.b_rank.as<uint32_t>(), cnt + 4);
   hipLaunchKernelGGL(k_pack, dim3(HS_GRID_PACK), dim3(256), 0, st, s.hl, (const uint32_t *)(cnt + 3), s.pw, (const uint32_t *)c->geo.b_rank.p,
                      (const uint8_t *)c->geo.b_desc.p, c->geo.b_out.as<KeyRec>());
   hipLaunchKernelGGL(k_desc_starts, dim3((B + 1 + 63) / 64), dim3(64), 0, st, (const int32_t *)c->geo.b_starts.p, B,
                      (const uint32_t *)c->geo.b_rank.p, (const uint32_t *)(cnt + 3), (const uint32_t *)(cnt + 4),
                      c->geo.b_starts.as<int32_t>() + (B + 1));
   tm.end(t);
   tm.end(tt);
   c->h_starts = (int32_t *)c->h_small_end.ensure_small(((size_t)2 * (B + 1) + 8) * 4);
   HIP_TRY(hipMemcpyAsync(c->h_starts, c->geo.b_starts.p, (size_t)2 * (B + 1) * 4, hipMemcpyDeviceToHost, st));
   HIP_TRY(hipMemcpyAsync(c->h_starts + 2 * (B + 1), cnt, 8 * 4, hipMemcpyDeviceToHost, st));
   HIP_TRY(hipEventRecord(c->ev_batch_done, st));
   const double dbg_cb = c->debug ? thread_cpu_ms() : 0.0;
   hs_wait_event(c->ev_batch_done);
   if (c->debug) fprintf(stderr, "[hesaff] run_batch: caller's CPU inside the wait for the end of the batch %.2f ms\n", thread_cpu_ms() - dbg_cb);
   HIP_TRY(hipGetLastError());
   if (c->profiling) collect_timings(c, tm, B);
   const int32_t *cn = c->h_starts + 2 * (B + 1);
   if (cn[2] != 0 || (uint32_t)cn[1] > c->cap)
      throw HsError(HESAFF_ERR_CAPACITY, "keypoint capacity exceeded; raise hesaff_params.max_kpts_per_mpx");
   if (cn[6] != 0) throw HsError(HESAFF_ERR_NOMEM, "large-window row buffer exceeded (internal bound violated)");
}

void run_batch(hesaff_ctx *c, const SrcImages &src, int B, int H, int W)
{
   plan(c, B, H, W);
   c->ev_used = 0;
   StageTimer tm(c);
   Lists s = make_lists(c);
   const int tt = tm.begin(T_TOTAL);
   run_detection(c, src, B, s, tm, false, nullptr);
   run_keypoint_stages(c, s, tm, tt, B, H, W, fetch_hessian_starts(c, B), true);
}

inline size_t describe_records_offset(int B) { return (((size_t)B + 1) * 4 + 255) & ~(size_t)255; }
void run_describe(hesaff_ctx *c, const SrcImages &src, int B, int H, int W, const uint8_t *d_block, uint32_t n_rec, int from)
{
   plan(c, B, H, W);
   if (n_rec > c->cap) throw HsError(HESAFF_ERR_CAPACITY, "more records than the keypoint capacity; raise hesaff_params.max_kpts_per_mpx");
   c->ev_used = 0;
   StageTimer tm(c);
   Lists s = make_lists(c);
   hipStream_t st = c->stream;
   uint32_t *cnt = s.counters;
   const bool shapes = from == HESAFF_FROM_SHAPES;
   const int tt = tm.begin(T_TOTAL);
   HIP_TRY(hipMemsetAsync(cnt, 0, 64 * 4, st));
   hipLaunchKernelGGL(k_ingest_regions, dim3(std::max<uint32_t>(1u, std::min<uint32_t>((std::max<uint32_t>(n_rec, (uint32_t)B + 1) + 255) / 256, 4096u))), dim3(256), 0, st,
                      (const uint4 *)(d_block + describe_records_offset(B)), n_rec, (const int32_t *)d_block, B, shapes ? 1 : 0, s.hl, s.ao,
                      cnt + 3, c->geo.b_starts.as<int32_t>());
   HIP_TRY(hipMemsetAsync(c->geo.b_starts.as<int32_t>() + 2 * (B + 1), 0, (size_t)(B + 2) * 4, st));
   hipLaunchKernelGGL(k_image_large_rows, dim3(512), dim3(256), 0, st, s.hl, (const uint32_t *)(cnt + 3), c->consts.mrSize,
                      c->geo.b_starts.as<uint32_t>() + 2 * (B + 1), B, c->max_p0);
   const int32_t *hs = fetch_hessian_starts(c, B);
   if (!shapes || c->fast_pyramid) {
      run_detection(c, src, B, s, tm, false, nullptr, false);
   } else {
      const dim3 grid((W + 1023) / 1024, H, B);
      if (src.format == HS_SRC_F32) hipLaunchKernelGGL(k_gray_plane<2>, grid, dim3(256), 0, st, src.p, src.img_stride, src.row_stride, c->gray);
      else if (src.format == HS_SRC_U8C3) hipLaunchKernelGGL(k_gray_plane<1>, grid, dim3(256), 0, st, src.p, src.img_stride, src.row_stride, c->gray);
      else hipLaunchKernelGGL(k_gray_plane<0>, grid, dim3(256), 0, st, src.p, src.img_stride, src.row_stride, c->gray);
   }
   HIP_TRY(hipEventRecord(c->ev_detect_done, st));
   run_keypoint_stages(c, s, tm, tt, B, H, W, hs, !shapes);
}

unsigned long long export_text_prepare(hesaff_ctx *c, const KeyRec *keys, uint32_t n, const int32_t *d_starts, int B,
                                       std::vector<unsigned long long> &img_off)
{
   img_off.assign((size_t)B + 1, 0ull);
   if (n == 0) return 0ull;
   hipStream_t st = c->stream;
   const uint32_t nblk = (n + EX_ROWS - 1) / EX_ROWS;
   c->b_ex_len.ensure_grow(((size_t)n + 64) * 2);
   c->b_ex_sums.ensure_grow((size_t)nblk * 4);
   c->b_ex_off.ensure_grow(((size_t)nblk + 1) * 8);
   c->b_ex_imgoff.ensure(((size_t)B + 1) * 8);
   hipLaunchKernelGGL(k_text_len, dim3((n + 255) / 256), dim3(256), 0, st, keys, n, c->par.mrSize, c->b_ex_len.as<uint16_t>(), c->b_ex_sums.as<uint32_t>());
   hipLaunchKernelGGL(k_text_scan, dim3(1), dim3(1024), 0, st, (const uint32_t *)c->b_ex_sums.p, nblk, c->b_ex_off.as<unsigned long long>());
   hipLaunchKernelGGL(k_text_imgoff, dim3((B + 1 + 63) / 64), dim3(64), 0, st, d_starts, B, (const uint16_t *)c->b_ex_len.p,
                      (const unsigned long long *)c->b_ex_off.p, c->b_ex_imgoff.as<unsigned long long>());
   unsigned long long *ho = (unsigned long long *)c->h_small_exp.ensure_small(((size_t)B + 1) * 8);
   HIP_TRY(hipMemcpyAsync(ho, c->b_ex_imgoff.p, ((size_t)B + 1) * 8, hipMemcpyDeviceToHost, st));
   HIP_TRY(hipEventRecord(c->ev_batch_done, st));
   hs_wait_event(c->ev_batch_done);
   HIP_TRY(hipGetLastError());
   memcpy(img_off.data(), ho, ((size_t)B + 1) * 8);
   return img_off[(size_t)B];
}

void export_text_write(hesaff_ctx *c, const KeyRec *keys, uint32_t n, char *d_text)
{
   if (n == 0) return;
   hipLaunchKernelGGL(k_text_write, dim3((n + EX_ROWS - 1) / EX_ROWS), dim3(EX_ROWS), 0, c->stream, keys, n, c->par.mrSize, (const uint16_t *)c->b_ex_len.p,
                      (const unsigned long long *)c->b_ex_off.p, d_text);
}

JpegGeom make_jpeg_geom(const hesaff_jpeg_layout &L)
{
   JpegGeom g;
   memset(&g, 0, sizeof g);
   if (L.width < 1 || L.height < 1 || L.width > 65535 || L.height > 65535 || (L.channels != 1 && L.channels != 3))
      throw HsError(HESAFF_ERR_ARG, "bad JPEG layout");
   g.W = L.width; g.H = L.height; g.nc = L.channels;
   unsigned long long coef = HESAFF_JPEG_BLOB_HEADER, plane = 0, blocks = 0;
   for (int i = 0; i < g.nc; i++) {
      const long long bw = L.bw[i], bh = L.bh[i], cw = L.cw[i], chgt = L.chgt[i], hx = L.hx[i], vx = L.vx[i];
      if (bw < 1 || bh < 1 || bw > 8192 || bh > 8192 || cw < 1 || chgt < 1 || cw > bw * 8 || chgt > bh * 8 || hx < 1 || hx > 4 || vx < 1 || vx > 4 ||
          cw * hx < L.width || chgt * vx < L.height || (g.nc == 1 && (hx != 1 || vx != 1)))
         throw HsError(HESAFF_ERR_ARG, "bad JPEG layout");
      g.bw[i] = (int)bw; g.bh[i] = (int)bh; g.cw[i] = (int)cw; g.chgt[i] = (int)chgt; g.hx[i] = (int)hx; g.vx[i] = (int)vx;
      g.mode[i] = (hx == 1 && vx == 1) ? JPEG_UP_NONE : (hx == 2 && vx == 1 && cw > 2) ? JPEG_UP_H2V1 : (hx == 2 && vx == 2 && cw > 2) ? JPEG_UP_H2V2
                  : (hx == 1 && vx == 2) ? JPEG_UP_H1V2 : JPEG_UP_REPLICATE;
      g.blocks[i] = (unsigned int)(bw * bh);
      g.coef_off[i] = coef; g.plane_off[i] = plane;
      coef += (unsigned long long)(bw * bh) * 128;
      plane += (unsigned long long)(bw * bh) * 64;
      blocks += (unsigned long long)(bw * bh);
   }
   if (blocks > 0x7fffffffull) throw HsError(HESAFF_ERR_ARG, "bad JPEG layout");
   g.blob_bytes = coef; g.plane_bytes = plane; g.blocks_per_image = (unsigned int)blocks;
   return g;
}

void jpeg_pixels(hesaff_ctx *c, const uint8_t *d_blobs, const JpegGeom &g, int B, uint8_t *d_out, size_t out_img_stride, hipStream_t st)
{
   if (B < 1) return;
   c->b_jplane.ensure_grow((size_t)g.plane_bytes * (size_t)B);
   const unsigned long long total = (unsigned long long)B * g.blocks_per_image;
   hipLaunchKernelGGL(k_jpeg_idct, dim3((unsigned)std::min<unsigned long long>((total + 255) / 256, 1u << 20)), dim3(256), 0, st, d_blobs,
                      c->b_jplane.as<uint8_t>(), g, B);
   hipLaunchKernelGGL(k_jpeg_pixels, dim3(((g.W + 3) / 4 + 255) / 256, g.H, B), dim3(256), 0, st, d_blobs, (const uint8_t *)c->b_jplane.as<uint8_t>(), d_out, g,
                      (unsigned long long)out_img_stride);
}

void export_bin_rows(hesaff_ctx *c, const KeyRec *keys, uint32_t n, char *d_bin)
{
   if (n == 0) return;
   hipLaunchKernelGGL(k_bin_rows, dim3(std::min<uint32_t>((n + 7) / 8, 4096u)), dim3(256), 0, c->stream, keys, n, c->par.mrSize, (uint32_t *)d_bin);
}

void pack_regions(hesaff_ctx *c, uint32_t n_hess, int B, hesaff_region *d_regions)
{
   static_assert(sizeof(hesaff_region) == 4 * HS_REGION_DW, "hesaff_region layout");
   if (n_hess == 0) return;
   if (n_hess > c->cap) throw HsError(HESAFF_ERR_CAPACITY, "keypoint capacity exceeded; raise hesaff_params.max_kpts_per_mpx");
   const Lists s = make_lists(c);
   RegionTab tab;
   for (int o = 0; o < HS_MAX_OCTAVES; o++) tab.pd[o] = c->consts.pd0 * (float)(1 << o);
   hipLaunchKernelGGL(k_pack_regions, dim3(std::min<uint32_t>((n_hess + 255) / 256, 4096u)), dim3(256), 0, c->stream, s.hl, n_hess, s.ao, s.pw,
                      (const uint32_t *)c->geo.b_rank.p, (const int32_t *)c->geo.b_starts.as<int32_t>() + (B + 1), tab, (uint4 *)d_regions);
}

}
#include "capi_impl.h"
```

Baseline: 38.64 million.

## Start SIFT on bin-0 patches early and rework quantize/meanvar kernels

```diff
diff --git a/hesaff_amd/csrc/capi_impl.h b/hesaff_amd/csrc/capi_impl.h
--- a/hesaff_amd/csrc/capi_impl.h
+++ b/hesaff_amd/csrc/capi_impl.h
@@ -158,6 +158,7 @@
       for (int i = 0; i < HS_NSLOT; i++) {
          c->ev_extract_done[i] = DevEvent(hipEventDisableTiming);
          c->ev_sift_done[i] = DevEvent(hipEventDisableTiming);
+         c->ev_bin0_done[i] = DevEvent(hipEventDisableTiming);
       }
       set_kernel_attrs(c);
       build_tables(c);
@@ -973,6 +974,7 @@
    plan(c, 1, rows, cols);
    if ((uint32_t)n > c->cap) throw HsError(HESAFF_ERR_CAPACITY, "too many keypoints for this image size");
    Lists s = make_lists(c);
+   ensure_work_lists(c, s, (uint32_t)n);
    hipStream_t st = c->stream;
    HIP_TRY(hipMemcpy2DAsync(c->gray.p, (size_t)c->gray.pitch * 4, img, (size_t)cols * 4, (size_t)cols * 4, rows, hipMemcpyHostToDevice, st));
    std::vector<float> x(n), y(n), sc(n);
diff --git a/hesaff_amd/csrc/hmath.h b/hesaff_amd/csrc/hmath.h
--- a/hesaff_amd/csrc/hmath.h
+++ b/hesaff_amd/csrc/hmath.h
@@ -190,7 +190,7 @@
    const int32_t hx = (int32_t)hm_f2u(x), hy = (int32_t)hm_f2u(y);
    const int32_t ix = hx & 0x7fffffff, iy = hy & 0x7fffffff;
    const int32_t k = (iy - ix) >> 23;
-   if ((ix >= 0x7f800000) | (iy >= 0x7f800000) | ((iy != 0) & (ix != 0) & ((k > 60) | (k < -60)))) return hm_atan2f_rare(y, x);
+   if (!ND && ((ix >= 0x7f800000) | (iy >= 0x7f800000) | ((iy != 0) & (ix != 0) & ((k > 60) | (k < -60))))) return hm_atan2f_rare(y, x);
    const float q = hm_fabsf(ND ? hm_div_normal(y, x) : y / x);
    const int32_t iq = (int32_t)hm_f2u(q);
    const int id = (int)(iq >= 0x3ee00000) + (int)(iq >= 0x3f300000) + (int)(iq >= 0x3f980000) + (int)(iq >= 0x401c0000);
@@ -208,7 +208,7 @@
    const float s1 = z * (aT0 + w * (aT2 + w * (aT4 + w * (aT6 + w * (aT8 + w * aT10)))));
    const float s2 = w * (aT1 + w * (aT3 + w * (aT5 + w * (aT7 + w * aT9))));
    float za = hi - ((xr * (s1 + s2) - lo) - xr);
-   za = (iq >= 0x4c000000) ? hm_u2f(0x3fc90fdau) + hm_u2f(0x33a22168u) : za;
+   if (!ND) za = (iq >= 0x4c000000) ? hm_u2f(0x3fc90fdau) + hm_u2f(0x33a22168u) : za;
    float r = (hx < 0) ? pi - (za - pi_lo) : za;
    r = (ix == 0) ? ((iy == 0) ? ((hx < 0) ? pi : 0.0f) : pi_o_2) : r;
    return hm_u2f(hm_f2u(r) ^ ((uint32_t)hy & 0x80000000u));
diff --git a/hesaff_amd/csrc/kernels_keypoint.h b/hesaff_amd/csrc/kernels_keypoint.h
--- a/hesaff_amd/csrc/kernels_keypoint.h
+++ b/hesaff_amd/csrc/kernels_keypoint.h
@@ -252,6 +252,8 @@
 
 #define HS_NBINS 5
 #define HS_BIN3_PMAX 512
+#define HS_NLISTS (HS_NBINS + 1)
+#define HS_LIST_REST HS_NBINS
 __host__ __device__ inline int hs_patch_bin(int P) { return P <= 41 ? 0 : (P <= 64 ? 1 : (P <= 128 ? 2 : (P <= HS_BIN3_PMAX ? 3 : 4))); }
 
 struct PatchWork {
@@ -317,6 +319,16 @@
          if (lane == leader) base = atomicAdd(pw.bin_count + bq, (uint32_t)__popcll(m));
          base = __shfl(base, leader, 64);
          if (bin == bq) pw.bin_items[(size_t)bq * pw.cap + base + (uint32_t)__popcll(m & ((1ull << lane) - 1ull))] = h;
+      }
+      {
+         const unsigned long long m = __ballot(bin >= 1);
+         if (m != 0ull) {
+            const int leader = __ffsll((long long)m) - 1;
+            uint32_t base = 0;
+            if (lane == leader) base = atomicAdd(pw.bin_count + HS_LIST_REST, (uint32_t)__popcll(m));
+            base = __shfl(base, leader, 64);
+            if (bin >= 1) pw.bin_items[(size_t)HS_LIST_REST * pw.cap + base + (uint32_t)__popcll(m & ((1ull << lane) - 1ull))] = h;
+         }
       }
    }
 }
diff --git a/hesaff_amd/csrc/kernels_sift.h b/hesaff_amd/csrc/kernels_sift.h
--- a/hesaff_amd/csrc/kernels_sift.h
+++ b/hesaff_amd/csrc/kernels_sift.h
@@ -8,7 +8,11 @@
    float *vec;
    uint8_t *desc;
    uint32_t h_lo, h_hi;
+   const uint32_t *items = nullptr;
+   const uint32_t *count = nullptr;
 };
+__device__ __forceinline__ uint32_t hs_sift_n(const SiftIO &io) { return io.items ? min(*io.count, io.h_hi - io.h_lo) : io.h_hi - io.h_lo; }
+__device__ __forceinline__ uint32_t hs_sift_k(const SiftIO &io, uint32_t i) { return io.items ? io.items[i] - io.h_lo : i; }
 
 #define HS_VO_DIM 40
 #define HS_VO_TILE (HS_VO_DIM * HS_VO_DIM)
@@ -16,7 +20,6 @@
 #define HS_VO_ZERO 642
 #define HS_VO_PITCH (2 * HS_VO_ITEMS)
 #define HS_SIFT_MSK_IT 5
-#define SM_TILE 64
 
 #define SM_KP 16
 #define SM_PX (64 * 64 / SM_KP)
@@ -26,11 +29,13 @@
 {
    __shared__ float s_tile[SM_KP * SM_ROW];
    const int lane = threadIdx.x;
-   const uint32_t n = io.h_hi - io.h_lo;
+   const uint32_t n = hs_sift_n(io);
    const uint32_t k0 = blockIdx.x * SM_KP;
+   if (k0 >= n) return;
    const int nm = tb.n_masked;
    const float gsum = (float)nm;
-   const uint32_t kmine = min(k0 + (uint32_t)min(lane, SM_KP - 1), n - 1);
+   const uint32_t kmine = hs_sift_k(io, min(k0 + (uint32_t)min(lane, SM_KP - 1), n - 1));
+   const bool mine = lane < SM_KP && k0 + lane < n;
    float sum = 0.0f, mean = 0.0f;
    for (int pass = 0; pass < 2; pass++) {
       float acc = 0.0f;
@@ -41,29 +46,28 @@
          for (int u = 0; u < SM_PX / 64; u++) pix[u] = (lane + 64 * u < cnt) ? tb.mask_idx[c0 + lane + 64 * u] : 0;
 #pragma unroll SM_UNROLL
          for (int k = 0; k < SM_KP; k++) {
-            const uint32_t kp = min(k0 + k, n - 1);
+            const uint32_t kp = (uint32_t)__builtin_amdgcn_readlane((int)kmine, k);
+            const float mk = __int_as_float(__builtin_amdgcn_readlane(__float_as_int(mean), k));
             const float *pp = io.patches + (size_t)kp * HS_PATCH_PIX;
 #pragma unroll
             for (int u = 0; u < SM_PX / 64; u++) {
                const float *q = pp + pix[u];
-               s_tile[k * SM_ROW + lane + 64 * u] = *q;
+               float x = *q;
+               if (pass) { const float d = mk - x; x = d * d; }
+               s_tile[k * SM_ROW + lane + 64 * u] = x;
             }
          }
          __syncthreads();
          if (lane < SM_KP) {
             const float *row = s_tile + lane * SM_ROW;
-            if (pass == 0) {
-               for (int l = 0; l < cnt; l++) acc += row[l];
-            } else {
-               for (int l = 0; l < cnt; l++) { const float d = mean - row[l]; acc += d * d; }
-            }
+            for (int l = 0; l < cnt; l++) acc += row[l];
          }
          __syncthreads();
       }
       if (pass == 0) { sum = acc; mean = sum / gsum; }
       else {
          const float var = sqrtf(acc / gsum);
-         if (lane < SM_KP && k0 + lane < n) { io.meanvar[2 * (size_t)kmine] = mean; io.meanvar[2 * (size_t)kmine + 1] = var; }
+         if (mine) { io.meanvar[2 * (size_t)kmine] = mean; io.meanvar[2 * (size_t)kmine + 1] = var; }
       }
    }
 }
@@ -74,7 +78,7 @@
    __shared__ float s_at[HM_ATAN_TAB_FLOATS];
    __shared__ __attribute__((aligned(16))) float2 s_vo[HS_VO_TILE];
    const int tid = threadIdx.x;
-   const uint32_t n = io.h_hi - io.h_lo;
+   const uint32_t n = hs_sift_n(io);
    for (int i = tid; i < HS_VO_TILE; i += 256) s_vo[i] = make_float2(0.0f, 0.0f);
    constexpr int VO_NI = (HS_VO_ITEMS + 255) / 256;
    int vsrc[VO_NI];
@@ -88,8 +92,10 @@
    int2 omq[HS_SIFT_MSK_IT];
 #pragma unroll
    for (int q = 0; q < HS_SIFT_MSK_IT; q++) { nbq[q] = tb.sgrad_nb[tid + 256 * q]; omq[q] = tb.sgrad_om[tid + 256 * q]; }
-   uint32_t k = blockIdx.x;
-   if (k >= n) return;
+   uint32_t i = blockIdx.x;
+   if (i >= n) return;
+   uint32_t k = hs_sift_k(io, i);
+   uint32_t kn = i + gridDim.x < n ? hs_sift_k(io, i + gridDim.x) : 0u;
    float pv[HS_PATCH_PIX_IT];
    int alive = io.alive[io.h_lo + k];
    float mean = io.meanvar[2 * (size_t)k], var = io.meanvar[2 * (size_t)k + 1];
@@ -98,7 +104,7 @@
 #pragma unroll
       for (int q = 0; q < HS_PATCH_PIX_IT; q++) pv[q] = gp[min(tid + 256 * q, HS_PATCH_PIX - 1)];
    }
-   for (; k < n; k += gridDim.x) {
+   for (; i < n; i += gridDim.x) {
       const bool cur_alive = alive != 0;
       const bool cur_norm = !((double)var < 0.0001);
       if (cur_alive) {
@@ -114,8 +120,8 @@
             }
          }
       }
-      const uint32_t kn = k + gridDim.x;
-      if (kn < n) {
+      const uint32_t knn = i + 2 * gridDim.x < n ? hs_sift_k(io, i + 2 * gridDim.x) : 0u;
+      if (i + gridDim.x < n) {
          alive = io.alive[io.h_lo + kn];
          mean = io.meanvar[2 * (size_t)kn]; var = io.meanvar[2 * (size_t)kn + 1];
          const float *gp = io.patches + (size_t)kn * HS_PATCH_PIX;
@@ -157,6 +163,7 @@
          }
       }
       __syncthreads();
+      k = kn; kn = knn;
    }
 }
 
@@ -199,7 +206,8 @@
    float cwc[16];
 #pragma unroll
    for (int j = 0; j < 16; j++) cwc[j] = s_cw[cb_c * 16 + j];
-   const uint32_t n = io.h_hi - io.h_lo;
+   const uint32_t n = hs_sift_n(io);
+   if (n == 0) return;
    float *acc = s_acc + tid;
    typedef __attribute__((address_space(3))) float lds_float;
    const uint32_t acc_base = (uint32_t)(uintptr_t)(lds_float *)acc;
@@ -220,17 +228,21 @@
       st_tab[u] = s_vtab + 8 * (row16 & 3) * (HS_VO_DIM / 2) + (e - row16 * (HS_VO_DIM / 2));
    }
    const float4 *my_rows = s_rows + (4 * kq + cb_r) * (HS_VO_DIM / 2) + 4 * cb_c;
-   for (uint32_t g = blockIdx.x; 4 * g < n; g += gridDim.x) {
-      const uint32_t k = 4 * g + kq;
-      const bool valid = k < n && io.alive[io.h_lo + min(k, n - 1)];
+   uint32_t g = blockIdx.x;
+   uint32_t kl = 4 * g < n ? hs_sift_k(io, min(4 * g + (uint32_t)(tid & 3), n - 1)) : 0u;
+   for (; 4 * g < n; g += gridDim.x) {
+      const uint32_t kcur = kl;
+      if (4 * (g + gridDim.x) < n) kl = hs_sift_k(io, min(4 * (g + gridDim.x) + (uint32_t)(tid & 3), n - 1));
+      const uint32_t k = (uint32_t)__shfl((int)kcur, kq, 64);
+      const bool in_list = 4 * g + kq < n;
+      const bool valid = in_list && io.alive[io.h_lo + k];
 #pragma unroll
       for (int b = 0; b < 8; b++) acc[64 * b] = 0.0f;
-      const float4 *g4 = reinterpret_cast<const float4 *>(vo + (size_t)(4 * g) * HS_VO_PITCH);
-      const int kmax = (int)min(3u, n - 1 - 4 * g);
-      int st_src[5];
-#pragma unroll
-      for (int u = 0; u < 5; u++) st_src[u] = min(st_kq[u], kmax) * HS_VO_ITEMS;
-      auto item_at = [&](int u, int i) { return st_src[u] + (int)st_tab[u][i * (HS_VO_DIM / 2)]; };
+      const float4 *g4 = reinterpret_cast<const float4 *>(vo);
+      size_t st_src[5];
+#pragma unroll
+      for (int u = 0; u < 5; u++) st_src[u] = (size_t)(uint32_t)__shfl((int)kcur, st_kq[u], 64) * HS_VO_ITEMS;
+      auto item_at = [&](int u, int i) { return st_src[u] + (size_t)st_tab[u][i * (HS_VO_DIM / 2)]; };
       float4 st0 = g4[item_at(0, 0)], st1 = g4[item_at(1, 0)], st2 = g4[item_at(2, 0)], st3 = g4[item_at(3, 0)],
              st4 = g4[item_at(4, 0)];
       auto step = [&](int i, float4 &a0, float4 &a1, float4 &a2, float4 &a3, float4 &a4) {
@@ -267,7 +279,7 @@
       };
 #pragma unroll 1
       for (int i = 0; i < 16; i++) step(i, st0, st1, st2, st3, st4);
-      if (k < n) {
+      if (in_list) {
          float4 *dst = reinterpret_cast<float4 *>(io.vec + (size_t)k * 128 + cell * 8);
          dst[0] = make_float4(acc[0], acc[64], acc[128], acc[192]);
          dst[1] = make_float4(acc[256], acc[320], acc[384], acc[448]);
@@ -275,52 +287,73 @@
    }
 }
 
+#define SQ_KP 32
 __global__ __launch_bounds__(64) void k_sift_quantize(SiftIO io, DConsts kc)
 {
-   __shared__ float s_t[SM_TILE * 129];
+   __shared__ float s_t[SQ_KP * 129];
+   __shared__ float s_f[SQ_KP];
+   __shared__ uint32_t s_k[SQ_KP];
    const int lane = threadIdx.x;
-   const uint32_t n = io.h_hi - io.h_lo;
-   const uint32_t k0 = blockIdx.x * SM_TILE;
-   for (int k = 0; k < SM_TILE; k++) {
-      const uint32_t kp = min(k0 + k, n - 1);
-      s_t[k * 129 + lane] = io.vec[(size_t)kp * 128 + lane];
-      s_t[k * 129 + 64 + lane] = io.vec[(size_t)kp * 128 + 64 + lane];
-   }
-   __syncthreads();
-   float *v = s_t + lane * 129;
-   {
+   const uint32_t n = hs_sift_n(io);
+   const uint32_t k0 = blockIdx.x * SQ_KP;
+   if (k0 >= n) return;
+   if (lane < SQ_KP) s_k[lane] = hs_sift_k(io, min(k0 + lane, n - 1));
+   __syncthreads();
+#pragma unroll 4
+   for (int k = 0; k < SQ_KP; k++) {
+      const float *src = io.vec + (size_t)s_k[k] * 128;
+      s_t[k * 129 + lane] = src[lane];
+      s_t[k * 129 + 64 + lane] = src[64 + lane];
+   }
+   __syncthreads();
+   if (lane < SQ_KP) {
+      const float *v = s_t + lane * 129;
       float vectlen = 0.0f;
+#pragma unroll 8
       for (int i = 0; i < 128; i++) { const float x = v[i]; vectlen += x * x; }
       vectlen = sqrtf(vectlen);
-      const float fac = 1.0f / vectlen;
-      bool changed = false;
-      for (int i = 0; i < 128; i++) {
-         float x = v[i] * fac;
-         if (x > kc.maxBinValue) { x = kc.maxBinValue; changed = true; }
-         v[i] = x;
-      }
-      if (changed) {
-         float l2 = 0.0f;
-         for (int i = 0; i < 128; i++) { const float x = v[i]; l2 += x * x; }
-         l2 = sqrtf(l2);
-         const float f2 = 1.0f / l2;
-         for (int i = 0; i < 128; i++) v[i] *= f2;
-      }
-      for (int i = 0; i < 128; i++) {
-         const float q = 512.0f * v[i];
-         int bq = (q == q) ? (int)q : 0;
-         v[i] = (float)min(bq, 255);
-      }
-   }
-   __syncthreads();
-   for (int k = 0; k < SM_TILE; k++) {
-      const uint32_t kp = k0 + k;
-      if (kp >= n) break;
-      const uint32_t h = io.h_lo + kp;
+      s_f[lane] = 1.0f / vectlen;
+   }
+   __syncthreads();
+   uint32_t changed = 0;
+#pragma unroll 4
+   for (int k = 0; k < SQ_KP; k++) {
+      const float fac = s_f[k];
+      float x0 = s_t[k * 129 + lane] * fac, x1 = s_t[k * 129 + 64 + lane] * fac;
+      const bool c0 = x0 > kc.maxBinValue, c1 = x1 > kc.maxBinValue;
+      if (c0) x0 = kc.maxBinValue;
+      if (c1) x1 = kc.maxBinValue;
+      s_t[k * 129 + lane] = x0;
+      s_t[k * 129 + 64 + lane] = x1;
+      if (__ballot(c0 || c1) != 0ull) changed |= 1u << k;
+   }
+   __syncthreads();
+   if (lane < SQ_KP && ((changed >> lane) & 1u)) {
+      const float *v = s_t + lane * 129;
+      float l2 = 0.0f;
+#pragma unroll 8
+      for (int i = 0; i < 128; i++) { const float x = v[i]; l2 += x * x; }
+      l2 = sqrtf(l2);
+      s_f[lane] = 1.0f / l2;
+   }
+   __syncthreads();
+   for (int k = 0; k < SQ_KP; k++) {
+      if (k0 + k >= n) break;
+      const uint32_t h = io.h_lo + s_k[k];
       if (!io.alive[h]) continue;
       if (lane < 32) {
          const float *r = s_t + k * 129 + 4 * lane;
-         const uint32_t w = (uint32_t)r[0] | ((uint32_t)r[1] << 8) | ((uint32_t)r[2] << 16) | ((uint32_t)r[3] << 24);
+         const bool resc = (changed >> k) & 1u;
+         const float f2 = s_f[k];
+         uint32_t w = 0;
+#pragma unroll
+         for (int j = 0; j < 4; j++) {
+            float x = r[j];
+            if (resc) x *= f2;
+            const float q = 512.0f * x;
+            const int bq = (q == q) ? (int)q : 0;
+            w |= (uint32_t)(float)min(bq, 255) << (8 * j);
+         }
          *reinterpret_cast<uint32_t *>(io.desc + (size_t)h * 128 + 4 * lane) = w;
       }
    }
diff --git a/hesaff_amd/csrc/pipeline.hip b/hesaff_amd/csrc/pipeline.hip
--- a/hesaff_amd/csrc/pipeline.hip
+++ b/hesaff_amd/csrc/pipeline.hip
@@ -370,7 +370,7 @@
    hipStream_t aff_stream = nullptr;
    DevEvent ev_detect_done, ev_batch_done;
    std::vector<DevEvent> ev_aff;
-   DevEvent ev_extract_done[HS_NSLOT], ev_sift_done[HS_NSLOT];
+   DevEvent ev_extract_done[HS_NSLOT], ev_sift_done[HS_NSLOT], ev_bin0_done[HS_NSLOT];
    DevBuf b_patches2[HS_NSLOT];
    DevBuf b_siftvec2, b_meanvar2, b_siftvo2;
    DevEvent ev_fork, ev_join[HS_NSIDE];
@@ -643,7 +643,7 @@
    const size_t cap = c->cap;
    const long long scan_items = std::max<long long>(total_words, (long long)cap);
    c->geo.b_blocksums.ensure((size_t)((scan_items + SCAN_BLOCK - 1) / SCAN_BLOCK + 1) * 4);
-   c->b_counters.ensure(64 * 4);
+   c->b_counters.ensure((64 + 32 * HS_NSLOT) * 4);
    {
       const unsigned long long waves0 = (unsigned long long)((PW + EXM_STRIP - 1) / EXM_STRIP) * (unsigned long long)(PH / 32 + 1) * (unsigned long long)B;
       const unsigned long long cc = (unsigned long long)cap + (unsigned long long)cap / 8 + HS_CAND_BLOCK * waves0;
@@ -658,7 +658,6 @@
    c->geo.b_hess_i.ensure(cap * 2 * 4);
    c->geo.b_aff.ensure(cap * 6 * 4);
    c->geo.b_pw.ensure(cap * 6 * 4);
-   c->geo.b_bins.ensure(cap * HS_NBINS * 4);
    c->geo.b_rank.ensure((cap + 1) * 4);
    c->geo.b_desc.ensure(cap * 128);
    c->geo.b_out.ensure(cap * sizeof(KeyRec));
@@ -796,12 +795,29 @@
    s.ao.converged = ai; s.ao.iters = ai + cap; s.ao.U = (float *)(ai + 2 * cap);
    int32_t *pi = c->geo.b_pw.as<int32_t>();
    s.pw.P0 = pi; s.pw.alive = pi + cap; s.pw.A = (float *)(pi + 2 * cap);
-   s.pw.bin_count = cnt + 8; s.pw.bin_work = cnt + 24; s.pw.bin_items = c->geo.b_bins.as<uint32_t>(); s.pw.cap = c->cap;
+   s.pw.bin_count = cnt + 8; s.pw.bin_work = cnt + 24; s.pw.bin_items = nullptr; s.pw.cap = 0;
    return s;
 }
 
-void run_patch_stage(hesaff_ctx *c, const Lists &s, const DPlane &image, float *patches_out, uint32_t h_base, uint32_t large_rows_bound,
-                     const PlaneTab *pt = nullptr)
+void ensure_work_lists(hesaff_ctx *c, Lists &s, uint32_t n)
+{
+   c->geo.b_bins.ensure_grow((size_t)n * HS_NLISTS * 4);
+   s.pw.bin_items = c->geo.b_bins.as<uint32_t>();
+   s.pw.cap = n;
+}
+
+PatchWork group_patch_work(hesaff_ctx *c, const Lists &s, int slot, uint32_t max_n)
+{
+   PatchWork pw = s.pw;
+   uint32_t *base = s.counters + 64 + 32 * slot;
+   pw.bin_count = base; pw.bin_work = base + 16;
+   pw.bin_items = c->geo.b_bins.as<uint32_t>() + (size_t)slot * HS_NLISTS * max_n;
+   pw.cap = max_n;
+   return pw;
+}
+
+bool run_patch_stage(hesaff_ctx *c, const Lists &s, const DPlane &image, float *patches_out, uint32_t h_base, uint32_t large_rows_bound,
+                     const PlaneTab *pt = nullptr, hipEvent_t ev_bin0 = nullptr)
 {
    hipStream_t st = c->stream;
    PatchIO io;
@@ -819,9 +835,10 @@
       }
       hipLaunchKernelGGL(k_patch_extract_small<0>, dim3(c->g_small0), dim3(256), small_extract_lds_bytes(0), s0, s.hl, s.pw, io, c->tables);
       if (forked) HIP_TRY(hipEventRecord(c->ev_join[0], s0));
+      if (forked && ev_bin0) HIP_TRY(hipEventRecord(ev_bin0, s0));
       hipLaunchKernelGGL(k_patch_pyramid, dim3((uint32_t)c->n_cu * 32u), dim3(256), 0, st, s.hl, s.pw, io, *pt, (int)c->oct.size(), c->consts.pd0, 1);
       if (forked) HIP_TRY(hipStreamWaitEvent(st, c->ev_join[0], 0));
-      return;
+      return forked && ev_bin0;
    }
    hipStream_t s0 = st, s1 = st, s2 = st, s3 = st;
    const bool forked = c->side_streams[0] && !c->no_overlap;
@@ -836,6 +853,7 @@
       PatchIO io3 = io;
       io3.trows = c->b_trows3.as<float>();
       hipLaunchKernelGGL(k_patch_extract_small<0>, dim3(c->g_small0), dim3(256), small_extract_lds_bytes(0), s0, s.hl, s.pw, io, c->tables);
+      if (forked && ev_bin0) HIP_TRY(hipEventRecord(ev_bin0, s0));
       hipLaunchKernelGGL(k_patch_extract_small<1>, dim3(c->g_small1), dim3(256), small_extract_lds_bytes(1), s1, s.hl, s.pw, io, c->tables);
       hipLaunchKernelGGL(k_patch_mid<HS_MID_PMAX>, dim3(c->g_mid), dim3(256), mid_lds_bytes(), s2, s.hl, s.pw, io2, c->tables);
       hipLaunchKernelGGL(k_patch_mid<HS_BIN3_PMAX>, dim3(c->g_big), dim3(256), big_lds_bytes(), s3, s.hl, s.pw, io3, c->tables);
@@ -872,6 +890,7 @@
       for (int i = 0; i < HS_NSIDE; i++) HIP_TRY(hipEventRecord(c->ev_join[i], c->side_streams[i]));
       for (int i = 0; i < HS_NSIDE; i++) HIP_TRY(hipStreamWaitEvent(st, c->ev_join[i], 0));
    }
+   return forked && ev_bin0;
 }
 
 void run_detection(hesaff_ctx *c, const SrcImages &src, int B, const Lists &s, StageTimer &tm, bool keep_all_planes, float *planes_out,
@@ -1067,16 +1086,17 @@
 
 void launch_sift(hesaff_ctx *c, hipStream_t ss, const SiftIO &so, uint32_t n, float2 *vo)
 {
-   const uint32_t nb64 = (n + 63) / 64;
+   const uint32_t nbq = (n + SQ_KP - 1) / SQ_KP;
    hipLaunchKernelGGL(k_sift_meanvar, dim3((n + SM_KP - 1) / SM_KP), dim3(64), 0, ss, so, c->tables);
    hipLaunchKernelGGL(k_sift_grad, dim3(std::min(n, c->sgrad_grid)), dim3(256), 0, ss, so, c->tables, vo);
    hipLaunchKernelGGL(k_sift_hist, dim3(std::min<uint32_t>((n + 3) / 4, c->g_shist)), dim3(64), 0, ss, so, c->tables, (const float2 *)vo);
-   hipLaunchKernelGGL(k_sift_quantize, dim3(nb64), dim3(64), 0, ss, so, c->consts);
+   hipLaunchKernelGGL(k_sift_quantize, dim3(nbq), dim3(64), 0, ss, so, c->consts);
 }
 
 void ensure_group_buffers(hesaff_ctx *c, uint32_t n)
 {
    for (int slot = 0; slot < HS_NSLOT; slot++) c->b_patches2[slot].ensure_grow((size_t)n * HS_PATCH_PIX * 4);
+   c->geo.b_bins.ensure_grow((size_t)HS_NSLOT * HS_NLISTS * n * 4);
    c->b_siftvec2.ensure_grow((size_t)n * 128 * 4);
    c->b_meanvar2.ensure_grow((size_t)n * 2 * 4);
    const void *before = c->b_siftvo2.p;
@@ -1147,19 +1167,26 @@
          if (as != st && with_affine) HIP_TRY(hipStreamWaitEvent(st, c->ev_aff[gi], 0));
          const int slot = (int)(gi % HS_NSLOT);
          if (slot_used[slot]) HIP_TRY(hipStreamWaitEvent(st, c->ev_sift_done[slot], 0));
+         Lists sg = s;
+         sg.pw = group_patch_work(c, s, slot, max_n);
          t = tm.begin(T_PATCH);
-         HIP_TRY(hipMemsetAsync(cnt + 8, 0, 24 * 4, st));
+         HIP_TRY(hipMemsetAsync(sg.pw.bin_count, 0, 32 * 4, st));
          hipLaunchKernelGGL(k_prepare_patch, dim3(1024), dim3(256), 0, st, s.hl, h_lo, h_hi, (const uint32_t *)(cnt + 3), s.ao, H, W, c->consts,
-                            c->tables, s.pw);
-         run_patch_stage(c, s, c->gray, c->b_patches2[slot].as<float>(), h_lo, groups[gi].large_rows, &pt);
+                            c->tables, sg.pw);
+         hipStream_t ss = c->no_overlap ? st : c->sift_stream;
+         const bool early = run_patch_stage(c, sg, c->gray, c->b_patches2[slot].as<float>(), h_lo, groups[gi].large_rows, &pt,
+                                            ss != st ? (hipEvent_t)c->ev_bin0_done[slot] : (hipEvent_t) nullptr);
          tm.end(t);
          HIP_TRY(hipEventRecord(c->ev_extract_done[slot], st));
-         hipStream_t ss = c->no_overlap ? st : c->sift_stream;
-         if (ss != st) HIP_TRY(hipStreamWaitEvent(ss, c->ev_extract_done[slot], 0));
          SiftIO so;
          so.patches = c->b_patches2[slot].as<float>(); so.alive = s.pw.alive; so.meanvar = c->b_meanvar2.as<float>();
          so.vec = c->b_siftvec2.as<float>(); so.desc = c->geo.b_desc.as<uint8_t>(); so.h_lo = h_lo; so.h_hi = h_hi;
+         if (ss != st) HIP_TRY(hipStreamWaitEvent(ss, early ? (hipEvent_t)c->ev_bin0_done[slot] : (hipEvent_t)c->ev_extract_done[slot], 0));
          const int ts = tm.begin(T_SIFT, 0, ss);
+         so.items = sg.pw.bin_items; so.count = sg.pw.bin_count;
+         launch_sift(c, ss, so, n, c->b_siftvo2.as<float2>());
+         if (ss != st && early) HIP_TRY(hipStreamWaitEvent(ss, c->ev_extract_done[slot], 0));
+         so.items = sg.pw.bin_items + (size_t)HS_LIST_REST * sg.pw.cap; so.count = sg.pw.bin_count + HS_LIST_REST;
          launch_sift(c, ss, so, n, c->b_siftvo2.as<float2>());
          tm.end(ts);
          HIP_TRY(hipEventRecord(c->ev_sift_done[slot], ss));
```

Result: no change. 38.34 million (-0.8%).
